# l-tamas/Fiasco

Hardware: AMD Instinct MI355X
Metric: grayscale frames/sec encoded (higher is better)
Workload: dtype f32

## Files before the change

### fiasco_amd/__init__.py

```python
import ctypes
import os
import subprocess

_HERE = os.path.dirname(os.path.abspath(__file__))
LIB_PATH = os.path.join(_HERE, "libfiasco_amd.so")
CSRC = os.path.join(_HERE, "csrc")

FIASCO_NO_VERBOSITY, FIASCO_SOME_VERBOSITY, FIASCO_ULTIMATE_VERBOSITY = 0, 1, 2
FIASCO_TILING_SPIRAL_ASC, FIASCO_TILING_SPIRAL_DSC = 0, 1
FIASCO_TILING_VARIANCE_ASC, FIASCO_TILING_VARIANCE_DSC = 2, 3
FIASCO_RPF_RANGE_0_75, FIASCO_RPF_RANGE_1_00, FIASCO_RPF_RANGE_1_50, FIASCO_RPF_RANGE_2_00 = 0, 1, 2, 3
FIASCO_PROGRESS_NONE, FIASCO_PROGRESS_BAR, FIASCO_PROGRESS_PERCENT = 0, 1, 2

EXPORTED_SYMBOLS = [
    "fiasco_get_error_message", "fiasco_set_verbosity", "fiasco_get_verbosity", "fiasco_coder",
    "fiasco_c_options_new", "fiasco_c_options_delete", "fiasco_c_options_set_smoothing",
    "fiasco_c_options_set_frame_pattern", "fiasco_c_options_set_tiling",
    "fiasco_c_options_set_basisfile", "fiasco_c_options_set_chroma_quality",
    "fiasco_c_options_set_optimizations", "fiasco_c_options_set_prediction",
    "fiasco_c_options_set_video_param", "fiasco_c_options_set_quantization",
    "fiasco_c_options_set_progress_meter", "fiasco_c_options_set_comment",
    "fiasco_c_options_set_title", "fiasco_calloc", "open_file", "fiasco_amd_set_limits",
    "fiasco_amd_get_limits", "fiasco_amd_encode_batch", "fiasco_amd_free",
    "fiasco_amd_get_stats", "fiasco_amd_reset_stats", "fiasco_amd_spec_workgroups", "fiasco_amd_core_name", "fiasco_amd_rccl_gather", "fiasco_amd_set_device",
    "fiasco_amd_batch_stage", "fiasco_amd_batch_encode", "fiasco_amd_batch_free",
    "fiasco_amd_batch_submit", "fiasco_amd_batch_collect", "fiasco_amd_batch_stats", "fiasco_amd_batch_decode_psnr", "fiasco_amd_batch_decode_psnr_all", "fiasco_amd_coop_workgroups", "fiasco_amd_share_of", "fiasco_amd_spec_append_helpers", "fiasco_amd_batch_decode_plane", "fiasco_amd_c_options_set_models",
    "fiasco_amd_release_memory", "fiasco_amd_batch_upload", "fiasco_amd_set_devices", "fiasco_amd_device_count",
    "fiasco_amd_selftest_log2", "fiasco_amd_selftest_log2_patched",
    "fiasco_amd_selftest_log2_max_ulp",
    "fiasco_amd_seq_open", "fiasco_amd_seq_free", "fiasco_amd_seq_gops", "fiasco_amd_seq_frames",
    "fiasco_amd_seq_gop_of", "fiasco_amd_seq_ycol_size", "fiasco_amd_seq_initial_level",
    "fiasco_amd_seq_search", "fiasco_amd_seq_gop_result", "fiasco_amd_seq_ycol", "fiasco_amd_seq_write",
    "fiasco_amd_seq_probe",
    "fiasco_amd_batch_stage_device", "fiasco_amd_batch_upload_device", "fiasco_amd_batch_input_planes",
]

FIASCO_AMD_GRAY8, FIASCO_AMD_RGB8_INTERLEAVED, FIASCO_AMD_RGB8_PLANAR = 0, 1, 2


class DeviceFrame(ctypes.Structure):
    _fields_ = [("data", ctypes.c_void_p), ("pitch", ctypes.c_size_t), ("plane_stride", ctypes.c_size_t),
                ("width", ctypes.c_uint), ("height", ctypes.c_uint), ("layout", ctypes.c_int)]


class Stats(ctypes.Structure):
    _fields_ = [("kernel_ms", ctypes.c_double), ("launches", ctypes.c_ulonglong),
                ("frames", ctypes.c_ulonglong), ("bytes_mp", ctypes.c_ulonglong),
                ("bytes_img", ctypes.c_ulonglong), ("bytes_gram", ctypes.c_ulonglong),
                ("n_mp", ctypes.c_ulonglong), ("n_steps", ctypes.c_ulonglong),
                ("n_blocks", ctypes.c_ulonglong), ("n_appends", ctypes.c_ulonglong),
                ("n_fulleval", ctypes.c_ulonglong), ("t_init", ctypes.c_ulonglong),
                ("t_approx", ctypes.c_ulonglong), ("t_ipis", ctypes.c_ulonglong),
                ("t_append", ctypes.c_ulonglong), ("t_serial", ctypes.c_ulonglong),
                ("t_total", ctypes.c_ulonglong), ("t_mpA", ctypes.c_ulonglong),
                ("t_mpB", ctypes.c_ulonglong), ("n_blockevals", ctypes.c_ulonglong),
                ("dbg", ctypes.c_ulonglong * 8), ("states_sum", ctypes.c_ulonglong),
                ("states_max", ctypes.c_ulonglong), ("reencodes", ctypes.c_ulonglong),
                ("frames_by_build", ctypes.c_ulonglong * 5),
                ("spec_frames", ctypes.c_ulonglong), ("spec_tasks", ctypes.c_ulonglong),
                ("spec_confirmed", ctypes.c_ulonglong), ("spec_wrong", ctypes.c_ulonglong),
                ("spec_timeout", ctypes.c_ulonglong), ("spec_inline", ctypes.c_ulonglong),
                ("spec_wait", ctypes.c_ulonglong), ("spec_tab_used", ctypes.c_ulonglong),
                ("spec_tab_missed", ctypes.c_ulonglong), ("spec_adopted", ctypes.c_ulonglong),
                ("decoder_frames", ctypes.c_ulonglong), ("decoder_bytes", ctypes.c_ulonglong),
                ("decoder_us", ctypes.c_ulonglong), ("coop_frames", ctypes.c_ulonglong),
                ("coop_workgroups", ctypes.c_ulonglong),
                ("spec_app_rows", ctypes.c_ulonglong), ("spec_app_wait", ctypes.c_ulonglong)]


def build(verbose=False):
    out = None if verbose else subprocess.DEVNULL
    subprocess.check_call(["make", "-C", CSRC], stdout=out)
    if not os.path.exists(LIB_PATH):
        raise RuntimeError("build did not produce %s" % LIB_PATH)


class FiascoError(RuntimeError):
    pass


class Library:

    def __init__(self, path=LIB_PATH):
        if not os.path.exists(path):
            raise FiascoError("%s is missing: run fiasco_amd.build() (there is no fallback)" % path)
        self.path = path
        L = self.L = ctypes.CDLL(path)
        c = ctypes
        L.fiasco_get_error_message.restype = c.c_char_p
        L.fiasco_set_verbosity.argtypes = [c.c_int]
        L.fiasco_get_verbosity.restype = c.c_int
        L.fiasco_c_options_new.restype = c.c_void_p
        L.fiasco_c_options_delete.argtypes = [c.c_void_p]
        L.fiasco_coder.argtypes = [c.POINTER(c.c_char_p), c.c_char_p, c.c_float, c.c_void_p]
        L.fiasco_coder.restype = c.c_int
        L.fiasco_amd_c_options_set_models.argtypes = [c.c_void_p, c.c_char_p, c.c_char_p, c.c_char_p, c.c_char_p]
        L.fiasco_amd_c_options_set_models.restype = c.c_int
        for name, args in [
            ("set_smoothing", [c.c_int]), ("set_frame_pattern", [c.c_char_p]),
            ("set_tiling", [c.c_int, c.c_uint]), ("set_basisfile", [c.c_char_p]),
            ("set_chroma_quality", [c.c_float, c.c_uint]),
            ("set_optimizations", [c.c_uint] * 5), ("set_prediction", [c.c_int, c.c_uint, c.c_uint]),
            ("set_video_param", [c.c_uint, c.c_int, c.c_int, c.c_int]),
            ("set_quantization", [c.c_uint, c.c_int, c.c_uint, c.c_int]),
            ("set_progress_meter", [c.c_int]), ("set_comment", [c.c_char_p]),
            ("set_title", [c.c_char_p]),
        ]:
            fn = getattr(L, "fiasco_c_options_" + name)
            fn.argtypes = [c.c_void_p] + args
            fn.restype = c.c_int
        L.fiasco_amd_set_limits.argtypes = [c.c_uint, c.c_uint]
        L.fiasco_amd_set_limits.restype = c.c_int
        L.fiasco_amd_get_limits.argtypes = [c.POINTER(c.c_uint), c.POINTER(c.c_uint)]
        L.fiasco_amd_encode_batch.argtypes = [c.c_uint, c.POINTER(c.c_char_p), c.POINTER(c.c_size_t),
                                              c.c_float, c.c_void_p, c.POINTER(c.c_void_p),
                                              c.POINTER(c.c_size_t)]
        L.fiasco_amd_encode_batch.restype = c.c_int
        L.fiasco_amd_free.argtypes = [c.c_void_p]
        L.fiasco_amd_core_name.restype = c.c_char_p
        if hasattr(L, "fiasco_amd_get_stats"):
            L.fiasco_amd_get_stats.argtypes = [c.POINTER(Stats)]

    def error_message(self):
        return self.L.fiasco_get_error_message().decode("latin-1")

    def core_name(self):
        return self.L.fiasco_amd_core_name().decode()

    def set_verbosity(self, level):
        self.L.fiasco_set_verbosity(level)

    def set_limits(self, max_states, max_level):
        if not self.L.fiasco_amd_set_limits(max_states, max_level):
            raise FiascoError(self.error_message())

    def get_limits(self):
        a, b = ctypes.c_uint(), ctypes.c_uint()
        self.L.fiasco_amd_get_limits(ctypes.byref(a), ctypes.byref(b))
        return a.value, b.value

    def set_devices(self, ids):
        arr = (ctypes.c_int * max(len(ids), 1))(*ids)
        self.L.fiasco_amd_set_devices.argtypes = [ctypes.POINTER(ctypes.c_int), ctypes.c_int]
        if not self.L.fiasco_amd_set_devices(arr, len(ids)):
            raise FiascoError(self.error_message())

    def device_count(self):
        return self.L.fiasco_amd_device_count()

    def set_device(self, device):
# ... 404 lines not shown
```

### fiasco_amd/csrc/hip/core_hip.cpp

```cpp
#include <hip/hip_runtime.h>
#include <stdio.h>
#include <stdlib.h>
#include <string.h>
#include <stddef.h>
#include <pthread.h>
#include <algorithm>
#include <utility>
#include <vector>
#include "fa_host.h"
#include "frame_coder.h"
#include "libfiasco_amd_hip.h"

extern "C" const char *fa_knob(const char *name)
{
    const char *d = getenv("FIASCO_AMD_DEBUG");
    return d && *d && strcmp(d, "0") != 0 ? getenv(name) : nullptr;
}
static long long knob_int(const char *name, long long d)
{
    const char *e = fa_knob(name);
    return e ? atoll(e) : d;
}


// ... 741 lines not shown
    return room > (size_t) G ? room - (size_t) G : 0;
}
static int spec_app_policy(size_t frames, int cus, int G, bool wide_build, int occ)
{
    if (!frames || G < 2 || cus < 1) return 0;
    size_t H = spec_app_room(frames, cus, G, occ);
    if (!wide_build) {
        return H >= 3 && 2 * frames * ((size_t) G + 3) <= 3 * (size_t) cus ? 3 : 0;
    }
    if (H > 3) H = 3;
    return H >= 2 ? (int) H : 0;
}
extern "C" int fiasco_amd_spec_append_helpers(unsigned frames, int cus, int G, int wide_build)
{
    return spec_app_policy(frames, cus, G, wide_build != 0, wide_build ? 1 : 4);
}

static int spec_groups(size_t frames, int cus, bool big_frames, bool narrow_only)
{
    const char *e = fa_knob("FIASCO_AMD_SPEC");
    if (e && atoi(e) <= 1) return 0;
    if (fa_knob("FIASCO_AMD_TRACE") || fa_knob("FIASCO_AMD_NO_WIDE") || fa_knob("FIASCO_AMD_FORCE_TRI")) return 0;
    int occ = fc_occupancy_spec();
    if (occ < 1) occ = 1;
    if (!frames) return 0;
    if (e) {
        size_t G = (size_t) cus * (size_t) occ / frames;
        if ((size_t) atoi(e) < G) G = (size_t) atoi(e);
        if (G > FC_SPEC_MAXG) G = FC_SPEC_MAXG;
        return G >= 2 ? (int) G : 0;
    }
    return spec_policy(frames, cus, big_frames, narrow_only, occ);
}

static int spec_policy(size_t frames, int cus, bool big_frames, bool narrow_only, int occ)
{
    if (!frames || cus < 1) return 0;
    size_t G = (size_t) cus / frames;
    if (G > FC_SPEC_MAXG) G = FC_SPEC_MAXG;
    if (narrow_only && !big_frames && occ >= 2) {
        G = (size_t) cus * (size_t) occ / frames;
        if (G > FC_SPEC_MAXG) G = FC_SPEC_MAXG;
        if (G > 5 && 2 * frames * G > 5 * (size_t) cus) {
            G = 5 * (size_t) cus / (2 * frames);
            if (G < 5) G = 5;
        }
    }
    (void) big_frames;
    return G >= 3 ? (int) G : 0;
}

static void fill_frame(FrameSlot &fs, const fa_job *job)
{
    const fa_cparams *cp = &job->cp;
    const fa_wfa *w = job->wfa;
    DevFrame &F = fs.F;
    const Layout &L = fs.L;
    char *base = fs.base;
    memset(&F, 0, sizeof F);
    F.price = cp->price;
    F.lc_min = (int) cp->lc_min_level; F.lc_max = (int) cp->lc_max_level;
    F.images_level = (int) cp->images_level; F.max_elements = (int) cp->max_elements;
    const bool bxl = long_basis(w);
    {
        unsigned live = cp->max_elements;
        for (unsigned st = 0; st < (bxl ? 0u : w->basis_states); st++)
            for (unsigned l = 0; l < 2; l++) {
                unsigned e = 0;
                while (e < 6 && FA_INTO(w, st, l, e) != FA_NO_EDGE) e++;
                if (e > live) live = e;
            }
        F.maxe_live = (int) live;
    }
    F.level = (int) cp->level; F.width = (int) job->image->width; F.height = (int) job->image->height;
    F.pool_max = (int) cp->pool_max_states; F.limit_states = (int) cp->limit_states;
    F.ML = (int) cp->limit_level;
    F.rpf_mant = (int) cp->rpf.mantissa_bits; F.dc_mant = (int) cp->dc_rpf.mantissa_bits;
    F.rpf_range = cp->rpf.range; F.dc_range = cp->dc_rpf.range;
    F.P = fs.P; F.PA = fs.PA;
    F.gram_ls = fs.tri ? (unsigned) ((size_t) fs.P * (fs.P + 1) / 2 + fs.P) : (unsigned) fs.P * (unsigned) fs.P;
    F.color = job->image->color ? 1 : 0;
    F.chroma_cl_cap = (int) knob_int("FIASCO_AMD_CLMAX", 0);
    F.chroma_sparse = !fa_knob("FIASCO_AMD_CHROMA_FULL") && (cp->pool_kind == FA_POOL_RLE || cp->pool_kind == FA_POOL_ADAPTIVE || cp->pool_kind == FA_POOL_BASIS);
    F.chroma_max = (int) cp->chroma_max_states;
    F.chroma_decrease = cp->chroma_decrease;
    F.plane = (unsigned long long) job->image->width * job->image->height;
    F.gl0 = (int) (cp->lc_min_level < cp->images_level ? cp->lc_min_level : cp->images_level);
    F.NL = (int) cp->lc_max_level - F.gl0 + 1;
    F.second_domain_block = cp->second_domain_block ? 1 : 0;
    F.check_underflow = cp->check_for_underflow ? 1 : 0;
    F.check_overflow = cp->check_for_overflow ? 1 : 0;
    F.full_search = cp->full_search ? 1 : 0;
    F.NS = (int) fa_size_of_tree(cp->products_level);
    F.NA = 1 << (cp->lc_max_level - cp->images_level);
    F.NI = (int) fa_size_of_tree(cp->images_level);
    F.dcs = 1 << (1 + F.dc_mant); F.sy = 1 << (1 + F.rpf_mant);
    F.coeff_size = (F.lc_max - F.lc_min + 1) * F.sy + F.dcs;
    F.coeff_nt = F.lc_max - F.lc_min + 2;
    F.basis_states = (int) w->basis_states;
    F.bx = bxl ? (const int *) (base + L.bx) : nullptr;
    F.gm_pool[0] = (int) cp->pool_kind; F.gm_pool[1] = (int) cp->d_pool_kind;
    F.gm_coeff[0] = (int) cp->coeff_kind; F.gm_coeff[1] = (int) cp->d_coeff_kind;
    F.gq = fs.gm ? (int16_t *) (base + L.gq) : nullptr;
    F.lginv = fs.gm ? (const double *) (base + L.lginv) : nullptr;
    for (unsigned s = 0; s < (bxl ? 0u : w->basis_states); s++) {
        F.b_final[s] = w->final_distribution[s];
        F.b_dtype[s] = w->domain_type[s];
        for (int l = 0; l < 2; l++) {
            F.b_tree[s][l] = FA_TREE(w, s, l);
            for (int e = 0; e < 6; e++) {
                F.b_into[s][l][e] = FA_INTO(w, s, l, e);
                F.b_weight[s][l][e] = FA_WEIGHT(w, s, l, e);
                if (FA_INTO(w, s, l, e) == FA_NO_EDGE) break;
            }
        }
    }
    F.pix16 = (const int16_t *) (base + L.pix16);
    F.gram = (float *) (base + L.gram); F.diag = (float *) (base + L.diag);
    F.ipis = (float *) (base + L.ipis); F.d5 = (float *) (base + L.d5);
    F.gcol = (float *) (base + L.gcol);
    F.d4 = (float *) (base + L.d4); F.imgT4 = (float *) (base + L.imgT4);
    F.img = (float *) (base + L.img); F.imgT = (float *) (base + L.imgT);
    F.norms = (float *) (base + L.norms);
    F.num = (float *) (base + L.num); F.den = (float *) (base + L.den);
    F.est = (float *) (base + L.est); F.ipdo = (float *) (base + L.ipdo);
    F.used = (uint8_t *) (base + L.used);
    F.tree = (int16_t *) (base + L.tree); F.into = (int16_t *) (base + L.into);
    F.weight = (float *) (base + L.weight); F.final_d = (float *) (base + L.final_d);
    F.level_of_state = (uint8_t *) (base + L.level_of_state);
    F.domain_type = (uint8_t *) (base + L.domain_type);
    F.x = (uint16_t *) (base + L.x); F.y = (uint16_t *) (base + L.y);
    F.ycol = (uint8_t *) (base + L.ycol);
    F.ycol0 = job->ycol_carry ? (const uint8_t *) (base + L.ycol0) : nullptr;
    F.pool_states = (int16_t *) (base + L.pool_states);
    F.pos = (int16_t *) (base + L.pos);
    F.hits = (int *) (base + L.hits);
    F.snap_hbm = fs.big ? (void *) (base + L.snap) : nullptr;
    F.l2_keys = g_l2.d_keys; F.l2_vals = g_l2.d_vals; F.l2_mask = g_l2.mask;
    const int inter = job->frame_type != FA_I_FRAME;
    F.pred_on = cp->prediction || inter ? 1 : 0;
    F.pred_root = job->image->color ? inter : (cp->prediction || inter ? 1 : 0);
    F.search_range = (int) cp->search_range;
    F.mv = (int16_t *) (base + L.mv);
    F.past = (const int16_t *) (base + L.past); F.future = (const int16_t *) (base + L.future);
    F.coop = (FcCoop *) (base + L.coop);
    F.mc_fwd = (float *) (base + L.mc_fwd); F.mc_bwd = inter ? (float *) (base + L.mc_bwd) : nullptr;
    F.pix_chroma = (int16_t *) (base + L.pix_chroma);
    F.frame_type = job->frame_type;
    F.p_min = (int) cp->p_min_level; F.p_max = (int) cp->p_max_level;
    F.d_rpf_mant = (int) cp->d_rpf.mantissa_bits; F.d_dc_mant = (int) cp->d_dc_rpf.mantissa_bits;
    F.d_rpf_range = cp->d_rpf.range; F.d_dc_range = cp->d_dc_rpf.range;
    F.d_dcs = 1 << (1 + F.d_dc_mant); F.d_sy = 1 << (1 + F.d_rpf_mant);
    F.d_coeff_size = (F.lc_max - F.lc_min + 1) * F.d_sy + F.d_dcs;
    F.ipis_alt = (float *) (base + L.ipis_alt); F.d5_alt = (float *) (base + L.d5_alt);
    F.d4_alt = (float *) (base + L.d4_alt); F.pix_save = (float *) (base + L.pix_save);
    F.sv_gram = (float *) (base + L.sv_gram); F.sv_img = (float *) (base + L.sv_img);
    F.sv_auto = (FcSavedRow *) (base + L.sv_auto);
    F.max_save = L.max_save;
    F.slab_base = base; F.slab_bytes = L.total;
}

static void slot_layout(Staged *S, FrameSlot &fs)
{
    const fa_job *job = &S->jobs[fs.job];
    const fa_cparams *cp = &job->cp;
    int il = (int) cp->images_level;
// ... 431 lines not shown
    }
    const char *const host = pinned;
    const int16_t *tree = (const int16_t *) host;
    const int16_t *into = (const int16_t *) (host + (L.into - L.tree));
    const float *weight = (const float *) (host + (L.weight - L.tree));
    const float *fin = (const float *) (host + (L.final_d - L.tree));
    const uint8_t *los = (const uint8_t *) (host + (L.level_of_state - L.tree));
    const uint8_t *dt = (const uint8_t *) (host + (L.domain_type - L.tree));
    const uint16_t *xs = (const uint16_t *) (host + (L.x - L.tree));
    const uint16_t *ys = (const uint16_t *) (host + (L.y - L.tree));
    const uint8_t *ycol = (const uint8_t *) (host + (L.ycol - L.tree));
    const int16_t *mv = (const int16_t *) (host + (L.mv - L.tree));
    const bool inter = job->frame_type != FA_I_FRAME;
    for (unsigned s = 0; s < w->basis_states; s++) w->level_of_state[s] = 0xff;
    fa_wfa_remove_states(w, w->basis_states);
    for (unsigned s = w->basis_states; s < ns; s++) {
        w->final_distribution[s] = fin[s];
        w->domain_type[s] = dt[s];
        w->level_of_state[s] = los[s];
        w->delta_state[s] = 0;
        for (int l = 0; l < 2; l++) {
            FA_TREE(w, s, l) = tree[(size_t) l * P + s];
            w->x[s * 2 + l] = xs[(size_t) l * P + s];
            w->y[s * 2 + l] = ys[(size_t) l * P + s];
            w->y_state[s * 2 + l] = FA_RANGE;
            w->y_column[s * 2 + l] = F.color ? ycol[(size_t) l * P + s] : 0;
            w->prediction[s * 2 + l] = 0;
            if (inter) {
                fa_mv *m = &w->mv[s * 2 + l];
                m->type = mv[(size_t) (0 * 2 + l) * P + s]; m->fx = mv[(size_t) (1 * 2 + l) * P + s];
                m->fy = mv[(size_t) (2 * 2 + l) * P + s]; m->bx = mv[(size_t) (3 * 2 + l) * P + s];
                m->by = mv[(size_t) (4 * 2 + l) * P + s];
            }
            for (int e = 0; e < 6; e++) {
                FA_INTO(w, s, l, e) = into[(size_t) (l * 6 + e) * P + s];
                FA_WEIGHT(w, s, l, e) = weight[(size_t) (l * 6 + e) * P + s];
                if (FA_INTO(w, s, l, e) == FA_NO_EDGE) break;
            }
        }
    }
    if (F.color)
        for (unsigned s = 0; s < w->cap && s < (unsigned) P; s++)
            for (int l = 0; l < 2; l++) w->y_column[s * 2 + l] = ycol[(size_t) l * P + s];
    w->states = ns;
    w->root_state = (unsigned) F.root_state;
    job->stats[0].costs = F.costs; job->stats[0].err = F.err;
    job->stats[0].tree_bits = F.tree_bits; job->stats[0].matrix_bits = F.matrix_bits;
    job->stats[0].weights_bits = F.weights_bits;
    if (F.color) {
        for (int b = 0; b < 2; b++) {
            job->stats[b + 1].costs = F.c_costs[b]; job->stats[b + 1].err = F.c_err[b];
            job->stats[b + 1].tree_bits = F.c_tree_bits[b];
            job->stats[b + 1].matrix_bits = F.c_matrix_bits[b];
            job->stats[b + 1].weights_bits = F.c_weights_bits[b];
        }
        int ycb = FA_TREE(w, ns - 1, 0), crs = FA_TREE(w, ns - 1, 1);
        int roots[2] = { FA_TREE(w, ycb, 1), FA_TREE(w, crs, 0) };
        int yroot = FA_TREE(w, ycb, 0);
        std::vector<std::pair<int, int>> stack;
        for (int b = 0; b < 2; b++) {
            stack.push_back(std::make_pair(roots[b], yroot));
            while (!stack.empty()) {
                std::pair<int, int> t = stack.back();
                stack.pop_back();
                int s = t.first, y = t.second;
                if (s == FA_RANGE || (unsigned) s < w->basis_states) continue;
                for (int l = 0; l < 2; l++) {
                    int ny = y != FA_RANGE ? FA_TREE(w, y, l) : FA_RANGE;
                    w->y_state[s * 2 + l] = (int16_t) ny;
                    stack.push_back(std::make_pair((int) FA_TREE(w, s, l), ny));
                }
            }
        }
    }
    job->lc_min_level_out = (unsigned) F.lc_min_out;
    job->status = 1;
    g_stats.frames += 1;
    g_stats.bytes_mp += F.bytes_mp; g_stats.bytes_img += F.bytes_img; g_stats.bytes_gram += F.bytes_gram;
    g_stats.n_mp += F.n_mp; g_stats.n_steps += F.n_steps; g_stats.n_blocks += F.n_blocks;
    g_stats.n_appends += F.n_appends; g_stats.n_fulleval += F.n_fulleval;
    g_stats.t_init += F.t_init; g_stats.t_approx += F.t_approx; g_stats.t_ipis += F.t_ipis;
    g_stats.t_append += F.t_append; g_stats.t_serial += F.t_serial; g_stats.t_total += F.t_total;
    g_stats.t_mpA += F.t_mpA; g_stats.t_mpB += F.t_mpB; g_stats.n_blockevals += F.n_blockevals;
    for (int k = 0; k < 8; k++) g_stats.dbg[k] += F.dbg[k];
    g_stats.states_sum += ns;
    if (ns > g_stats.states_max) g_stats.states_max = ns;
    cap_hint_put(job, F.ystates_out, F.states);
    if (fa_knob("FIASCO_AMD_CAP_TRACE"))
        fprintf(stderr, "capacity: frame type %d used %d table states of %d, %d states of %d; %.3f s on the device\n", job->frame_type,
                F.ystates_out, fs.P, F.states, fs.PA, (double) F.t_total / 1e8);
    return 1;
}

static bool queue_resources(Staged *S, size_t frames)
{
    if (!grow_buffer(S->d_ring, S->ring_n, 5 * frames)) return false;
    if (!S->d_queue && hipMalloc((void **) &S->d_queue, 2 * 5 * sizeof(unsigned)) != hipSuccess) {
        S->d_queue = nullptr; (void) hipGetLastError(); return false;
    }
    if (!S->ptrmask_ready) {
        const size_t words = FC_DESC_WORDS, mwords = (words + 31) / 32;
        std::vector<unsigned> mask(mwords, 0u);
        FrameSlot a = S->slots[S->lender0], b = S->slots[S->lender0];
        const fa_job *job = &S->jobs[a.job];
        b.base = a.base + (1u << 24);
        fill_frame(a, job); fill_frame(b, job);
        const unsigned long long *wa = (const unsigned long long *) &a.F, *wb = (const unsigned long long *) &b.F;
        for (size_t w = 0; w < sizeof(DevFrame) / 8; w++)
            if (wa[w] != wb[w]) mask[w >> 5] |= 1u << (w & 31);
        const size_t wp = offsetof(DevFrame, pack_src) / 8;
        mask[wp >> 5] |= 1u << (wp & 31);
        if (!S->d_ptrmask && hipMalloc((void **) &S->d_ptrmask, mwords * sizeof(unsigned)) != hipSuccess) {
            S->d_ptrmask = nullptr; (void) hipGetLastError(); return false;
        }
        if (hipMemcpy(S->d_ptrmask, mask.data(), mwords * sizeof(unsigned), hipMemcpyHostToDevice) != hipSuccess) return false;
        S->ptrmask_ready = true;
    }
    return true;
}

struct WaveGroups { size_t n[N_BUILDS], lend[N_BUILDS], borrow[N_BUILDS]; };

static bool order_batch(Staged *S, WaveGroups &g)
{
    std::vector<size_t> &batch = S->batch;
    batch.clear();
    for (size_t k = 0; k < S->slots.size(); k++)
        if (S->slots[k].staged && !S->slots[k].done) batch.push_back(k);
    if (batch.empty()) return false;
    memset(&g, 0, sizeof g);
    const bool few = batch.size() <= (size_t) S->ncu && !fa_knob("FIASCO_AMD_NO_WIDE");
    std::vector<int> key(S->slots.size());
    for (size_t k : batch) {
        const FrameSlot &fs = S->slots[k];
        const Build b = build_of(S, fs, few);
        const int part = fs.borrow ? 1 : S->borrowers && queue_eligible(S, fs) && queue_layout(S, fs) ? 0 : 2;
        key[k] = 3 * b + part;
        g.n[b]++;
        if (part == 0) g.lend[b]++; else if (part == 1) g.borrow[b]++;
        if (k_build[b].stats_slot >= 0) g_stats.frames_by_build[k_build[b].stats_slot]++; else g_stats.spec_frames++;
    }
    std::stable_sort(batch.begin(), batch.end(), [&](size_t a, size_t b) { return key[a] < key[b]; });
    return true;
}

static void place_packs(Staged *S)
{
    const std::vector<size_t> &batch = S->batch;
    std::vector<DevFrame> &hf = S->hf;
    hf.resize(batch.size());
    S->pack_off.assign(batch.size(), 0);
    size_t need = 0;
    for (size_t b = 0; b < batch.size(); b++) {
        const FrameSlot &fs = S->slots[batch[b]];
        hf[b] = fs.F;
        hf[b].pack_src = fs.F.slab_base + fs.L.tree;
        hf[b].pack_bytes = (unsigned) (fs.L.pool_states - fs.L.tree);
        S->pack_off[b] = need;
        need += align_up(fs.L.pool_states - fs.L.tree, 256);
    }
    S->pack_need = need;
    S->parity ^= 1;
    char *&pack = S->d_pack[S->parity];
    (void) grow_buffer(pack, S->d_pack_bytes[S->parity], need);
    if (!S->cstream && hipStreamCreateWithFlags(&S->cstream, hipStreamNonBlocking) != hipSuccess) {
        S->cstream = nullptr; (void) hipGetLastError();
// ... 930 lines not shown
```

### fiasco_amd/csrc/hip/fc_lds.inc

```

#define RANGE_E (FC_MAXE + 1)
struct __attribute__((aligned(16))) Range {
    int   x, y, image, address, level, tree;
    float weight[RANGE_E];
    short into[RANGE_E];
    float err, tree_bits, matrix_bits, weights_bits;
#if FC_VARIANT_BIG
    float nd_tree_bits, nd_weights_bits, mv_tree_bits, mv_coord_bits;
    int   prediction;
    short mv[5];
#endif
};

struct Pool {
    short count[MAXED + 1];
    unsigned short total, n, max_domains, y_index;
    short d0_index;
    unsigned short d0_yindex, d0_n;
};

struct __attribute__((aligned(16))) SFrame {
    Range rg, lrange, rrange, child[2];
    Pool  pool0, pool_lc;
    float max_costs, lincomb, subdiv, ret, price;
    int   label, states, phase, leaf, coop;
    int   y_state, ny[2];
#if FC_GM
    int   rn0;
#endif
#if FC_SPEC
    int   ckpt;
#endif
#if FC_VARIANT_BIG
    int   pred, delta, try_pred, pred_done, rec_states;
    int   norm_first, norm_done;
    Pool  dpool0, pool_rec, dpool_rec;
    Range prange;
    float pred_max, pred_costs, nd_w, nd_wbits, nd_tbits;
#endif
};

struct MPState {
    int   n, best_n, index, D, N, level, image, address, row_state;
    short indices[MAXED + 1], into[MAXED + 1];
    float weight[MAXED];
    unsigned symp;
    float matrix_bits, weights_bits, err, costs, min_costs;
    float sel_ipdo[MAXED][MAXED];
    float norm_ov[MAXED + 1], ipio[MAXED + 1];
    short psorted[MAXED + 1];
    int   np;
    float wb_dc, wb_nd, norm, ab, price;
    int   y_state, ypos;
#if FC_VARIANT_BIG
    const float *numrow;
    short excl[MAXED + 1];
#endif
#if FC_GM
    short kq[MAXED + 1];
#endif
    float s1_pre[MAXED], s1_sfx[MAXED], s1_z0, s1_zy;
    int   s1_last[MAXED], s1_k[MAXED], s1_thr[MAXED];
    unsigned s1_cd, s1_has;
};

struct __attribute__((aligned(16))) CoeffBuf {
    short tot[16];
    short cnt[FC_VARIANT_BIG ? FC_MAXCOEFF_BIG : FC_MAXCOEFF];
};
#if FC_VARIANT_BIG
#define SNAP_POOL16 880
#define SNAP_TM_WORDS 2392
#else
#define SNAP_POOL16 (FC_VARIANT_WIDE ? FC_SNAP16_WIDE : FC_SNAP16_NARROW)
#define SNAP_TM_WORDS (FC_VARIANT_WIDE ? FC_SNAPTM_WIDE : FC_SNAPTM_NARROW)
#endif
#if FC_VARIANT_BIG || FC_VARIANT_WIDE
#define NBLOCKMIN   256
#else
#define NBLOCKMIN   64
#endif
#define TM_WORDS    (4 * 26 + 8)

struct RoundBox {
    float m2[2];
    int   state;
    int   idx;
    float cost, mbits, wbits, err, f[MAXED];
    float num, den, ip[MAXED - 1];
    unsigned evals, blockevals;
    unsigned symp;
};
#define SYMP_NONE 0u
#define SYMP_HAS(p, k) ((k) < 3 && (((p) >> (10 * (k))) & 1023u) != 0u)
#define SYMP_GET(p, k) ((int) (((p) >> (10 * (k))) & 1023u) - 2)
#define SYMP_PUT(sym, k) ((unsigned) ((sym) + 2) << (10 * (k)))

struct Sh {
    RoundBox rb;
    SFrame   st[FC_DEPTH];
    int      sp;
    int      op, a0, a1, a2, a3;
#if FC_VARIANT_BIG
    unsigned coopW, coop_seq;
    int      coopD, coop_minsub;
    unsigned long long coop_ticks;
#endif
    Pool     pool;
    CoeffBuf cb;
#if FC_VARIANT_BIG
    Pool     dpool;
    CoeffBuf dcb;
    struct { int rpf_mant, dc_mant, sy, dcs; float rpf_range, dc_range; int half_nd, half_dc; } dq;
    int      nslot;
    uint4   *snap_tm_p;
    int      pred_active, pred_lo, pred_rec;
    struct { int type, fx, fy, bx, by; float bits, tree_bits; } mc;
    unsigned long long mcred[B / 64];
    unsigned pred_saved[FC_MAXSAVE / 32];
#endif
    uint4    snap_pool[SNAP_POOL16];
    uint4   *snap;
    int      n16;
    __attribute__((aligned(16))) unsigned tm[TM_WORDS];
    __attribute__((aligned(16))) unsigned snap_tm[SNAP_TM_WORDS];
    float    m0tab[12];
    double   lgdc[FC_MAXSYM], lglv[FC_MAXSYM], lglv_m1;
    float    Ltab[MAXED + 1];
    float    Q0, Q1;
    float    tb[2];
    MPState  mp;
#if FC_VARIANT_BIG
    MPState  mp_keep;
    int      apx_stage, apx_it, apx_more;
#endif
    float    blockmin[NBLOCKMIN];
    __attribute__((aligned(16))) float pixels[FC_PIXELS];
    float    norms[FC_PIXELS / 32];
    unsigned long long tk[16];
    struct {
        unsigned long long bytes_mp, bytes_img, bytes_gram, n_mp, n_steps, n_blocks, n_appends,
                           n_fulleval, n_blockevals, t_mpA, t_mpB;
    } cnt;
#ifdef FC_SERIAL_PROFILE
    unsigned long long tk_ph[8], ph_t0, tk_init[2], tk_apx[4];
    int      ph_prev;
#endif
    int      band, lc_min, tree_band[3], ystates, after_chroma;
    short    dl[64];
#if !FC_SPEC
    short    cl[FC_CLMAX];
    int      cln;
#endif
    unsigned long long red[B / 64];
    int      gs_idx[2][MAXED + 1], gs_n[2], gs_c[2], gs_raw_idx[2][MAXED + 1];
    float    gs_raw_w[2][MAXED + 1];
    float    gs_w[2][MAXED + 1];
    struct {
        int lc_max, width, height, limit_states, PA, P, ML; float price, chroma_decrease;
        float *gram, *diag, *ipis; int16_t *pos; unsigned gram_ls;
        float *gcol;
        float *d5, *d4;
        const unsigned *l2_keys; const double *l2_vals; unsigned l2_mask;
        int max_elements, rpf_mant, dc_mant, sy, dcs, gl0, images_level, lc_min_opt, trace_on;
        int snap_b1;
        int16_t *at_tree, *at_into, *at_pool; float *at_weight, *at_final; uint8_t *at_los, *at_dtype, *at_ycol;
        uint16_t *at_x, *at_y; int color;
        float rpf_range, dc_range;
        int half_nd, half_dc;
    } par;
#if FC_GM
    struct { int pk[2], ck[2], qa; float base, kept; double lg1; int16_t *gq; int P; } gm;
#endif
    int      states;
    int      flim;
    int      failed;
#if FC_SPEC
    int      gap_lo, gap_hi, gap_shift;
    unsigned deadmask;
    int      cap;
    int      blk;
    int      tab_shared;
    int      tab_from;
    struct SpecLocal {
        FcSpecCtl *ctl;
        char     *slots;
        int       role, on;
        int       mode;
        int       T;
        int       chroma_tabs;
        char     *tabs;
        unsigned  rb_s[32];
        unsigned  blkof[FC_SPEC_W];
        unsigned  sk[FC_SPEC_W];
        unsigned long long n_tab_used, n_tab_missed, n_adopted;
        int       floor;
        unsigned  head, commit;
        unsigned  spec_mask;
        int       nospec;
        unsigned  epoch;
        int       verdict, abort, busy;
        unsigned  ops;
        float     mlc, lin[FC_SPEC_W];
        unsigned  nlc;
        float     learn;
        unsigned long long n_tasks, n_confirmed, n_wrong, n_timeout, n_inline, t_wait;
        unsigned  app_H, app_min, app_seq, app_off;
        unsigned long long n_app_dealt, t_app_wait;
    } sl;
#endif
};
#if FC_GM
#define GM_QAC(k)   ((k) == FC_PK_ADAPTIVE || (k) == FC_PK_BASIS)
#define GM_RLE(k)   ((k) == FC_PK_RLE || (k) == FC_PK_RLE_NO_CHROMA)
#define GQ_CUR(sh, set)          ((sh).gm.gq + (size_t) ((sh).gm.qa ^ (set)) * (sh).gm.P)
#define GQ_SNAP(sh, depth, slot) ((sh).gm.gq + (size_t) (2 + (depth) * 5 + (slot)) * (sh).gm.P)
#endif
#if FC_SPEC
#define DEAD(sh, s) ((unsigned) ((int) (s) - (sh).gap_lo) < (unsigned) ((sh).gap_hi - (sh).gap_lo))
#else
#define DEAD(sh, s) false
#endif
```

### fiasco_amd/csrc/hip/fc_models.inc

```

#if FC_VARIANT_BIG
#define SNAP(sh) ((sh).snap)
#define NSLOT(sh) ((sh).nslot)
#define SNAP_TM(sh) ((sh).snap_tm_p)
#define TM_SLOTS(sh) ((sh).nslot == 5 ? 2 : 1)
#else
#define SNAP(sh) ((sh).snap_pool)
#define NSLOT(sh) 2
#define SNAP_TM(sh) ((uint4 *) (sh).snap_tm)
#define TM_SLOTS(sh) 1
#endif
#if FC_VARIANT_BIG
#define SNAP_AT(sh, depth, which) (SNAP(sh) + ((depth) * NSLOT(sh) + (which)) * (sh).n16)
#else
#define SNAP_AT(sh, depth, which) (SNAP(sh) + ((which) ? (sh).par.snap_b1 + (depth) : (depth)) * (sh).n16)
#endif
#if FC_VARIANT_BIG
#define TM_N16(ML) (ML)
#else
#define TM_N16(ML) ((2 * (ML) + 3) / 4)
#endif
#define TM_AT(sh, depth, which, ML) (SNAP_TM(sh) + ((depth) * TM_SLOTS(sh) + (which)) * TM_N16(ML))

#if FC_GM

__device__ __forceinline__ float gm_m0(const Sh &sh, int idx) { return sh.m0tab[qac_shift(idx)]; }
__device__ __forceinline__ float gm_m1(int idx) { return (float) qac_shift(idx); }

__device__ void gq_copy(int16_t *dst, const int16_t *src, int n)
{
    const int n16 = (n + 7) / 8;
    for (int i = 0; i < n16; i++) ((uint4 *) dst)[i] = ((const uint4 *) src)[i];
}
__device__ void gq_save(Sh &sh, int set, int depth, int slot)
{
    if (GM_QAC(sh.gm.pk[set])) gq_copy(GQ_SNAP(sh, depth, slot), GQ_CUR(sh, set), set ? sh.dpool.n : sh.pool.n);
}
__device__ void gq_load(Sh &sh, int set, int depth, int slot)
{
    if (GM_QAC(sh.gm.pk[set])) gq_copy(GQ_CUR(sh, set), GQ_SNAP(sh, depth, slot), set ? sh.dpool.n : sh.pool.n);
}
__device__ __forceinline__ void gq_save_par(Sh &sh, int set, int depth, int slot)
{
    if (!GM_QAC(sh.gm.pk[set])) return;
    const int n = set ? sh.dpool.n : sh.pool.n;
    int16_t *d = GQ_SNAP(sh, depth, slot);
    const int16_t *c = GQ_CUR(sh, set);
    for (int i = threadIdx.x; i < n; i += B) d[i] = c[i];
}

__device__ __forceinline__ bool gm_accepts(const Pool &m, int kind)
{
    return kind == FC_PK_CONSTANT || kind == FC_PK_UNIFORM || m.n < m.max_domains;
}
__device__ bool gm_take(Sh &sh, Pool &m, int kind, int set, int state)
{
    if (kind == FC_PK_CONSTANT) return false;
    if (kind != FC_PK_UNIFORM && m.n >= m.max_domains) return false;
    if (GM_QAC(kind)) { int16_t *q = GQ_CUR(sh, set); q[m.n] = m.n > 0 ? q[m.n - 1] : (int16_t) 0; }
    if (GM_RLE(kind) && state == 0) { m.d0_index = 0; m.d0_n = 1; }
    m.n++;
    return true;
}
__device__ void gm_offer(DevFrame &F, Sh &sh, int s)
{
    const int L = sh.pool.n > sh.dpool.n ? sh.pool.n : sh.dpool.n;
    bool grow = gm_take(sh, sh.pool, sh.gm.pk[0], 0, s);
    if (F.pred_on) grow = gm_take(sh, sh.dpool, sh.gm.pk[1], 1, s) || grow;
    F.pos[s] = -1;
    if (grow) { F.pos[s] = (short) L; F.pool_states[L] = (short) s; }
}
#endif

__device__ __forceinline__ void snap_coop_before(Sh &sh, SFrame &fr, int depth, int ML)
{
    const int tid = threadIdx.x;
#if FC_HM
    for (int i = tid; i < sh.n16; i += B) SNAP_AT(sh, depth, 0)[i] = ((const uint4 *) &sh.cb)[i];
    if (tid >= 96 && tid < 96 + TM_N16(ML)) TM_AT(sh, depth, 0, ML)[tid - 96] = ((const uint4 *) sh.tm)[tid - 96];
    if (tid == 128) fr.pool0 = sh.pool;
#if FC_GM
    if (tid == 130) fr.rn0 = sh.dpool.n;
    gq_save_par(sh, 0, depth, 0);
#endif
    if (sh.nslot == 5 && !fr.delta) {
        if (tid == 129) fr.dpool0 = sh.dpool;
        for (int i = tid; i < sh.n16; i += B) SNAP_AT(sh, depth, 2)[i] = ((const uint4 *) &sh.dcb)[i];
#if FC_GM
        gq_save_par(sh, 1, depth, 2);
#endif
    }
    return;
#endif
    if (tid < sh.n16) SNAP_AT(sh, depth, 0)[tid] = ((const uint4 *) &sh.cb)[tid];
    else if (tid >= 96 && tid < 96 + TM_N16(ML))
        TM_AT(sh, depth, 0, ML)[tid - 96] = ((const uint4 *) sh.tm)[tid - 96];
    else if (tid == 128) fr.pool0 = sh.pool;
#if FC_VARIANT_BIG
    else if (sh.nslot == 5 && !fr.delta) {
        if (tid == 129) fr.dpool0 = sh.dpool;
        else if (tid >= 160 && tid < 160 + sh.n16) SNAP_AT(sh, depth, 2)[tid - 160] = ((const uint4 *) &sh.dcb)[tid - 160];
    }
#endif
}

__device__ __forceinline__ void snap_coop_after(Sh &sh, SFrame &fr, int depth)
{
    const int tid = threadIdx.x;
#if FC_HM
    for (int i = tid; i < sh.n16; i += B) {
        SNAP_AT(sh, depth, 1)[i] = ((const uint4 *) &sh.cb)[i];
        ((uint4 *) &sh.cb)[i] = SNAP_AT(sh, depth, 0)[i];
    }
#if FC_GM
    if (GM_QAC(sh.gm.pk[0])) {
        const int n1 = sh.pool.n, n0 = fr.pool0.n;
        int16_t *cur = GQ_CUR(sh, 0), *s1 = GQ_SNAP(sh, depth, 1);
        const int16_t *s0 = GQ_SNAP(sh, depth, 0);
        for (int i = tid; i < (n1 > n0 ? n1 : n0); i += B) {
            if (i < n1) s1[i] = cur[i];
            if (i < n0) cur[i] = s0[i];
        }
    }
    __syncthreads();
#endif
    if (tid == 128) {
#else
    if (tid < sh.n16) {
        SNAP_AT(sh, depth, 1)[tid] = ((const uint4 *) &sh.cb)[tid];
        ((uint4 *) &sh.cb)[tid] = SNAP_AT(sh, depth, 0)[tid];
    } else if (tid == 128) {
#endif
        fr.pool_lc = sh.pool;
        sh.pool = fr.pool0;
#if FC_GM
        if (fr.delta) sh.dpool.n = (unsigned short) fr.rn0;
#endif
    }
}

__device__ float tree_bits_dev(const Sh &sh, int ML, int child, int level, int which);
```

### fiasco_amd/csrc/hip/fc_serial.inc

```


__device__ float tree_bits_dev(const Sh &sh, int ML, int child, int level, int which)
{
    const unsigned *counts = sh.tm + which * 2 * ML;
    float prob = counts[level] / (float) counts[ML + level];
    return child ? (float) -log2((double) prob) : (float) -log2((double) (1 - prob));
}

__device__ void tree_update_dev(Sh &sh, int ML, int child, int level, int which)
{
    unsigned *counts = sh.tm + which * 2 * ML;
    if (child) counts[level]++;
    counts[ML + level]++;
}

__device__ __forceinline__ void copy16(uint4 *dst, const uint4 *src, int n)
{
    int i = 0;
    for (; i + 8 <= n; i += 8) {
        uint4 t0 = src[i], t1 = src[i + 1], t2 = src[i + 2], t3 = src[i + 3];
        uint4 t4 = src[i + 4], t5 = src[i + 5], t6 = src[i + 6], t7 = src[i + 7];
        dst[i] = t0; dst[i + 1] = t1; dst[i + 2] = t2; dst[i + 3] = t3;
        dst[i + 4] = t4; dst[i + 5] = t5; dst[i + 6] = t6; dst[i + 7] = t7;
    }
    for (; i < n; i++) dst[i] = src[i];
}

__device__ void snap_save(const DevFrame &F, Sh &sh, int depth, int which)
{
    copy16(SNAP_AT(sh, depth, which), (const uint4 *) &sh.cb, sh.n16);
}

__device__ void snap_load(const DevFrame &F, Sh &sh, int depth, int which)
{
    copy16((uint4 *) &sh.cb, SNAP_AT(sh, depth, which), sh.n16);
}

#if FC_VARIANT_BIG
__device__ void snap_save_d(Sh &sh, int depth, int which)
{
    copy16(SNAP_AT(sh, depth, which), (const uint4 *) &sh.dcb, sh.n16);
}

__device__ void snap_load_d(Sh &sh, int depth, int which)
{
    copy16((uint4 *) &sh.dcb, SNAP_AT(sh, depth, which), sh.n16);
}
#endif

__device__ __forceinline__ void tm_save(Sh &sh, int depth, int ML, int which = 0)
{
    copy16(TM_AT(sh, depth, which, ML), (const uint4 *) sh.tm, TM_N16(ML));
}

__device__ __forceinline__ void tm_load(Sh &sh, int depth, int ML, int which = 0)
{
    copy16((uint4 *) sh.tm, TM_AT(sh, depth, which, ML), TM_N16(ML));
}

__device__ float final_distribution_dev(const DevFrame &F, int s)
{
    float f = 0;
    int dom;
    for (int l = 0; l < 2; l++) {
        if ((dom = TREE(F, s, l)) != RANGE_) f += F.final_d[dom];
        for (int e = 0; (dom = INTO(F, s, l, e)) != NOEDGE; e++)
            f += WEIGHT(F, s, l, e) * F.final_d[dom];
    }
    return f / 2;
}

#if !FC_VARIANT_BIG
__device__ void store_new_state(DevFrame &__restrict__ F, Sh &sh, SFrame &fr, int aux)
{
    const int s = sh.states, PA = sh.par.PA;
    GLOBAL_AS int16_t *const tree = (GLOBAL_AS int16_t *) sh.par.at_tree, *const into = (GLOBAL_AS int16_t *) sh.par.at_into;
    GLOBAL_AS int16_t *const posv = (GLOBAL_AS int16_t *) sh.par.pos, *const pool = (GLOBAL_AS int16_t *) sh.par.at_pool;
    GLOBAL_AS float *const weight = (GLOBAL_AS float *) sh.par.at_weight, *const fin = (GLOBAL_AS float *) sh.par.at_final;
    GLOBAL_AS uint16_t *const xs = (GLOBAL_AS uint16_t *) sh.par.at_x, *const ys = (GLOBAL_AS uint16_t *) sh.par.at_y;
    short p = -1;
    if (!aux && sh.pool.n < sh.pool.max_domains) {
        p = (short) sh.pool.n;
        pool[sh.pool.n++] = (short) s;
    }
    posv[s] = p;
    fr.rrange.into[0] = NOEDGE;
    fr.rrange.tree = s;
    int   tr[2], i[2][3];
    float w[2][3], fd_t[2], fd_e[2][3];
#pragma unroll
    for (int l = 0; l < 2; l++) {
        const Range &ch = fr.child[l];
        tr[l] = ch.tree;
        bool live = true;
#pragma unroll
        for (int e = 0; e < 3; e++) {
// ... 103 lines not shown
    F.final_d[s] = final_distribution_dev(F, s);
    F.level_of_state[s] = (uint8_t) fr.rrange.level;
    F.domain_type[s] = aux ? 0 : 2;
}
#endif

__device__ int append_join_state(DevFrame &__restrict__ F, Sh &__restrict__ sh, int t0, int t1, int level)
{
    const int s = sh.states;
    if (s >= F.PA) { sh.failed = FC_ERR_CAPACITY; return 0; }
    TREE(F, s, 0) = (short) t0; TREE(F, s, 1) = (short) t1;
    for (int l = 0; l < 2; l++) {
        INTO(F, s, l, 0) = NOEDGE;
        F.x[l * F.PA + s] = 0; F.y[l * F.PA + s] = 0;
    }
    F.final_d[s] = final_distribution_dev(F, s);
    F.level_of_state[s] = (uint8_t) level;
    F.domain_type[s] = 0;
    F.pos[s] = -1;
#if FC_VARIANT_BIG
    if (F.frame_type) for (int k = 0; k < 10; k++) F.mv[k * F.PA + s] = 0;
#endif
    sh.states++;
    if (sh.states >= F.limit_states) { sh.failed = FC_ERR_STATES; return 0; }
    return 1;
}

__device__ void push_root(DevFrame &__restrict__ F, Sh &__restrict__ sh, int y_state)
{
    SFrame &r = sh.st[0];
    r.rg.x = r.rg.y = r.rg.image = r.rg.address = 0;
    r.rg.level = F.level; r.rg.tree = RANGE_;
    for (int i = 0; i < RANGE_E; i++) { r.rg.weight[i] = 0; r.rg.into[i] = 0; }
    r.rg.err = r.rg.tree_bits = r.rg.matrix_bits = r.rg.weights_bits = 0;
    r.max_costs = MAXCOSTS;
    r.y_state = y_state;
    r.phase = PH_ENTER;
#if FC_SPEC
    r.ckpt = 0;
#endif
#if FC_VARIANT_BIG
    r.rg.nd_tree_bits = r.rg.nd_weights_bits = r.rg.mv_tree_bits = r.rg.mv_coord_bits = 0; r.rg.prediction = 0;
    for (int i = 0; i < 5; i++) r.rg.mv[i] = 0;
    r.pred = sh.band == 0 ? F.pred_root : 0;
    r.delta = 0;
#endif
    sh.sp = 0;
}

__device__ int band_advance(DevFrame &__restrict__ F, Sh &__restrict__ sh)
{
    if (!sh.after_chroma) {
        const SFrame &r = sh.st[0];
        const Range &rg = r.rg;
        const int band = sh.band;
        if (band == 0) {
            F.costs = r.ret; F.err = rg.err; F.tree_bits = rg.tree_bits;
            F.matrix_bits = rg.matrix_bits; F.weights_bits = rg.weights_bits;
            F.root_state = rg.tree;
        } else {
            F.c_costs[band - 1] = r.ret; F.c_err[band - 1] = rg.err;
            F.c_tree_bits[band - 1] = rg.tree_bits; F.c_matrix_bits[band - 1] = rg.matrix_bits;
            F.c_weights_bits[band - 1] = rg.weights_bits;
        }
        if (sh.failed) return 0;
        if (rg.tree == RANGE_) { sh.failed = FC_ERR_NOROOT; return 0; }
        if (!F.color) return 0;
        sh.tree_band[band] = rg.tree;
        if (band == 1) {
            if (!append_join_state(F, sh, sh.tree_band[0], sh.tree_band[1], F.level + 1)) return 0;
            sh.tree_band[1] = sh.states - 1;
        }
        if (band == 2) {
            if (!append_join_state(F, sh, sh.tree_band[2], RANGE_, F.level + 1)) return 0;
            if (!append_join_state(F, sh, sh.tree_band[1], sh.states - 1, F.level + 2)) return 0;
            F.root_state = sh.states - 1;
            return 0;
        }
        sh.band = band + 1;
        if (band == 0) { sh.op = OP_CHROMA; sh.after_chroma = 1; return 1; }
    }
    sh.after_chroma = 0;
    sh.op = OP_NOP;
    push_root(F, sh, sh.tree_band[0]);
    return 1;
}

#if FC_SPEC
#define SPEC_DEKKER_FENCE() __builtin_amdgcn_fence(__ATOMIC_SEQ_CST, "agent")
#define SPEC_TIMEOUT_TICKS 20000000ull
__device__ __noinline__ int spec_poll(Sh &sh, bool drain)
{
    Sh::SpecLocal &sl = sh.sl;
    FcSpecCtl *c = sl.ctl;
    unsigned long long t0 = 0;
    if (sl.learn != 0.0f) { sl.mlc = sl.nlc ? 0.9f * sl.mlc + 0.1f * sl.learn : sl.learn; sl.nlc++; sl.learn = 0.0f; }
    while (sl.commit != sl.head) {
        const unsigned slot = sl.commit % FC_SPEC_W;
        const bool mine = (sl.spec_mask >> slot) & 1u;
        if (!mine) { sl.commit++; t0 = 0; continue; }
        const unsigned v = __hip_atomic_load(&c->verdict[slot], __ATOMIC_RELAXED, __HIP_MEMORY_SCOPE_AGENT);
        if ((v >> 11) != sl.commit + 1) {
            if (!drain && sl.head - sl.commit < FC_SPEC_W) {
                __hip_atomic_store(&c->committed, sl.commit, __ATOMIC_RELAXED, __HIP_MEMORY_SCOPE_AGENT);
                return 0;
            }
            const unsigned long long now = wall_clock64();
            if (!t0) t0 = now;
            if (now - t0 < SPEC_TIMEOUT_TICKS) { __builtin_amdgcn_s_sleep(16); continue; }
            sl.t_wait += now - t0;
            sl.n_timeout++;
        } else {
            if (t0) { sl.t_wait += wall_clock64() - t0; t0 = 0; }
            if ((v & 3u) == 1u) {
                if (sh.par.color) {
                    GLOBAL_AS uint8_t *yc = (GLOBAL_AS uint8_t *) sh.par.at_ycol;
                    const unsigned used = (v >> 2) & 63u, s0 = sl.sk[slot];
                    for (unsigned j = 0; j < used; j++) { yc[s0 + j] = 0; yc[(unsigned) sh.par.PA + s0 + j] = 0; }
                }
                sl.mlc = sl.nlc ? 0.9f * sl.mlc + 0.1f * sl.lin[slot] : sl.lin[slot]; sl.nlc++;
                sl.commit++; sl.n_confirmed++;
                continue;
            }
            sl.n_wrong++;
            if ((v & 3u) == 3u && sl.sk[slot] + ((v >> 2) & 63u) <= (unsigned) sh.cap)
                return (1 + (int) slot) | 0x100 | (int) (((v >> 2) & 63u) << 16) | (int) (((v >> 8) & 7u) << 24);
        }
        return 1 + (int) slot;
    }
    __hip_atomic_store(&c->committed, sl.commit, __ATOMIC_RELAXED, __HIP_MEMORY_SCOPE_AGENT);
    return 0;
}
#endif

#if FC_SPEC
__device__ __noinline__ void spec_luminance_done(Sh &sh)
{
    FcSpecCtl *c = sh.sl.ctl;
    sh.sl.epoch++;
    __hip_atomic_store(&c->epoch, sh.sl.epoch, __ATOMIC_RELEASE, __HIP_MEMORY_SCOPE_AGENT);
    SPEC_DEKKER_FENCE();
    const unsigned long long t0 = wall_clock64();
    while (__hip_atomic_load(&c->busy, __ATOMIC_ACQUIRE, __HIP_MEMORY_SCOPE_AGENT) != 0) {
        if (wall_clock64() - t0 > 100000000ull) { sh.failed = FC_ERR_INTERNAL; break; }
        __builtin_amdgcn_s_sleep(32);
    }
    sh.sl.on = 0; sh.sl.mode = 0;
    sh.sl.chroma_tabs = c->n_tabs > c->n_blocks;
}
#endif

#ifndef FC_SERIAL_LOOP
#define FC_SERIAL_LOOP 0
#endif
__device__ __forceinline__ int serial_step(DevFrame &__restrict__ F, Sh &__restrict__ sh, int &sp, int &phase)
{
    const int ML = sh.par.ML;
    {
#if FC_SPEC
        const int spec_mode = *(volatile int *) &sh.sl.mode;
#endif
        if (sp < 0) {
            sh.sp = sp;
#if FC_SPEC
            if (spec_mode == 1) {
                sh.op = OP_SPEC_CKPT; sh.a0 = 2;
                return 0;
            }
#endif
            const int more = band_advance(F, sh);
            sp = sh.sp; phase = sp >= 0 ? sh.st[sp].phase : 0;
            if (!more) { sh.op = OP_DONE; return 0; }
            if (sh.op == OP_CHROMA) return 0;
            return 1;
        }
        SFrame &fr = sh.st[sp];
#ifdef FC_SERIAL_PROFILE
        {
            unsigned long long t = wall_clock64();
            sh.tk_ph[sh.ph_prev] += t - sh.ph_t0; sh.ph_t0 = t; sh.ph_prev = phase;
        }
#endif
        switch (phase) {
        case PH_ENTER: {
            Range &rg = fr.rg;
            rg.into[0] = NOEDGE;
            rg.tree = RANGE_;
            fr.ret = MAXCOSTS;
            if (sh.failed || rg.level < 3) { fr.ret = MAXCOSTS; goto pop; }
            if (rg.x >= sh.par.width || rg.y >= sh.par.height) { fr.ret = 0; goto pop; }
#if FC_SPEC
#endif
            fr.price = sh.par.price;
            if (sh.band) fr.price *= sh.par.chroma_decrease;
#if FC_VARIANT_BIG
            fr.try_pred = 0;
            if (fr.pred && rg.level >= F.p_min && rg.level <= F.p_max) {
                if (F.frame_type == 0) fr.try_pred = 1;
                else if (rg.x + (int) width_of_level(rg.level) <= sh.par.width
                         && rg.y + (int) height_of_level(rg.level) <= sh.par.height) fr.try_pred = 2;
            }
            fr.pred_done = 0;
            fr.norm_first = 1; fr.norm_done = 0;
#endif
            phase = PH_AFTER_INIT;
            if (rg.level == sh.par.lc_max) {
                rg.address = rg.image = 0;
                sh.op = OP_INIT_RANGE; sh.a0 = rg.x; sh.a1 = rg.y;
#if FC_SPEC
                sh.a2 = (!sh.band || sh.sl.chroma_tabs) ? sh.blk++ : -1;
#endif
                return 0;
            }
            break;
        }
        case PH_AFTER_INIT: {
            Range &rg = fr.rg;
#if FC_SPEC
            if (spec_mode == 1 && rg.level == sh.par.lc_max && !sh.band && !fr.ckpt && sp > 0) {
                fr.ckpt = 1; sh.op = OP_SPEC_CKPT; sh.a0 = 1;
                return 0;
            }
#endif
            fr.leaf = rg.level <= sh.lc_min && rg.level <= sh.par.lc_max;
#if FC_VARIANT_BIG
            if (fr.try_pred) fr.leaf = 0;
#endif
            fr.coop = !fr.leaf && rg.level <= sh.par.lc_max;
            if (!fr.leaf && !fr.coop) {
                fr.pool0 = sh.pool;
                snap_save(F, sh, sp, 0);
                tm_save(sh, sp, ML);
#if FC_GM
                fr.rn0 = sh.dpool.n;
                gq_save(sh, 0, sp, 0);
#endif
#if FC_VARIANT_BIG
                if (sh.nslot == 5 && !fr.delta) {
                    fr.dpool0 = sh.dpool; snap_save_d(sh, sp, 2);
#if FC_GM
                    gq_save(sh, 1, sp, 2);
#endif
                }
#endif
            }
            fr.states = sh.states;
            for (int l = 0; l < 2; l++)
                fr.ny[l] = (sh.band && fr.y_state != RANGE_) ? (int) TREE(F, fr.y_state, l) : RANGE_;
            phase = PH_AFTER_LC;
            if (rg.level <= sh.par.lc_max) {
                fr.lrange = rg;
                fr.lrange.tree = RANGE_;
#if FC_VARIANT_BIG
                fr.lrange.tree_bits = tree_bits_dev(sh, ML, 0, rg.level, 0);
#endif
                fr.lrange.matrix_bits = 0;
                fr.lrange.weights_bits = 0;
#if FC_VARIANT_BIG
                fr.lrange.nd_tree_bits = 0; fr.lrange.nd_weights_bits = 0; fr.lrange.prediction = 0;
                fr.lrange.mv_tree_bits = fr.try_pred == 2 ? 1.0f : 0.0f;
                fr.lrange.mv_coord_bits = 0;
#endif
                sh.op = OP_APPROX;
                return 0;
            }
            fr.lincomb = MAXCOSTS;
            break;
        }
        case PH_AFTER_LC: {
            Range &rg = fr.rg;
            if (fr.leaf) {
                fr.subdiv = MAXCOSTS;
                phase = PH_DECIDE;
                break;
            }
            if (!fr.coop) {
#if FC_VARIANT_BIG
                fr.pool_lc = sh.pool;
                snap_save(F, sh, sp, 1);
#if FC_GM
                gq_save(sh, 0, sp, 1);
#endif
                sh.pool = fr.pool0;
                snap_load(F, sh, sp, 0);
#if FC_GM
                gq_load(sh, 0, sp, 0);
                if (fr.delta) sh.dpool.n = (unsigned short) fr.rn0;
#endif
#else
                fr.pool_lc = sh.pool;
#endif
            }
#if FC_SPEC
            if (fr.ckpt == 3) {
                fr.subdiv = MAXCOSTS;
                phase = PH_DECIDE;
                break;
            }
#endif
            if (rg.level > sh.lc_min) {
                Range z;
                z.x = z.y = z.image = z.address = z.level = 0; z.tree = 0;
                for (int i = 0; i < RANGE_E; i++) { z.weight[i] = 0; z.into[i] = 0; }
                z.err = z.tree_bits = z.matrix_bits = z.weights_bits = 0;
#if FC_VARIANT_BIG
                z.nd_tree_bits = z.nd_weights_bits = z.mv_tree_bits = z.mv_coord_bits = 0; z.prediction = 0;
                for (int i = 0; i < 5; i++) z.mv[i] = 0;
#endif
                fr.child[0] = z; fr.child[1] = z;
                fr.rrange = rg;
#if FC_VARIANT_BIG
                fr.rrange.tree_bits = tree_bits_dev(sh, ML, 1, rg.level, 0);
#else
                fr.rrange.tree_bits = rg.level <= sh.par.lc_max ? sh.tb[1] : tree_bits_dev(sh, ML, 1, rg.level, 0);
#endif
                fr.rrange.matrix_bits = 0;
                fr.rrange.weights_bits = 0;
                fr.rrange.err = 0;
#if FC_VARIANT_BIG
                fr.rrange.mv_tree_bits = fr.try_pred == 2 ? 1.0f : 0.0f;
                fr.rrange.mv_coord_bits = 0;
                fr.rrange.nd_tree_bits = fr.try_pred == 1 ? tree_bits_dev(sh, ML, 1, rg.level, 1) : 0.0f;
                fr.rrange.nd_weights_bits = 0;
                fr.rrange.prediction = 0;
                fr.subdiv = (fr.rrange.tree_bits + fr.rrange.weights_bits + fr.rrange.matrix_bits
                             + fr.rrange.mv_tree_bits + fr.rrange.mv_coord_bits + fr.rrange.nd_tree_bits
                             + fr.rrange.nd_weights_bits) * fr.price;
#else
                fr.subdiv = (fr.rrange.tree_bits + fr.rrange.weights_bits + fr.rrange.matrix_bits) * fr.price;
#endif
                fr.label = 0;
                phase = PH_CHILD;
            } else {
                fr.subdiv = MAXCOSTS;
                phase = PH_DECIDE;
            }
            break;
        }
        case PH_CHILD: {
            const Range &rr = fr.rrange;
            const int label = fr.label;
            Range &ch = fr.child[label];
            ch.image = rr.image * 2 + label + 1;
            ch.address = rr.address * 2 + label;
            ch.level = rr.level - 1;
            ch.x = (rr.level & 1) ? rr.x : rr.x + label * (int) width_of_level(rr.level - 1);
            ch.y = (rr.level & 1) ? rr.y + label * (int) height_of_level(rr.level - 1) : rr.y;
            phase = PH_CHILD2;
            if (label && rr.level <= sh.par.lc_max && sh.states > fr.states && !sh.band) {
                sh.op = OP_IPIS_INCR; sh.a0 = ch.image; sh.a1 = ch.address; sh.a2 = ch.level;
                sh.a3 = fr.states;
                return 0;
            }
            break;
        }
        case PH_CHILD2: {
            float lim = fr.lincomb > fr.max_costs ? fr.max_costs : fr.lincomb;
            float remaining = lim - fr.subdiv;
            phase = PH_CHILD_RET;
            fr.ret = 0;
            if (remaining > 0) {
                if (sp + 1 >= FC_DEPTH) { sh.failed = FC_ERR_INTERNAL; break; }
                SFrame &cf = sh.st[sp + 1];
                cf.rg = fr.child[fr.label];
                cf.y_state = fr.ny[fr.label];
                cf.max_costs = remaining;
                cf.phase = PH_ENTER;
#if FC_SPEC
                cf.ckpt = 0;
#endif
#if FC_VARIANT_BIG
                cf.pred = fr.pred; cf.delta = fr.delta;
#endif
                fr.phase = phase; sp++; phase = PH_ENTER;
                break;
            }
            fr.ret = -1;
            break;
        }
        case PH_CHILD_RET: {
            const int label = fr.label;
            float lim = fr.lincomb > fr.max_costs ? fr.max_costs : fr.lincomb;
#if FC_VARIANT_BIG
            if (fr.try_pred == 2 && !fr.norm_done) {
                const Range &c0 = fr.child[label];
                sh.op = OP_NORMS; sh.a0 = fr.rg.level; sh.a1 = fr.norm_first;
                sh.a2 = (fr.ret < 0 && c0.level >= F.p_min) ? c0.level : -1;
                sh.a3 = c0.x | (c0.y << 16);
                fr.norm_first = 0; fr.norm_done = 1;
                return 0;
            }
            fr.norm_done = 0;
#endif
            if (fr.ret >= 0) fr.subdiv += fr.ret;
            if (fr.subdiv >= lim) {
                fr.subdiv = MAXCOSTS;
                phase = PH_DECIDE;
                break;
            }
            const Range &ch = fr.child[label];
            fr.rrange.err          += ch.err;
            fr.rrange.tree_bits    += ch.tree_bits;
            fr.rrange.matrix_bits  += ch.matrix_bits;
            fr.rrange.weights_bits += ch.weights_bits;
#if FC_VARIANT_BIG
            fr.rrange.mv_tree_bits    += ch.mv_tree_bits;
            fr.rrange.mv_coord_bits   += ch.mv_coord_bits;
            fr.rrange.nd_weights_bits += ch.nd_weights_bits;
            fr.rrange.nd_tree_bits    += ch.nd_tree_bits;
            tree_update_dev(sh, ML, ch.tree != RANGE_, ch.level, 0);
            tree_update_dev(sh, ML, !ch.prediction, ch.level, 1);
#else
            tree_update_dev(sh, ML, ch.tree != RANGE_, ch.level, 0);
#endif
            fr.label = label + 1;
            phase = fr.label < 2 ? PH_CHILD : PH_DECIDE;
            break;
        }
        case PH_DECIDE: {
            Range &rg = fr.rg;
#if FC_SPEC
            if (spec_mode >= 2 && sp == spec_mode - 2) {
                sh.sl.verdict = (!sh.failed && !fr.leaf && fr.lincomb < MAXCOSTS && fr.lincomb < fr.subdiv) ? 1 : 2;
                if (!sh.failed && !fr.leaf && fr.subdiv < MAXCOSTS && !(fr.lincomb < fr.subdiv)) sh.sl.verdict = 3;
                sh.op = OP_DONE;
                return 0;
            }
#endif
#if FC_VARIANT_BIG
            if (fr.try_pred && !fr.pred_done && !sh.failed) { phase = PH_PRED_BEGIN; break; }
#endif
            if (fr.leaf) {
                if (fr.lincomb < MAXCOSTS) { rg = fr.lrange; fr.ret = fr.lincomb; }
                else fr.ret = MAXCOSTS;
                goto pop;
            } else if (fr.lincomb >= MAXCOSTS && fr.subdiv >= MAXCOSTS) {
                sh.pool = fr.pool0;
                snap_load(F, sh, sp, 0);
                tm_load(sh, sp, ML);
#if FC_GM
                gq_load(sh, 0, sp, 0);
                if (fr.delta) sh.dpool.n = (unsigned short) fr.rn0;
#endif
#if FC_VARIANT_BIG
                if (sh.nslot == 5 && !fr.delta) {
                    sh.dpool = fr.dpool0; snap_load_d(sh, sp, 2);
#if FC_GM
                    gq_load(sh, 1, sp, 2);
#endif
                }
#endif
                sh.states = fr.states;
                if (sh.flim > sh.states) sh.flim = sh.states & ~(GRAM_FB - 1);
                fr.ret = MAXCOSTS;
                goto pop;
            } else if (fr.lincomb < fr.subdiv) {
#if FC_SPEC
                if (fr.ckpt == 2 && spec_mode == 1) sh.sl.learn = fr.lincomb;
#endif
                sh.pool = fr.pool_lc;
                snap_load(F, sh, sp, 1);
                tm_load(sh, sp, ML);
#if FC_GM
                gq_load(sh, 0, sp, 1);
                if (fr.delta) sh.dpool.n = (unsigned short) fr.rn0;
#endif
#if FC_VARIANT_BIG
                if (sh.nslot == 5 && !fr.delta) {
                    sh.dpool = fr.dpool0; snap_load_d(sh, sp, 2);
#if FC_GM
                    gq_load(sh, 1, sp, 2);
#endif
                }
#endif
                rg = fr.lrange;
                sh.states = fr.states;
                if (sh.flim > sh.states) sh.flim = sh.states & ~(GRAM_FB - 1);
                fr.ret = fr.lincomb;
                goto pop;
            } else {
                int aux = sh.band > 0 || rg.x + (int) width_of_level(rg.level) > sh.par.width
                          || rg.y + (int) height_of_level(rg.level) > sh.par.height;
#if FC_VARIANT_BIG
#if FC_GM
                if (!(gm_accepts(sh.pool, sh.gm.pk[0]) || !F.pred_on || gm_accepts(sh.dpool, sh.gm.pk[1]))) aux = 1;
#else
                if (F.pred_on && sh.pool.n >= sh.pool.max_domains) aux = 1;
#endif
#endif
#if FC_SPEC
                if (sh.states >= (sh.band ? sh.par.PA : *(volatile int *) &sh.cap)) { sh.failed = FC_ERR_CAPACITY; fr.ret = MAXCOSTS; goto pop; }
#else
                if (sh.states >= (sh.band ? sh.par.PA : sh.par.P)) { sh.failed = FC_ERR_CAPACITY; fr.ret = MAXCOSTS; goto pop; }
#endif
                store_new_state(F, sh, fr, aux);
                phase = PH_AFTER_APPEND;
                if (!aux) { sh.op = OP_APPEND; sh.a0 = sh.states; return 0; }
                break;
            }
        }
#if FC_SPEC
        case PH_SPEC_END: {
            sh.sl.verdict = 2; sh.op = OP_DONE;
            return 0;
        }
#endif
        case PH_AFTER_APPEND: {
            sh.states++;
#if FC_SPEC
            if (sh.states - *(volatile int *) &sh.gap_shift >= sh.par.limit_states) sh.failed = FC_ERR_STATES;
#else
            if (sh.states >= sh.par.limit_states) sh.failed = FC_ERR_STATES;
#endif
            fr.rg = fr.rrange;
            fr.ret = fr.subdiv;
            goto pop;
        }
#if FC_VARIANT_BIG
        case PH_PRED_BEGIN: {
            Range &rg = fr.rg;
            const int il = sh.par.images_level, P = sh.par.P;
            float maxc = fr.lincomb > fr.subdiv ? fr.subdiv : fr.lincomb;
            if (maxc > fr.max_costs) maxc = fr.max_costs;
            fr.pred_done = 1;
            fr.pred_max = maxc;
            fr.rec_states = sh.states;
            fr.pool_rec = sh.pool; fr.dpool_rec = sh.dpool;
            snap_save(F, sh, sp, 3); snap_save_d(sh, sp, 4); tm_save(sh, sp, ML, 1);
#if FC_GM
            gq_save(sh, 0, sp, 3); gq_save(sh, 1, sp, 4);
#endif
            sh.pool = fr.pool0; sh.dpool = fr.dpool0;
            snap_load(F, sh, sp, 0); snap_load_d(sh, sp, 2); tm_load(sh, sp, ML, 0);
#if FC_GM
            gq_load(sh, 0, sp, 0); gq_load(sh, 1, sp, 2);
#endif
            sh.states = fr.states;
            if (sh.flim > sh.states) sh.flim = sh.states & ~(GRAM_FB - 1);
            if (fr.try_pred == 2) {
                sh.op = OP_MC_SEARCH; sh.a0 = rg.level; sh.a1 = rg.x | (rg.y << 16);
                sh.a2 = (rg.level == F.p_min ? 1 : 0) | (rg.level > F.p_min && fr.norm_first ? 2 : 0);
                phase = PH_PRED_MC2;
                return 0;
            }
            {
// ... 147 lines not shown
```

### fiasco_amd/csrc/hip/frame_coder.h

```cpp
#ifndef FRAME_CODER_H
#define FRAME_CODER_H
#include <stdint.h>

#define FC_MAXED    5
#define FC_BLOCK    256
#define FC_MAXDEPTH 22
#define FC_MAXDEPTH_BIG 32
#define FC_MAXDEPTH_NARROW 18
#define FC_SNAP16_NARROW 480
#define FC_SNAP16_WIDE   840
#define FC_SNAPTM_NARROW 988
#define FC_SNAPTM_WIDE   1092
#define FC_MAXSAVE  512
#define FC_MAXCOEFF 224
#ifndef FC_HM
#define FC_HM 0
#endif
#ifndef FC_GM
#define FC_GM 0
#endif
enum { FC_PK_ADAPTIVE = 0, FC_PK_CONSTANT = 1, FC_PK_BASIS = 2, FC_PK_UNIFORM = 3, FC_PK_RLE = 4, FC_PK_RLE_NO_CHROMA = 5 };
enum { FC_CK_ADAPTIVE = 0, FC_CK_UNIFORM = 1 };
#define FC_GQ_SLOTS (2 + FC_MAXDEPTH_BIG * 5)
#define FC_MAXCOEFF_BIG_STD 640
#define FC_MAXSYM_STD   64
#define FC_MAXCOEFF_HM  5120
#define FC_MAXSYM_HM    512
#define FC_MAXCOEFF_BIG (FC_HM ? FC_MAXCOEFF_HM : FC_MAXCOEFF_BIG_STD)
#define FC_MAXSYM       (FC_HM ? FC_MAXSYM_HM : FC_MAXSYM_STD)
#define FC_N16(coeffs)  ((32 + 2 * (coeffs) + 15) / 16)
#define FC_N16MAX       FC_N16(FC_MAXCOEFF_BIG)
#define FC_MAXBASIS 16
#define FC_BX_BYTES (64 * 1024)
#ifndef FC_TRI_HOT
#define FC_TRI_HOT  8
#endif

enum { FC_OK = 1, FC_ERR_STATES = 2, FC_ERR_CAPACITY = 3, FC_ERR_NOROOT = 4, FC_ERR_INTERNAL = 5,
       FC_ERR_QUEUE = 6,
       FC_ERR_COOP = 7 };
struct FcCoop {
    unsigned seq;
    unsigned done;
    unsigned quit;
    unsigned depth;
    int      level, from, to;
    int      minsub;
    float   *ipis, *d5, *d4;
    unsigned long long done_ticks;
};
#define FC_COOP_HDR 128
#define FC_COOP_WAIT_TICKS 3000000000ull
#define FC_COOP_DONE_TICKS 500000000ull
#define FC_QUEUE_WAIT_TICKS 60000000000ull

struct FcTrace;
typedef struct DevFrame {
    float    price;
    int      lc_min, lc_max, images_level, max_elements;
    int      maxe_live;
    int      gl0;
    int      second_domain_block;
    int      check_underflow, check_overflow, full_search;
    int      level, width, height;
    int      pool_max, limit_states, ML;
    int      rpf_mant, dc_mant;
    float    rpf_range, dc_range;
    int      P;
    unsigned gram_ls;
    int      PA;
    int      color;
    int      chroma_sparse;
    int      chroma_cl_cap;
    int      chroma_max;
    float    chroma_decrease;
    unsigned long long plane;
    int      NL, NS, NA, NI;
    int      coeff_size, coeff_nt, dcs, sy;
    int      basis_states;
    int16_t  b_tree[FC_MAXBASIS][2];
    int16_t  b_into[FC_MAXBASIS][2][6];
    float    b_weight[FC_MAXBASIS][2][6];
    float    b_final[FC_MAXBASIS];
    uint8_t  b_dtype[FC_MAXBASIS];
    const int *bx;
    int      gm_pool[2], gm_coeff[2];
    int16_t *gq;
    const double *lginv;
    const int16_t *pix16;
    float   *gram, *diag, *ipis, *d5, *img, *imgT, *norms;
    float   *gcol;
    float   *d4, *imgT4;
    float   *num, *den, *est, *ipdo;
    uint8_t *used;
    int16_t *tree, *into;
    float   *weight, *final_d;
    uint8_t *level_of_state, *domain_type;
    uint16_t *x, *y;
    uint8_t *ycol;
    const uint8_t *ycol0;
    void    *snap_hbm;
    int      pred_root;
    int      pred_on;
    int      frame_type;
    int      p_min, p_max;
    int      d_rpf_mant, d_dc_mant;
    float    d_rpf_range, d_dc_range;
    int      d_coeff_size, d_dcs, d_sy;
    float   *ipis_alt, *d5_alt, *d4_alt;
    float   *pix_save;
    float   *sv_gram;
    float   *sv_img;
    struct FcSavedRow *sv_auto;
    int      max_save;
    const int16_t *past, *future;
    float   *mc_fwd, *mc_bwd;
    int16_t *mv;
    int16_t *pix_chroma;
    int      search_range;
    int16_t *pool_states;
    int16_t *pos;
    int     *hits;
    const void *pack_src;
    void    *pack_dst;
    unsigned pack_bytes;
    const unsigned *l2_keys;
    const double   *l2_vals;
    unsigned        l2_mask;
    int      status;
    int      states, root_state;
    FcCoop  *coop;
    int      ystates_out;
    float    costs, err, tree_bits, matrix_bits, weights_bits;
    float    c_costs[2], c_err[2], c_tree_bits[2], c_matrix_bits[2], c_weights_bits[2];
    int      lc_min_out;
    unsigned long long bytes_mp, bytes_img, bytes_gram;
    unsigned long long n_mp, n_steps, n_blocks, n_appends, n_fulleval;
    unsigned long long t_init, t_approx, t_ipis, t_append, t_serial, t_total;
    unsigned long long t_mpA, t_mpB, n_blockevals;
    unsigned long long dbg[8];
    struct FcTrace *trace;
    int      trace_cap, trace_n;
    char    *slab_base;
    unsigned long long slab_bytes;
    struct FcSpecCtl *spec;
    int      spec_role, spec_G;
    int      spec_tb;
    int      spec_cap;
    int      spec_T;
} DevFrame;

#define FC_DESC_WORDS ((sizeof(DevFrame) + 7) / 8)

#define FC_SPEC_W      16
#define FC_SPEC_TEMPS  16
#define FC_SPEC_MAXG   8
#define FC_SPEC_R      24
typedef struct FcSpecCtl {
    unsigned next;
    unsigned epoch;
    unsigned done;
    unsigned committed;
    unsigned adopting;
    unsigned busy;
    unsigned slot_bytes;
    unsigned slot_seq[FC_SPEC_W];
    unsigned verdict[FC_SPEC_W];
    unsigned long long n_tasks, n_confirmed, n_wrong, n_timeout, n_inline, t_wait;
    unsigned long long n_tab_used, n_tab_missed;
    unsigned long long n_adopted;
    unsigned s_pub;
    unsigned tab_free;
    unsigned blk_cur;
    unsigned chroma_ready, tab_next, ystates;
    unsigned n_tabs;
    unsigned n_blocks;
    unsigned tab_stride;
    unsigned tab_wait;
    unsigned long long off_blocks, off_tabs;
    unsigned tab_seq[FC_SPEC_R];
    unsigned tab_s[FC_SPEC_R];
    unsigned tab_epoch[FC_SPEC_R];
    unsigned app_H;
    unsigned app_min;
    unsigned app_wait;
    unsigned app_seq;
    unsigned app_done;
    unsigned app_off;
    unsigned app_dbg;
    int      app_s, app_flim;
    int      app_n[2], app_c[2], app_idx[2][FC_MAXED + 1];
    float    app_w[2][FC_MAXED + 1];
    unsigned long long n_app_dealt, t_app_wait;
} FcSpecCtl;

typedef struct FcSavedRow {
    int16_t  tree[2], into[2][6];
    float    weight[2][6];
    float    final_d;
    uint16_t x[2], y[2];
    int16_t  pos;
    int16_t  mv[2][5];
    uint8_t  level, dtype, ycol[2], tables;
} FcSavedRow;

typedef struct FcTrace {
    int   seq, level, image, D, states, nedges;
    float cost, err, mbits, wbits;
    short into[6];
    float w[5];
} FcTrace;

#endif
```

### fiasco_amd/csrc/hip/frame_coder.hip

```cpp
#include <hip/hip_runtime.h>
#include <stdint.h>
#include <math.h>
#include "frame_coder.h"

#include "fc_config.inc"
#include "fc_lds.inc"
#include "fc_access.inc"
#include "fc_tables.inc"
#include "fc_append.inc"
#include "fc_predict.inc"
#include "fc_models.inc"
#include "mp_device.inc"
#include "fc_serial.inc"
#include "fc_spec.inc"

__device__ void basis_init(DevFrame &F, Sh &sh)
{
    const int nb = F.basis_states, il = F.images_level;
    for (int s = 0; s < nb; s++) {
        F.img[(size_t) s * F.NI] = F.final_d[s];
        if (il == 0) F.imgT[s] = F.final_d[s];
    }
    for (int l = 1; l <= il; l++)
        for (int s = 0; s < nb; s++)
// ... 102 lines not shown
    if (threadIdx.x == 0) {
        sh.coopW = F.coop ? cW : 1; sh.coop_seq = 0;
        sh.coopD = cW > 1 && F.coop ? (int) F.coop->depth : 0; sh.coop_minsub = cW > 1 && F.coop ? F.coop->minsub : 0;
        sh.coop_ticks = cW > 1 && F.coop ? F.coop->done_ticks : 0;
    }
#else
    DevFrame &F = frames[blockIdx.x];
#endif
    const int tid = threadIdx.x;

#if !FC_SPEC
    if (ring && blockIdx.x >= nlend) {
        __shared__ unsigned long long got;
        if (tid == 0) {
            const unsigned t = atomicAdd(&ctr[0], 1u);
            unsigned long long b;
            const unsigned long long t_give_up = wall_clock64() + queue_wait_ticks;
            while ((b = __hip_atomic_load(&ring[t], __ATOMIC_ACQUIRE, __HIP_MEMORY_SCOPE_AGENT)) == 0) {
                if (wall_clock64() > t_give_up) break;
                __builtin_amdgcn_s_sleep(32);
            }
            got = b;
        }
        __syncthreads();
        if (got == 0) {
            if (tid == 0) { F.status = FC_ERR_QUEUE; F.states = 0; }
            return;
        }
        {
            unsigned long long *d = (unsigned long long *) &F;
            const unsigned long long lo = (unsigned long long) F.slab_base, span = F.slab_bytes;
            const unsigned long long delta = got - lo;
            unsigned long long v[(FC_DESC_WORDS + B - 1) / B];
#pragma unroll
            for (unsigned k = 0; k < (FC_DESC_WORDS + B - 1) / B; k++) {
                const unsigned w = k * B + tid;
                v[k] = w < FC_DESC_WORDS ? d[w] : 0;
            }
            __syncthreads();
#pragma unroll
            for (unsigned k = 0; k < (FC_DESC_WORDS + B - 1) / B; k++) {
                const unsigned w = k * B + tid;
                if (w < FC_DESC_WORDS && ((ptrmask[w >> 5] >> (w & 31)) & 1u) && v[k] - lo < span) d[w] = v[k] + delta;
            }
        }
        __threadfence();
        __syncthreads();
        __builtin_amdgcn_s_dcache_inv();
    }
#endif

#if FC_SPEC
    if (tid == 0) {
        Sh::SpecLocal &sl = sh.sl;
        sh.gap_lo = sh.gap_hi = 0; sh.gap_shift = 0; sh.deadmask = 0;
        sh.cap = F.spec ? F.spec_cap : F.P;
        sl.ctl = F.spec; sl.slots = F.spec ? SPEC_SLOTS(F.spec) : nullptr;
        sl.role = (int) role; sl.on = F.spec != nullptr && G > 1;
        sl.mode = role == 0 && sl.on ? 1 : 0;
        sl.T = F.spec_T; sl.tabs = F.spec ? (char *) F.spec + F.spec->off_tabs : nullptr;
        sl.chroma_tabs = 0;
        sl.n_tab_used = sl.n_tab_missed = sl.n_adopted = 0;
        sl.app_H = role == 0 && F.spec && G > 1 ? F.spec->app_H : 0u; sl.app_min = F.spec ? F.spec->app_min : 0u;
        sl.app_seq = 0; sl.app_off = 0; sl.n_app_dealt = sl.t_app_wait = 0;
        for (int k = 0; k < 32; k++) sl.rb_s[k] = 0;
        sh.blk = 0; sh.tab_shared = 0; sh.tab_from = 0;
        sl.floor = 0; sl.head = sl.commit = 0; sl.spec_mask = 0; sl.nospec = 0; sl.epoch = 0;
        sl.verdict = 0; sl.abort = 0; sl.ops = 0; sl.mlc = 0.0f; sl.nlc = 0; sl.learn = 0.0f;
        sl.n_tasks = sl.n_confirmed = sl.n_wrong = sl.n_timeout = sl.n_inline = sl.t_wait = 0;
        sl_keep = sl;
    }
    if (role == 0) {
#endif
    if (tid < 10 && tid >= 1)
        sh.m0tab[tid] = (float) -log2((double) (1 - 1 / (float) (1 << tid)));
    if (tid == 0) {
        const int ML = F.ML;
        static const unsigned c0[22] = {20,17,15,10,5,4,3,2,1,1,1,1,1,1,1,1,1,1,1,1,1,1};
        static const unsigned c1[22] = {1,1,1,1,1,1,1,1,1,2,3,5,10,15,20,25,30,35,60,60,60,60};
        sh.failed = 0;
        sh.cnt.bytes_mp = sh.cnt.bytes_img = sh.cnt.bytes_gram = 0;
        sh.cnt.n_mp = sh.cnt.n_steps = sh.cnt.n_blocks = sh.cnt.n_appends = sh.cnt.n_fulleval = 0;
        sh.cnt.t_mpA = sh.cnt.t_mpB = sh.cnt.n_blockevals = 0;
        F.trace_n = 0;
        for (int k = 0; k < 8; k++) F.dbg[k] = 0;
#ifdef FC_LATENCY_PROBE
        {
            volatile float *a = F.est;
            for (int k = 0; k < 64; k++) a[k] = (float) ((k * 7 + 3) & 63);
            __builtin_amdgcn_s_waitcnt(0);
            unsigned long long c0 = __builtin_readcyclecounter();
            int idx = 0;
            for (int k = 0; k < 64; k++) idx = (int) a[idx];
            unsigned long long c1 = __builtin_readcyclecounter();
            F.dbg[5] = (c1 - c0) / 64 + (idx & 0);
            c0 = __builtin_readcyclecounter();
            for (int k = 0; k < 64; k++) { a[64] = (float) k; idx += (int) a[64]; }
            c1 = __builtin_readcyclecounter();
            F.dbg[6] = (c1 - c0) / 64 + (idx & 0);
        }
#endif
#if FC_VARIANT_BIG
        if (F.bx) {
            const BxView V = bx_view(F);
            for (int s = 0; s < V.nb; s++) {
                F.final_d[s] = V.final_d[s];
                F.domain_type[s] = (uint8_t) V.dtype[s];
                F.level_of_state[s] = 0xff;
                for (int l = 0; l < 2; l++) { TREE(F, s, l) = RANGE_; INTO(F, s, l, 0) = NOEDGE; }
            }
        } else
#endif
        for (int s = 0; s < F.basis_states; s++) {
            F.final_d[s] = F.b_final[s];
            F.domain_type[s] = F.b_dtype[s];
            F.level_of_state[s] = 0xff;
            for (int l = 0; l < 2; l++) {
                TREE(F, s, l) = F.b_tree[s][l];
                for (int e = 0; e < 6; e++) {
                    INTO(F, s, l, e) = F.b_into[s][l][e];
                    WEIGHT(F, s, l, e) = F.b_weight[s][l][e];
                    if (F.b_into[s][l][e] == NOEDGE) break;
                }
            }
        }
        for (int w = 0; w < 2; w++)
            for (int l = 0; l < ML; l++) {
                int k = l < 22 ? l : 21;
                sh.tm[w * 2 * ML + l] = c1[k];
                sh.tm[w * 2 * ML + ML + l] = c0[k] + c1[k];
            }
        for (int i = 4 * ML; i < TM_WORDS; i++) sh.tm[i] = 0;
        Pool &m = sh.pool;
        m.total = 0;
        for (int i = 0; i <= MAXED; i++) { m.count[i] = 1; m.total++; }
        m.n = 0; m.max_domains = (unsigned short) F.pool_max; m.y_index = 0;
        m.d0_index = 0; m.d0_yindex = 0; m.d0_n = 0;
#if FC_GM
        sh.gm.pk[0] = F.gm_pool[0]; sh.gm.pk[1] = F.pred_on ? F.gm_pool[1] : FC_PK_CONSTANT;
        sh.gm.ck[0] = F.gm_coeff[0]; sh.gm.ck[1] = F.gm_coeff[1];
        sh.gm.qa = 0; sh.gm.gq = F.gq; sh.gm.P = F.P;
        sh.gm.base = sh.gm.kept = 0.0f; sh.gm.lg1 = 0.0;
        sh.dpool = m;
        for (int set = 0; set < 2; set++) {
            Pool &pm = set ? sh.dpool : sh.pool;
            const int k = sh.gm.pk[set];
            int maxd = F.pool_max ? F.pool_max : 1;
            if (k == FC_PK_BASIS) maxd = F.basis_states;
            if (k == FC_PK_UNIFORM || k == FC_PK_CONSTANT) maxd = 0xffff;
            pm.max_domains = (unsigned short) maxd;
            if (!GM_RLE(k)) { pm.total = 0; for (int i = 0; i <= MAXED; i++) pm.count[i] = 0; }
        }
        for (int s = 0; s < F.basis_states; s++) {
            F.pos[s] = -1;
            if (F.domain_type[s] & 2) gm_offer(F, sh, s);
        }
        if ((F.domain_type[0] & 2) && F.pos[0] < 0) { F.pos[0] = 0; F.pool_states[0] = 0; }
        if (sh.gm.pk[0] == FC_PK_CONSTANT) sh.pool.n = 1;
        if (sh.gm.pk[1] == FC_PK_CONSTANT) sh.dpool.n = 0;
#else
        for (int s = 0; s < F.basis_states; s++) {
            F.pos[s] = -1;
            if ((F.domain_type[s] & 2) && m.n < m.max_domains) {
                F.pos[s] = (short) m.n;
                F.pool_states[m.n++] = (short) s;
                if (s == 0) m.d0_n = 1;
            }
        }
#endif
        sh.n16 = (32 + 2 * F.coeff_size + 15) / 16;
#if FC_VARIANT_BIG
        if (F.pred_on && (32 + 2 * F.d_coeff_size + 15) / 16 > sh.n16) sh.n16 = (32 + 2 * F.d_coeff_size + 15) / 16;
        sh.nslot = F.pred_on ? 5 : 2;
        sh.snap = (F.pred_on || (F.level - F.lc_min + 3) * 2 * sh.n16 > SNAP_POOL16) && F.snap_hbm
                  ? (uint4 *) F.snap_hbm : sh.snap_pool;
        sh.snap_tm_p = F.pred_on && F.snap_hbm ? (uint4 *) F.snap_hbm + FC_DEPTH * 5 * FC_N16MAX : (uint4 *) sh.snap_tm;
        sh.pred_active = 0; sh.pred_lo = sh.pred_rec = 0;
#endif
        {
            const int depth_need = F.level - F.lc_min + 2
#if FC_VARIANT_BIG
                                   + (F.pred_on ? F.p_max - F.lc_min + 2 : 0)
#endif
                                   ;
#if FC_VARIANT_BIG
            const bool snap_lds = sh.snap == &sh.snap_pool[0];
            const bool tm_lds = (const void *) sh.snap_tm_p == (const void *) &sh.snap_tm[0];
#else
            const bool snap_lds = true, tm_lds = true;
#endif
#if FC_VARIANT_BIG
            const int snap_need = (F.level - F.lc_min + 3) * 2 * sh.n16;
#else
            const int snap_need = (F.level - F.lc_min + 3 + F.lc_max - F.lc_min) * sh.n16;
            sh.par.snap_b1 = (F.level - F.lc_min + 3) - (F.level - F.lc_max);
#endif
            if ((snap_lds && snap_need > SNAP_POOL16)
                || (tm_lds && (F.level - F.lc_min + 3) * 4 * TM_N16(ML) > SNAP_TM_WORDS) || F.coeff_nt > 16
                || (F.P + 63) / 64 > NBLOCKMIN
                || depth_need > FC_DEPTH
                || F.max_elements > FC_MAXE
                || (!FC_VARIANT_BIG && F.pred_on))
                sh.failed = FC_ERR_INTERNAL;
        }
        for (int i = 0; i < (FC_VARIANT_BIG ? FC_MAXCOEFF_BIG : FC_MAXCOEFF); i++) sh.cb.cnt[i] = 0;
        for (int i = 0; i < 16; i++) sh.cb.tot[i] = 0;
        for (int i = 0; i < F.coeff_size; i++) sh.cb.cnt[i] = 1;
        sh.cb.tot[0] = (short) F.dcs;
        for (int i = 1; i < F.coeff_nt; i++) sh.cb.tot[i] = (short) F.sy;
#if FC_VARIANT_BIG
        for (int i = 0; i < FC_MAXCOEFF_BIG; i++) sh.dcb.cnt[i] = 0;
        for (int i = 0; i < 16; i++) sh.dcb.tot[i] = 0;
        for (int i = 0; i < F.d_coeff_size; i++) sh.dcb.cnt[i] = 1;
        sh.dcb.tot[0] = (short) F.d_dcs;
        for (int i = 1; i < F.coeff_nt; i++) sh.dcb.tot[i] = (short) F.d_sy;
#if !FC_GM
        sh.dpool = sh.pool;
#endif
        sh.dq.rpf_mant = F.d_rpf_mant; sh.dq.dc_mant = F.d_dc_mant; sh.dq.sy = F.d_sy; sh.dq.dcs = F.d_dcs;
        sh.dq.rpf_range = F.d_rpf_range; sh.dq.dc_range = F.d_dc_range;
        sh.dq.half_nd = rtob_dev(0.5f, F.d_rpf_mant, F.d_rpf_range); sh.dq.half_dc = rtob_dev(0.5f, F.d_dc_mant, F.d_dc_range);
        if (F.pred_on && F.d_coeff_size > FC_MAXCOEFF_BIG) sh.failed = FC_ERR_INTERNAL;
#endif
#if FC_VARIANT_BIG
        if (F.bx) sh.states = F.basis_states;
        else
#else
        if (F.bx) sh.failed = FC_ERR_INTERNAL;
#endif
        basis_init(F, sh);
        sh.flim = 0;
        sh.par.lc_max = F.lc_max; sh.par.width = F.width; sh.par.height = F.height;
        sh.par.limit_states = F.limit_states; sh.par.PA = F.PA; sh.par.P = F.P; sh.par.ML = F.ML;
        sh.par.price = F.price; sh.par.chroma_decrease = F.chroma_decrease;
        sh.par.gram = F.gram; sh.par.gram_ls = F.gram_ls; sh.par.diag = F.diag; sh.par.ipis = F.ipis; sh.par.pos = F.pos;
        sh.par.gcol = F.gcol;
        sh.par.d5 = F.d5; sh.par.d4 = F.d4;
        sh.par.at_tree = F.tree; sh.par.at_into = F.into; sh.par.at_pool = F.pool_states; sh.par.at_weight = F.weight;
        sh.par.at_final = F.final_d; sh.par.at_los = F.level_of_state; sh.par.at_dtype = F.domain_type;
        sh.par.at_ycol = F.ycol; sh.par.at_x = F.x; sh.par.at_y = F.y; sh.par.color = F.color;
        sh.par.l2_keys = F.l2_keys; sh.par.l2_vals = F.l2_vals; sh.par.l2_mask = F.l2_mask;
        sh.par.max_elements = F.max_elements; sh.par.rpf_mant = F.rpf_mant; sh.par.dc_mant = F.dc_mant;
        sh.par.sy = F.sy; sh.par.dcs = F.dcs; sh.par.gl0 = F.gl0; sh.par.images_level = F.images_level;
        sh.par.lc_min_opt = F.lc_min; sh.par.trace_on = F.trace != nullptr;
        sh.par.rpf_range = F.rpf_range; sh.par.dc_range = F.dc_range;
        sh.par.half_nd = rtob_dev(0.5f, F.rpf_mant, F.rpf_range); sh.par.half_dc = rtob_dev(0.5f, F.dc_mant, F.dc_range);
        sh.band = 0; sh.lc_min = F.lc_min; sh.after_chroma = 0; sh.ystates = 0;
        push_root(F, sh, RANGE_);
        sh.op = OP_NOP;
    }
    if (F.color)
        for (int i = tid; i < 2 * F.PA; i += B) F.ycol[i] = F.ycol0 ? F.ycol0[i] : (uint8_t) 0;
#if FC_VARIANT_BIG
    if (F.bx) { __syncthreads(); basis_init_bx(F, sh); }
#endif
#if FC_SPEC
    }
#endif
    unsigned long long *tk = sh.tk;
    if (tid == 0) for (int k = 0; k < 16; k++) tk[k] = 0;
#ifdef FC_SERIAL_PROFILE
    if (tid == 0) { for (int k = 0; k < 8; k++) sh.tk_ph[k] = 0; sh.ph_prev = 0; sh.ph_t0 = 0; sh.tk_init[0] = sh.tk_init[1] = 0; for (int k = 0; k < 4; k++) sh.tk_apx[k] = 0; }
#endif
    unsigned long long t_begin = wall_clock64();
#if FC_SPEC
    const unsigned T = F.spec ? (unsigned) F.spec_T : 0u;
    if (role == 0 && F.spec && G > 1) {
        __threadfence();
        __syncthreads();
        if (tid == 0) __hip_atomic_store(&F.spec->s_pub, (unsigned) sh.states, __ATOMIC_RELEASE, __HIP_MEMORY_SCOPE_AGENT);
    }
    if (role >= 1 && role <= T) { spec_worker(F, sh, role, T, false); return; }
    for (;;) {
    if (role) {
        FcSpecCtl *const c = F.spec;
        __syncthreads();
        if (tid == 0) {
            unsigned t = atomicAdd(&c->next, 1u);
            int go = 1;
            for (;;) {
                const unsigned q = __hip_atomic_load(&c->slot_seq[t % FC_SPEC_W], __ATOMIC_RELAXED, __HIP_MEMORY_SCOPE_AGENT);
                if (q == t + 1) { take_acquire(); break; }
                if (q > t + 1) { t = atomicAdd(&c->next, 1u); continue; }
                if (__hip_atomic_load(&c->done, __ATOMIC_RELAXED, __HIP_MEMORY_SCOPE_AGENT)) { go = 0; break; }
                if (__hip_atomic_load(&c->chroma_ready, __ATOMIC_RELAXED, __HIP_MEMORY_SCOPE_AGENT)) { take_acquire(); go = 2; break; }
                __builtin_amdgcn_s_sleep(32);
            }
            task_seq = t; task_go = go;
        }
        __syncthreads();
        if (task_go != 1) break;
        {
            const uint4 *src = (const uint4 *) (SPEC_SLOTS(c) + (size_t) (task_seq % FC_SPEC_W) * SPEC_STRIDE);
            for (unsigned i = tid; i < sizeof(Sh) / 16; i += B) ((uint4 *) &sh)[i] = src[i];
        }
        __syncthreads();
        if (tid == 0) {
            const unsigned task_epoch = sh.sl.epoch;
            bool valid = __hip_atomic_load(&c->slot_seq[task_seq % FC_SPEC_W], __ATOMIC_ACQUIRE, __HIP_MEMORY_SCOPE_AGENT) == task_seq + 1
                         && __hip_atomic_load(&c->epoch, __ATOMIC_ACQUIRE, __HIP_MEMORY_SCOPE_AGENT) == task_epoch;
            sh.sl = sl_keep;
            sh.sl.epoch = task_epoch;
            const int S0 = sh.states, TB = F.spec_tb;
            if (valid && (S0 > TB || sh.sp < 0 || sh.sp >= FC_DEPTH)) valid = false;
            sh.sl.floor = sh.sp; sh.sl.verdict = 2; sh.sl.abort = valid ? 0 : 1; sh.sl.ops = 0; sh.sl.busy = 0;
            sh.sl.mode = 2 + sh.sp;
            if (sh.sp > 0) sh.st[sh.sp - 1].phase = PH_SPEC_END;
            sh.gap_lo = S0; sh.gap_hi = TB; sh.gap_shift = TB - S0; sh.states = TB; sh.cap = TB + FC_SPEC_TEMPS;
            unsigned dm = 0;
            for (int k = 0; k < 32; k++) if (k * B >= S0 && (k + 1) * B <= TB) dm |= 1u << k;
            sh.deadmask = dm;
            sh.par.at_pool = F.pool_states;
            sh.par.trace_on = 0;
            sh.par.color = 0;
            for (int k = 0; k < FC_SPEC_TEMPS; k++) F.level_of_state[TB + k] = 0;
            sh.op = valid ? OP_NOP : OP_DONE;
            if (valid) {
                atomicAdd(&c->busy, 1u);
                SPEC_DEKKER_FENCE();
                if (__hip_atomic_load(&c->epoch, __ATOMIC_ACQUIRE, __HIP_MEMORY_SCOPE_AGENT) != task_epoch) {
                    atomicSub(&c->busy, 1u); valid = false; sh.sl.abort = 1; sh.op = OP_DONE;
                } else sh.sl.busy = 1;
            }
            if (valid && !sh.tab_shared) {
                const Range &rg = sh.st[sh.sp].rg;
                sh.par.ipis = F.ipis; sh.par.d5 = F.d5;
                sh.op = OP_INIT_RANGE; sh.a0 = rg.x; sh.a1 = rg.y; sh.a2 = -1;
            }
        }
    }
#endif
    for (;;) {
        __syncthreads();
        const int op = sh.op;
        if (op == OP_DONE) break;
        unsigned long long t0 = wall_clock64();
#if FC_PRIO_ROTATE
        {
            const unsigned pr = ((unsigned) (t0 >> FC_PRIO_SHIFT) + (blockIdx.x >> 8)) & 3u;
            if (pr == 0) __builtin_amdgcn_s_setprio(0);
            else if (pr == 1) __builtin_amdgcn_s_setprio(1);
            else if (pr == 2) __builtin_amdgcn_s_setprio(2);
            else __builtin_amdgcn_s_setprio(3);
        }
#endif
        switch (op) {
#if FC_SPEC
        case OP_SPEC_CKPT: {
            FcSpecCtl *const c = sh.sl.ctl;
            if (tid == 0) {
                int act = 0;
                const int back = spec_poll(sh, sh.a0 == 2);
                if (back) {
                    act = (back & 0x100) ? 3 : 2; spec_slot = (unsigned) ((back & 0xff) - 1);
                    spec_used = (unsigned) (back >> 16) & 63u; spec_vid = (unsigned) (back >> 24) & 7u;
                    if (act == 3) {
                        __builtin_amdgcn_fence(__ATOMIC_ACQUIRE, "agent");
                        const Sh *im = (const Sh *) (sh.sl.slots + (size_t) (FC_SPEC_W + spec_vid) * SPEC_STRIDE);
                        const int TB = im->gap_hi, S0 = im->gap_lo, m = im->states - TB;
                        int bad = 0;
                        if (S0 != (int) sh.sl.sk[spec_slot]) bad |= 1;
                        if (TB < F.spec_cap || TB + FC_SPEC_TEMPS > F.P || ((TB - F.spec_cap) % FC_SPEC_TEMPS)) bad |= 2;
                        if (m < 0 || m > FC_SPEC_TEMPS || m > (int) spec_used) bad |= 4;
                        if (im->sp < 1 || im->sp >= FC_DEPTH) bad |= 8;
                        if (im->sl.epoch != sh.sl.epoch) bad |= 16;
                        if (S0 + m > F.spec_cap) bad |= 32;
                        if (im->sl.verdict != 3 || im->failed) bad |= 64;
                        if (bad) { spec_bad |= bad; act = 2; }
                    }
                }
                else if (sh.a0 == 1) {
                    SFrame &fr = sh.st[sh.sp];
                    if (!sh.sl.nospec && fr.rg.level > sh.lc_min) { fr.ckpt = 2; act = 1; }
                } else if (sh.par.color && !sh.band && !sh.after_chroma) spec_luminance_done(sh);
                else { sh.sl.on = 0; sh.sl.mode = 0; }
                spec_act = act;
            }
            __syncthreads();
            if (spec_act == 1) {
                const unsigned seq = sh.sl.head, slot = seq % FC_SPEC_W;
                if (tid == 0) __hip_atomic_store(&c->slot_seq[slot], 0u, __ATOMIC_RELAXED, __HIP_MEMORY_SCOPE_AGENT);
                WAVE_DRAIN();
                __syncthreads();
                uint4 *dst = (uint4 *) (sh.sl.slots + (size_t) slot * SPEC_STRIDE);
                for (unsigned i = tid; i < sizeof(Sh) / 16; i += B) dst[i] = ((const uint4 *) &sh)[i];
                WAVE_DRAIN();
                __syncthreads();
                if (tid == 0) {
                    publish_release();
                    __hip_atomic_store(&c->s_pub, (unsigned) sh.states, __ATOMIC_RELAXED, __HIP_MEMORY_SCOPE_AGENT);
                    __hip_atomic_store(&c->slot_seq[slot], seq + 1, __ATOMIC_RELAXED, __HIP_MEMORY_SCOPE_AGENT);
                    sh.sl.head = seq + 1; sh.sl.spec_mask &= ~(1u << slot); sh.sl.n_tasks++;
                    sh.sl.blkof[slot] = (unsigned) (sh.blk - 1);
                    sh.sl.sk[slot] = (unsigned) sh.states;
                }
            } else if (spec_act == 3) {
                if (tid == 0) sl_keep = sh.sl;
                __builtin_amdgcn_fence(__ATOMIC_ACQUIRE, "agent");
                __syncthreads();
                const uint4 *src = (const uint4 *) (sl_keep.slots + (size_t) (FC_SPEC_W + spec_vid) * SPEC_STRIDE);
                for (unsigned i = tid; i < sizeof(Sh) / 16; i += B) ((uint4 *) &sh)[i] = src[i];
                __syncthreads();
                const int TB = sh.gap_hi, S0 = sh.gap_lo, m = sh.states - TB, shift = TB - S0;
                __syncthreads();
                if (tid == 0) {
                    sh.sl = sl_keep;
                    sh.sl.nospec = 0;
                    sh.sl.commit = sh.sl.head;
                    sh.sl.rb_s[sh.sl.epoch % 32u] = (unsigned) S0;
                    __hip_atomic_store(&c->s_pub, (unsigned) S0, __ATOMIC_RELEASE, __HIP_MEMORY_SCOPE_AGENT);
                    __hip_atomic_store(&c->adopting, 1u, __ATOMIC_RELEASE, __HIP_MEMORY_SCOPE_AGENT);
                    sh.sl.epoch++;
                    __hip_atomic_store(&c->epoch, sh.sl.epoch, __ATOMIC_RELEASE, __HIP_MEMORY_SCOPE_AGENT);
                    SPEC_DEKKER_FENCE();
                    while (__hip_atomic_load(&c->busy, __ATOMIC_ACQUIRE, __HIP_MEMORY_SCOPE_AGENT)) __builtin_amdgcn_s_sleep(8);
                    sh.sl.n_adopted++;
                    sh.gap_lo = sh.gap_hi = sh.gap_shift = 0; sh.deadmask = 0;
                    sh.cap = F.spec_cap;
                    sh.states = S0 + m;
                    sh.par.at_pool = F.pool_states; sh.par.color = F.color; sh.par.trace_on = 0;
                    if (!sh.tab_shared) { sh.par.ipis = F.ipis; sh.par.d5 = F.d5; }
                    sh.st[sh.sp - 1].phase = PH_CHILD_RET;
                    SFrame &fr = sh.st[sh.sp];
                    fr.states = S0;
                    for (int l = 0; l < 2; l++) {
                        Range &ch = fr.child[l];
                        if (ch.tree >= TB) ch.tree -= shift;
                        for (int e = 0; e < RANGE_E; e++) if (ch.into[e] >= TB) ch.into[e] = (short) (ch.into[e] - shift);
                    }
                    if (F.color) {
                        GLOBAL_AS uint8_t *yc = (GLOBAL_AS uint8_t *) F.ycol;
                        for (unsigned j = 0; j < spec_used; j++) { yc[S0 + j] = 0; yc[(unsigned) F.PA + S0 + j] = 0; }
                    }
                }
                __syncthreads();
                __builtin_amdgcn_fence(__ATOMIC_ACQUIRE, "agent");
                for (int j = 0; j < m; j++) {
                    const int sid = TB + j, did = S0 + j;
                    if (tid < 2) {
                        const int l = tid;
                        const int t = TREE(F, sid, l);
                        TREE(F, did, l) = (short) (t >= TB ? t - shift : t);
                        for (int e = 0; e < 6; e++) {
                            const int d = INTO(F, sid, l, e);
                            INTO(F, did, l, e) = (short) (d >= TB ? d - shift : d);
                            WEIGHT(F, did, l, e) = WEIGHT(F, sid, l, e);
                        }
                        F.x[l * F.PA + did] = F.x[l * F.PA + sid]; F.y[l * F.PA + did] = F.y[l * F.PA + sid];
                    } else if (tid == 2) {
                        F.final_d[did] = F.final_d[sid]; F.level_of_state[did] = F.level_of_state[sid];
                        F.domain_type[did] = F.domain_type[sid];
                        const short p = F.pos[sid];
                        F.pos[did] = p;
                        if (p >= 0) F.pool_states[p] = (short) did;
                    }
                    if (!F.domain_type[sid]) continue;
                    for (int i = tid; i < F.NI; i += B) F.img[(size_t) did * F.NI + i] = F.img[(size_t) sid * F.NI + i];
                    if (tid < 32) F.imgT[(size_t) tid * F.P + did] = F.imgT[(size_t) tid * F.P + sid];
                    for (int q = 0; q < F.NL; q++) {
                        const float *Gs = GRAM(F, q) + GROW(sid, F.P);
                        float *Gd = GRAM(F, q) + GROW(did, F.P);
                        for (int t = tid; t < S0; t += B) Gd[t] = Gs[t];
                        if (tid <= j) Gd[S0 + tid] = Gs[TB + tid];
                        if (tid == 0) F.diag[(size_t) q * F.P + did] = F.diag[(size_t) q * F.P + sid];
                    }
                }
                __threadfence();
                __syncthreads();
                if (tid == 0)
                    __hip_atomic_store(&c->adopting, 0u, __ATOMIC_RELEASE, __HIP_MEMORY_SCOPE_AGENT);
            } else if (spec_act == 2) {
                const unsigned slot = spec_slot;
                if (tid == 0) sl_keep = sh.sl;
                __builtin_amdgcn_fence(__ATOMIC_ACQUIRE, "agent");
                __syncthreads();
                const uint4 *src = (const uint4 *) (sl_keep.slots + (size_t) slot * SPEC_STRIDE);
                for (unsigned i = tid; i < sizeof(Sh) / 16; i += B) ((uint4 *) &sh)[i] = src[i];
                __syncthreads();
                if (tid == 0) {
                    sh.sl = sl_keep;
                    sh.sl.nospec = 1;
                    sh.sl.commit = sh.sl.head;
                    sh.sl.rb_s[sh.sl.epoch % 32u] = (unsigned) sh.states;
                    __hip_atomic_store(&c->s_pub, (unsigned) sh.states, __ATOMIC_RELEASE, __HIP_MEMORY_SCOPE_AGENT);
                    sh.sl.epoch++;
                    __hip_atomic_store(&c->epoch, sh.sl.epoch, __ATOMIC_RELEASE, __HIP_MEMORY_SCOPE_AGENT);
                    SPEC_DEKKER_FENCE();
                    while (__hip_atomic_load(&c->busy, __ATOMIC_ACQUIRE, __HIP_MEMORY_SCOPE_AGENT)) __builtin_amdgcn_s_sleep(8);
                }
                __syncthreads();
                if (!sh.tab_shared) op_init_range(F, sh, sh.st[sh.sp].rg.x, sh.st[sh.sp].rg.y, 0);
                if (tid == 0 && sh.sl.n_timeout >= 3) { sh.sl.on = 0; sh.sl.mode = 0; }
            }
            break;
        }
#endif
#if FC_SPEC
        case OP_INIT_RANGE:
            if (((sh.sl.on && sh.sl.T > 0) || sh.sl.chroma_tabs) && sh.sl.role == 0 && sh.a2 >= 0) spec_tables(F, sh, sh.a2);
            else if (tid == 0) { sh.tab_from = 0; if (sh.sl.role == 0) { sh.par.ipis = F.ipis; sh.par.d5 = F.d5; sh.tab_shared = 0; } }
            __syncthreads();
            op_init_range(F, sh, sh.a0, sh.a1, sh.tab_from);
            break;
#else
        case OP_INIT_RANGE: op_init_range(F, sh, sh.a0, sh.a1, 0); FC_DUP(OP_INIT_RANGE, op_init_range(F, sh, sh.a0, sh.a1, 0)); break;
#endif
        case OP_APPROX:     op_approx(F, sh); break;
        case OP_IPIS_INCR:  op_ipis(F, sh, sh.a0, sh.a1, sh.a2, sh.a3); FC_DUP(OP_IPIS_INCR, op_ipis(F, sh, sh.a0, sh.a1, sh.a2, sh.a3)); break;
        case OP_APPEND:     op_append(F, sh, sh.a0); FC_DUP(OP_APPEND, op_append(F, sh, sh.a0)); break;
        case OP_CHROMA:
            op_chroma_pool(F, sh);
#if FC_SPEC
            if (sh.sl.chroma_tabs) {
                __threadfence();
                __syncthreads();
                if (tid == 0) {
                    FcSpecCtl *c = sh.sl.ctl;
                    c->ystates = (unsigned) sh.ystates;
                    __hip_atomic_store(&c->chroma_ready, 1u, __ATOMIC_RELEASE, __HIP_MEMORY_SCOPE_AGENT);
                }
            }
#endif
            break;
#if FC_VARIANT_BIG
        case OP_PRED_SETUP:  op_pred_setup(F, sh, sh.a0, sh.a1); break;
        case OP_PRED_FINISH: op_pred_finish(F, sh, sh.a0); break;
        case OP_NORMS:       op_norms(F, sh, sh.a0, sh.a1, sh.a2, sh.a3); break;
        case OP_MC_SEARCH:   op_mc_search(F, sh, sh.a0, sh.a1, sh.a2); break;
#endif
        default: break;
        }
        __syncthreads();
#if FC_SPEC
        if (tid == 0 && role && (++sh.sl.ops & 1u) == 0
            && __hip_atomic_load(&F.spec->epoch, __ATOMIC_RELAXED, __HIP_MEMORY_SCOPE_AGENT) != sh.sl.epoch) {
            sh.sl.abort = 1; sh.op = OP_DONE;
        } else
#endif
        if (tid == 0) {
            unsigned long long t1 = wall_clock64();
            tk[op] += t1 - t0;
#ifdef FC_SERIAL_PROFILE
            sh.ph_t0 = t1;
#endif
            serial_advance(F, sh);
#ifdef FC_SERIAL_PROFILE
            { unsigned long long t = wall_clock64(); sh.tk_ph[sh.ph_prev] += t - sh.ph_t0; }
#endif
            tk[0] += wall_clock64() - t1;
        }
    }
#if FC_SPEC
    if (!role) break;
    __syncthreads();
    if (tid == 0 && !sh.sl.abort
        && __hip_atomic_load(&F.spec->epoch, __ATOMIC_ACQUIRE, __HIP_MEMORY_SCOPE_AGENT) != sh.sl.epoch) sh.sl.abort = 1;
    __syncthreads();
    if (!sh.sl.abort && sh.sl.verdict == 3) {
        uint4 *dst = (uint4 *) (SPEC_SLOTS(F.spec) + (size_t) (FC_SPEC_W + (role - T - 1)) * SPEC_STRIDE);
        for (unsigned i = tid; i < sizeof(Sh) / 16; i += B) dst[i] = ((const uint4 *) &sh)[i];
        __threadfence();
        __syncthreads();
    }
    if (tid == 0) {
        if (!sh.sl.abort) {
            unsigned used = 0;
            while (used < FC_SPEC_TEMPS && F.level_of_state[sh.gap_hi + (int) used] != 0) used++;
            __hip_atomic_store(&F.spec->verdict[task_seq % FC_SPEC_W],
                               ((task_seq + 1) << 11) | ((role - T - 1) << 8) | (used << 2) | (unsigned) sh.sl.verdict,
                               __ATOMIC_RELEASE, __HIP_MEMORY_SCOPE_AGENT);
        }
        if (sh.sl.busy) { __threadfence(); atomicSub(&F.spec->busy, 1u); }
        if (!sh.sl.abort && sh.sl.verdict == 3) {
            while (__hip_atomic_load(&F.spec->epoch, __ATOMIC_ACQUIRE, __HIP_MEMORY_SCOPE_AGENT) == sh.sl.epoch
                   && __hip_atomic_load(&F.spec->committed, __ATOMIC_ACQUIRE, __HIP_MEMORY_SCOPE_AGENT) <= task_seq
                   && !__hip_atomic_load(&F.spec->done, __ATOMIC_ACQUIRE, __HIP_MEMORY_SCOPE_AGENT))
                __builtin_amdgcn_s_sleep(16);
            while (__hip_atomic_load(&F.spec->adopting, __ATOMIC_ACQUIRE, __HIP_MEMORY_SCOPE_AGENT)) __builtin_amdgcn_s_sleep(16);
        }
    }
    }
    if (role) {
        if (task_go == 2) spec_worker(F, sh, role, T, true);
        return;
    }
    if (tid == 0 && sh.sl.ctl && G > 1) {
        FcSpecCtl *const c = sh.sl.ctl;
        __hip_atomic_store(&c->epoch, sh.sl.epoch + 1, __ATOMIC_RELEASE, __HIP_MEMORY_SCOPE_AGENT);
        __hip_atomic_store(&c->done, 1u, __ATOMIC_RELEASE, __HIP_MEMORY_SCOPE_AGENT);
        c->n_tasks = sh.sl.n_tasks; c->n_confirmed = sh.sl.n_confirmed; c->n_wrong = sh.sl.n_wrong;
        c->n_timeout = sh.sl.n_timeout; c->n_inline = sh.sl.n_inline; c->t_wait = sh.sl.t_wait;
        c->n_tab_used = sh.sl.n_tab_used; c->n_tab_missed = sh.sl.n_tab_missed; c->n_adopted = sh.sl.n_adopted;
        c->n_app_dealt = sh.sl.n_app_dealt; c->t_app_wait = sh.sl.t_app_wait;
    }
#endif
    if (tid == 0) {
        F.t_serial = tk[0]; F.t_init = tk[OP_INIT_RANGE]; F.t_approx = tk[OP_APPROX];
        F.t_ipis = tk[OP_IPIS_INCR]; F.t_append = tk[OP_APPEND];
        F.t_total = wall_clock64() - t_begin;
        F.bytes_mp = sh.cnt.bytes_mp; F.bytes_img = sh.cnt.bytes_img; F.bytes_gram = sh.cnt.bytes_gram;
        F.n_mp = sh.cnt.n_mp; F.n_steps = sh.cnt.n_steps; F.n_blocks = sh.cnt.n_blocks;
        F.n_appends = sh.cnt.n_appends; F.n_fulleval = sh.cnt.n_fulleval;
        F.n_blockevals = sh.cnt.n_blockevals; F.t_mpA = sh.cnt.t_mpA; F.t_mpB = sh.cnt.t_mpB;
#if FC_VARIANT_BIG && !defined(FC_SERIAL_PROFILE)
        F.dbg[2] = tk[OP_CHROMA]; F.dbg[3] = tk[OP_PRED_SETUP]; F.dbg[4] = tk[OP_PRED_FINISH];
        F.dbg[5] = tk[OP_NORMS]; F.dbg[6] = tk[OP_MC_SEARCH];
#endif
#ifdef FC_SERIAL_PROFILE
        for (int k = 0; k < 8; k++) F.dbg[k] = sh.tk_ph[k];
        F.dbg[0] = sh.tk_init[0]; F.dbg[7] = sh.tk_init[1];
        F.dbg[3] = sh.tk_apx[0]; F.dbg[4] = sh.tk_apx[1]; F.dbg[5] = sh.tk_apx[2]; F.dbg[2] = sh.tk_apx[3];
#endif
    }
#if FC_SPEC && !defined(FC_SERIAL_PROFILE)
    if (tid == 0) { F.dbg[0] = tk[OP_SPEC_CKPT]; F.dbg[1] = 0; }
#endif
    if (tid == 0) {
#if FC_VARIANT_BIG && !FC_SPEC
        if (sh.coopW > 1 && F.coop) __hip_atomic_store(&F.coop->quit, 1u, __ATOMIC_RELAXED, __HIP_MEMORY_SCOPE_AGENT);
#endif
        F.states = sh.states;
        F.ystates_out = sh.band ? sh.ystates : sh.states;
        F.lc_min_out = sh.lc_min;
        F.status = sh.failed ? sh.failed : FC_OK;
#if FC_SPEC
        if (spec_bad) F.status = 128 + spec_bad;
#endif
    }
    if (F.pack_dst) {
        const uint4 *src = (const uint4 *) F.pack_src;
        uint4 *dst = (uint4 *) F.pack_dst;
        const unsigned n16 = F.pack_bytes / 16;
        for (unsigned i = tid; i < n16; i += B) dst[i] = src[i];
    }
#if !FC_SPEC
    if (ring) {
        __threadfence();
        __syncthreads();
        if (tid == 0) {
            const unsigned i = atomicAdd(&ctr[1], 1u);
            __hip_atomic_store(&ring[i], (unsigned long long) F.slab_base, __ATOMIC_RELEASE, __HIP_MEMORY_SCOPE_AGENT);
        }
    }
#endif
}

extern "C" int FC_OCCUPANCY(void)
{
    const int by_lds = (int) (163840 / sizeof(Sh));
    return by_lds < FC_WG_PER_CU ? (by_lds < 1 ? 1 : by_lds) : FC_WG_PER_CU;
}

#if FC_SPEC
extern "C" void FC_LAUNCH(DevFrame *d_frames, DevFrame *d_vframes, unsigned n, unsigned G, unsigned H, hipStream_t stream)
{
    hipLaunchKernelGGL(FC_KERNEL, dim3(n * (G + H)), dim3(B), 0, stream, d_frames, d_vframes, G, n, H);
}
extern "C" unsigned FC_SPEC_SLOT_BYTES(void) { return SPEC_STRIDE; }
#if !FC_VARIANT_WIDE
extern "C" unsigned fc_spec_ctl_bytes(void) { return (unsigned) ((sizeof(FcSpecCtl) + 255) / 256 * 256); }
#endif
#else
extern "C" void FC_LAUNCH(DevFrame *d_frames, unsigned n, unsigned nlend, unsigned long long *ring, unsigned *ctr,
                          const unsigned *ptrmask, unsigned long long queue_wait_ticks, unsigned coopW, hipStream_t stream)
{
    const unsigned grid = coopW > 1 ? (n + 7) / 8 * 8 * coopW : n;
    hipLaunchKernelGGL(FC_KERNEL, dim3(grid), dim3(B), 0, stream, d_frames, nlend, ring, ctr, ptrmask, queue_wait_ticks, coopW);
}
#endif
```

### fiasco_amd/csrc/hip/mp_device.inc

```

struct StepCtx {
    int      np;
    int      p[MAXED - 1];
    float    pre[MAXED];
    int      last[MAXED], k[MAXED], thr[MAXED];
    unsigned cd, has;
    float    sfx[MAXED - 1];
    float    z0, zy;
    int      ypos;
    float    wb_dc, wb_nd;
    float    ab, price, err;
    unsigned N;
};

__device__ __forceinline__ int   uni(int v)      { return __builtin_amdgcn_readfirstlane(v); }
__device__ __forceinline__ float unif(float v)   { return __int_as_float(__builtin_amdgcn_readfirstlane(__float_as_int(v))); }

__device__ __forceinline__ void load_step_ctx(const MPState &mp, StepCtx &c)
{
    c.np = uni(mp.np);
#pragma unroll
    for (int i = 0; i < MAXED - 1; i++) { c.p[i] = uni(mp.psorted[i]); c.sfx[i] = unif(mp.s1_sfx[i]); }
#pragma unroll
    for (int i = 0; i < MAXED; i++) {
// ... 194 lines not shown
#endif
        ev.m_bits = bits;
    }
    nov[NN] = den; ipio[NN] = num;
#pragma unroll
    for (int k = 0; k <= NN; k++)
#pragma unroll
        for (int l = 0; l <= NN; l++)
            if (l > k) r[k] += ipd[l][k] * r[l] / nov[k];
    float m_err = mp.norm;
#pragma unroll
    for (int k = 0; k <= NN; k++) m_err += r[k] * r[k] * nov[k] - 2 * r[k] * ipio[k];
    ev.m_err = m_err;
    ev.costs = (ev.m_bits + ev.w_bits + mp.ab) * mp.price + m_err;
#pragma unroll
    for (int k = 0; k < MAXED; k++) ev.f[k] = k <= NN ? f[k] : 0.0f;
}

template <int MAXN>
__device__ __forceinline__ void full_eval(const DevFrame &F, const Sh &sh, const MPState &mp, const double *lglv,
                                          int n, int d, int state,
                                          float num, float den, float ip0, float ip1, float ip2,
                                          float ip3, Eval &ev)
{
    if (n == 0) full_eval_n<0>(F, sh, mp, lglv, d, state, num, den, ip0, ip1, ip2, ip3, ev);
    else if (n == 1 && MAXN >= 1) full_eval_n<(MAXN >= 1 ? 1 : 0)>(F, sh, mp, lglv, d, state, num, den, ip0, ip1, ip2, ip3, ev);
    else if (n == 2 && MAXN >= 2) full_eval_n<(MAXN >= 2 ? 2 : 0)>(F, sh, mp, lglv, d, state, num, den, ip0, ip1, ip2, ip3, ev);
    else if (n == 3 && MAXN >= 3) full_eval_n<(MAXN >= 3 ? 3 : 0)>(F, sh, mp, lglv, d, state, num, den, ip0, ip1, ip2, ip3, ev);
    else if (MAXN >= 4) full_eval_n<(MAXN >= 4 ? 4 : 0)>(F, sh, mp, lglv, d, state, num, den, ip0, ip1, ip2, ip3, ev);
}

#if FC_HM
__device__ __noinline__ void mp_tables(const DevFrame &F, Sh &sh, int level, int y)
{
    const int tid = threadIdx.x;
    const int ctx = level - sh.par.lc_min_opt, dcs = sh.par.dcs, sy = sh.par.sy;
    const int nrole = dcs + sy + MAXED + 2;
    for (int t = tid; t < nrole; t += B) {
        const int r = t - dcs - sy;
        int ci, ti = 0;
        const bool coeff = r <= 0;
        if (t < dcs) ci = t;
        else if (r < 0) { ci = dcs + ctx * sy + t - dcs; ti = ctx + 1; }
        else if (r == 0) { ci = dcs + ctx * sy - 1; ti = ctx + 1; }
        else ci = r - 1;
        const float num = coeff ? (float) sh.cb.cnt[ci] : (float) sh.pool.count[ci];
        const float den = coeff ? (float) sh.cb.tot[ti] : (float) sh.pool.total;
        const double lg = log2((double) (num / den));
        if (t < dcs) sh.lgdc[t] = lg;
        else if (r < 0) sh.lglv[t - dcs] = lg;
        else if (r == 0) sh.lglv_m1 = lg;
        else sh.Ltab[ci] = (float) -lg;
    }
    __syncthreads();
    if (tid == 0) {
        const Pool &m = sh.pool;
        float q0 = 0, q1;
        if (m.d0_n && y != 0) q0 += sh.m0tab[qac_shift(m.d0_index)];
        if (y >= 0) q0 += sh.m0tab[qac_shift(m.d0_yindex)];
        q1 = q0;
        if (y == 0) { q1 -= sh.m0tab[qac_shift(m.d0_yindex)]; q1 += (float) qac_shift(m.d0_yindex); }
        else        { q1 -= sh.m0tab[qac_shift(m.d0_index)];  q1 += (float) qac_shift(m.d0_index); }
        sh.Q0 = q0; sh.Q1 = q1;
#if FC_GM
        {
            const int k = sh.gm.pk[0];
            sh.gm.base = 0.0f;
            if (GM_QAC(k)) {
                const int16_t *q = GQ_CUR(sh, 0), *list = F.pool_states;
                float bits = 0;
                for (int e = 0; e < (int) m.n; e++)
                    if (list[e] != y) bits += gm_m0(sh, q[e]);
                if (y >= 0) bits += gm_m0(sh, m.y_index);
                sh.gm.base = bits;
            } else if (k == FC_PK_UNIFORM) {
                const unsigned nn = m.n;
                sh.gm.base = (float) ((double) (0u - nn) * log2_host(sh, (float) (nn - 1) / (float) nn));
                sh.gm.lg1 = F.lginv[nn];
            }
        }
#endif
    }
}
#else
__device__ __noinline__ void mp_tables(const DevFrame &F, Sh &sh, int level, int y)
{
    const int tid = threadIdx.x;
    const int ctx = level - sh.par.lc_min_opt, dcs = sh.par.dcs, sy = sh.par.sy;
    const int om = 64 + sy + 12 <= 128 ? 64 + sy : 128;
    const int sl = (om + 12 <= 128 && B > 128) ? 128 : om + 11;
    if (tid == sl) {
        const Pool &m = sh.pool;
        float q0 = 0, q1;
        if (m.d0_n && y != 0) q0 += sh.m0tab[qac_shift(m.d0_index)];
        if (y >= 0) q0 += sh.m0tab[qac_shift(m.d0_yindex)];
        q1 = q0;
        if (y == 0) { q1 -= sh.m0tab[qac_shift(m.d0_yindex)]; q1 += (float) qac_shift(m.d0_yindex); }
        else        { q1 -= sh.m0tab[qac_shift(m.d0_index)];  q1 += (float) qac_shift(m.d0_index); }
        sh.Q0 = q0; sh.Q1 = q1;
#if !FC_VARIANT_BIG
        if (!sh.band) {
            MPState &mp = sh.mp;
            const unsigned N = (unsigned) sh.pool.n;
            mp.s1_last[0] = 1;
            const unsigned mv = N - 2u;
            if (mv != 0) {
                const unsigned kk = 31u - (unsigned) __clz((int) (mv + 1));
                const unsigned r = (mv + 1) - (1u << kk);
                mp.s1_cd = 1u; mp.s1_k[0] = (int) kk; mp.s1_thr[0] = (int) (mv + 1 - 2 * r);
            } else {
                mp.s1_cd = 0u; mp.s1_k[0] = 0; mp.s1_thr[0] = 0;
            }
            mp.s1_has = 0u;
            mp.np = 0;
        }
#endif
    }
    if (tid < om + 12) {
        int ci = 0, ti = 0, role = 0;
        const int r = tid - om;
        if (tid < dcs) { role = 1; ci = tid; ti = 0; }
        else if (tid >= 64 && tid < 64 + sy) { role = 1; ci = dcs + ctx * sy + tid - 64; ti = ctx + 1; }
        else if (r == 6) {
            role = 1; ci = dcs + ctx * sy - 1; ti = ctx + 1;
        }
        else if (r >= 0 && r < MAXED + 1) { role = 2; ci = r; }
#if !FC_VARIANT_BIG
        else if (r == 7 || r == 8) role = 3;
        else if (r == 9 && !sh.band) {
            role = 1; ci = dcs + ctx * sy + sh.par.half_nd; ti = ctx + 1;
        } else if (r == 10 && !sh.band) {
            role = 1; ci = sh.par.half_dc; ti = 0;
        }
#endif
        float num = 1.0f, den = 1.0f;
        if (role == 1)      { num = (float) sh.cb.cnt[ci]; den = (float) sh.cb.tot[ti]; }
        else if (role == 2) { num = (float) sh.pool.count[ci]; den = (float) sh.pool.total; }
#if !FC_VARIANT_BIG
        else if (role == 3) {
            const unsigned *counts = sh.tm;
            num = (float) counts[level]; den = (float) counts[sh.par.ML + level];
        }
#endif
        float p = num / den;
#if !FC_VARIANT_BIG
        if (r == 7) p = 1 - p;
#endif
        const double lg = log2((double) p);
        if (role == 1) {
            if (tid < dcs) sh.lgdc[tid] = lg;
            else if (r == 6) sh.lglv_m1 = lg;
#if !FC_VARIANT_BIG
            else if (r == 9) sh.mp.wb_nd = sub_log2(sh, 0.0f, lg, ci, ti);
            else if (r == 10) sh.mp.wb_dc = sub_log2(sh, 0.0f, lg, ci, ti);
#endif
            else sh.lglv[tid - 64] = lg;
        } else if (role == 2) sh.Ltab[ci] = (float) -lg;
#if !FC_VARIANT_BIG
        else if (role == 3) sh.tb[r - 7] = (float) -lg;
#endif
    }
}

#endif

__device__ void mp_step_prepare(const DevFrame &F, Sh &sh, MPState &mp, const double *lglv, double lglv_m1)
{
    float wb = 0;
    int np = 0;
    for (int k = 0; k < mp.n; k++)
        if (mp.weight[k] != 0) {
            const bool have = SYMP_HAS(mp.symp, k);
            if (mp.into[k]) {
                const int sym = have ? SYMP_GET(mp.symp, k) : rtob_dev(mp.weight[k], sh.par.rpf_mant, sh.par.rpf_range);
                {
                    const int ctx = mp.level - sh.par.lc_min_opt;
                    wb = sub_log2(sh, wb, sym >= 0 ? lglv[sym] : lglv_m1, sh.par.dcs + ctx * sh.par.sy + sym, ctx + 1);
                }
            }
            else {
                const int sym = have ? SYMP_GET(mp.symp, k) : rtob_dev(mp.weight[k], sh.par.dc_mant, sh.par.dc_range);
                wb = sym >= 0 ? sub_log2(sh, wb, sh.lgdc[sym], sym, 0)
                              : (float) ((double) wb + (double) INFINITY);
            }
            if (mp.indices[k] == mp.ypos) continue;
            int j = np++;
            while (j > 0 && mp.psorted[j - 1] > mp.indices[k]) { mp.psorted[j] = mp.psorted[j - 1]; j--; }
            mp.psorted[j] = mp.indices[k];
        }
    mp.np = np;
    {
        const unsigned N = (unsigned) mp.N;
        const short *p = mp.psorted;
        const bool p0zero = np > 0 && p[0] == 0;
        float e[MAXED];
        bool  ev[MAXED];
        for (int j = 0; j < np; j++) {
            if (j == 0) {
                ev[0] = p[0] != 0 && (N - 2) != 0;
                e[0] = ev[0] ? (float) bits_bin_code((unsigned) p[0] - 1, N - 2) : 0.0f;
            } else {
                ev[j] = (unsigned) p[j - 1] != N - 2;
                e[j] = ev[j] ? (float) bits_bin_code((unsigned) (p[j] - p[j - 1] - 1), N - 2 - (unsigned) p[j - 1]) : 0.0f;
            }
        }
        float b = sh.Ltab[np + 1];
        b += p0zero ? sh.Q1 : sh.Q0;
        unsigned cd = 0, has = 0;
        for (int i = 0; i <= np; i++) {
            mp.s1_pre[i] = b;
            unsigned last = i == 0 ? 1u : (unsigned) p[i - 1] + 1;
            unsigned mv = N - 1 - last;
            mp.s1_last[i] = (int) last;
            if (mv != 0) {
                unsigned kk = 31u - (unsigned) __clz((int) (mv + 1));
                unsigned r = (mv + 1) - (1u << kk);
                cd |= 1u << i;
                mp.s1_k[i] = (int) kk; mp.s1_thr[i] = (int) (mv + 1 - 2 * r);
            } else {
                mp.s1_k[i] = 0; mp.s1_thr[i] = 0;
            }
            if (i < np && ev[i]) b += e[i];
        }
        for (int j = 1; j < np; j++) { mp.s1_sfx[j] = e[j]; if (ev[j]) has |= 1u << j; }
        mp.s1_cd = cd; mp.s1_has = has;
        b = sh.Ltab[np + 1]; b += sh.Q1;
        for (int j = 0; j < np; j++) if (ev[j]) b += e[j];
        mp.s1_z0 = b;
        b = sh.Ltab[np]; b += p0zero ? sh.Q1 : sh.Q0;
        for (int j = 0; j < np; j++) if (ev[j]) b += e[j];
        mp.s1_zy = b;
    }
    {
        const int ctx = mp.level - sh.par.lc_min_opt;
        const int s_nd = sh.par.half_nd, s_dc = sh.par.half_dc;
        mp.wb_nd = sub_log2(sh, wb, lglv[s_nd], sh.par.dcs + ctx * sh.par.sy + s_nd, ctx + 1);
        mp.wb_dc = sub_log2(sh, wb, sh.lgdc[s_dc], s_dc, 0);
    }
#if FC_GM
    {
        const int k = sh.gm.pk[0];
        float b = sh.gm.base;
        if (GM_QAC(k)) {
            for (int i = 0; i < mp.n; i++)
                if (mp.weight[i] != 0) {
                    if (mp.indices[i] == mp.ypos) { b -= gm_m0(sh, sh.pool.y_index); b += gm_m1(sh.pool.y_index); }
// ... 12 lines not shown
            mp.wb_dc = w; mp.wb_dc += (float) (sh.par.dc_mant + 1);
        }
    }
#endif
#if FC_VARIANT_BIG
    mp.min_costs = F.full_search ? MAXCOSTS : mp.costs;
#else
    mp.min_costs = mp.costs;
#endif
}

__device__ void models_update(const DevFrame &F, Sh &sh, const short *indices, const short *into,
                              const float *weight, int level, int y, unsigned symp = SYMP_NONE)
{
    Pool &m = sh.pool;
    int state_0 = 0, state_y = 0, edge = 0;
#if FC_GM
    if (GM_QAC(sh.gm.pk[0])) {
        int16_t *q = GQ_CUR(sh, 0);
        const int16_t *list = F.pool_states;
        int used_y = 0, y_is_domain = y >= 0 && F.pos[y] >= 0 && F.pos[y] < (int) m.n;
        short nv[MAXED + 1], np_[MAXED + 1];
        int nu = 0;
        for (int e = 0; indices[e] != NOEDGE; e++) {
            const int p = indices[e];
            if (into[e] == y && y >= 0) {
                if (y_is_domain) { np_[nu] = (short) p; nv[nu] = q[p]; nu++; }
                m.y_index >>= 1;
                used_y = 1;
            } else { np_[nu] = (short) p; nv[nu] = (short) (q[p] >> 1); nu++; }
        }
        (void) list;
        for (int i = 0; i < ((int) m.n + 7) / 8; i++) {
            uint4 v = ((uint4 *) q)[i];
            unsigned *w = (unsigned *) &v;
            for (int j = 0; j < 4; j++) {
                unsigned lo = (w[j] & 0xffffu) + 1, hi = (w[j] >> 16) + 1;
                if (lo > 1020) lo = 1020;
                if (hi > 1020) hi = 1020;
                w[j] = lo | (hi << 16);
            }
            ((uint4 *) q)[i] = v;
        }
        for (int i = 0; i < nu; i++) q[np_[i]] = nv[i] > 1020 ? (short) 1020 : nv[i];
        if (y >= 0 && !used_y) m.y_index++;
        if (m.y_index > 1020) m.y_index = 1020;
    } else if (!GM_RLE(sh.gm.pk[0])) {
    } else {
#endif
    for (; indices[edge] != NOEDGE; edge++) {
        if (into[edge] == 0) state_0 = 1;
        else if (into[edge] == y) state_y = 1;
    }
    m.count[edge]++;
    m.total++;
    {
        int used_y = 0, y_is_domain = 0;
        if (m.d0_n) { m.d0_index++; if (y == 0) y_is_domain = 1; }
        if (state_0) {
            if (y == 0) { if (y_is_domain) m.d0_index--; m.d0_yindex >>= 1; used_y = 1; }
            else { m.d0_index--; m.d0_index >>= 1; }
        }
        if (y >= 0 && !used_y) m.d0_yindex++;
        if (m.d0_n && m.d0_index > 1020) m.d0_index = 1020;
        if (m.d0_yindex > 1020) m.d0_yindex = 1020;
    }
    if (state_y) m.y_index >>= 1; else m.y_index++;
    if (m.y_index > 1020) m.y_index = 1020;
#if FC_GM
    }
    if (sh.gm.ck[0] == FC_CK_UNIFORM) return;
#endif
    int ctx = level - sh.par.lc_min_opt;
    for (int e = 0; into[e] != NOEDGE; e++) {
        const bool have = SYMP_HAS(symp, e);
        if (into[e]) {
            sh.cb.cnt[sh.par.dcs + ctx * sh.par.sy + (have ? SYMP_GET(symp, e) : rtob_dev(weight[e], sh.par.rpf_mant, sh.par.rpf_range))]++;
            sh.cb.tot[ctx + 1]++;
        } else {
            sh.cb.cnt[have ? SYMP_GET(symp, e) : rtob_dev(weight[e], sh.par.dc_mant, sh.par.dc_range)]++;
            sh.cb.tot[0]++;
        }
    }
}

__device__ __forceinline__ float wave_min_l63(float v)
{
    asm volatile(
        "s_nop 1\n\t"
        "v_min_f32_dpp %0, %0, %0 row_shr:1 row_mask:0xf bank_mask:0xf\n\t"
        "s_nop 1\n\t"
        "v_min_f32_dpp %0, %0, %0 row_shr:2 row_mask:0xf bank_mask:0xf\n\t"
        "s_nop 1\n\t"
        "v_min_f32_dpp %0, %0, %0 row_shr:4 row_mask:0xf bank_mask:0xf\n\t"
        "s_nop 1\n\t"
        "v_min_f32_dpp %0, %0, %0 row_shr:8 row_mask:0xf bank_mask:0xf\n\t"
        "s_nop 1\n\t"
        "v_min_f32_dpp %0, %0, %0 row_bcast:15 row_mask:0xa bank_mask:0xf\n\t"
        "s_nop 1\n\t"
        "v_min_f32_dpp %0, %0, %0 row_bcast:31 row_mask:0xc bank_mask:0xf\n\t"
        "s_nop 1"
        : "+v"(v));
    return v;
}

__device__ __forceinline__ void wave_min4_l63(float &a, float &b, float &c, float &d)
{
#define MIN4_STEP(ctl)                                                     \
        "v_min_f32_dpp %0, %0, %0 " ctl "\n\t"                             \
        "v_min_f32_dpp %1, %1, %1 " ctl "\n\t"                             \
        "v_min_f32_dpp %2, %2, %2 " ctl "\n\t"                             \
        "v_min_f32_dpp %3, %3, %3 " ctl "\n\t"
    asm volatile(
        "s_nop 1\n\t"
        MIN4_STEP("row_shr:1 row_mask:0xf bank_mask:0xf")
        MIN4_STEP("row_shr:2 row_mask:0xf bank_mask:0xf")
        MIN4_STEP("row_shr:4 row_mask:0xf bank_mask:0xf")
        MIN4_STEP("row_shr:8 row_mask:0xf bank_mask:0xf")
        MIN4_STEP("row_bcast:15 row_mask:0xa bank_mask:0xf")
        MIN4_STEP("row_bcast:31 row_mask:0xc bank_mask:0xf")
        "s_nop 1"
        : "+v"(a), "+v"(b), "+v"(c), "+v"(d));
#undef MIN4_STEP
}

__device__ __forceinline__ float wave_min(float v)
{
    return __int_as_float(__builtin_amdgcn_readlane(__float_as_int(wave_min_l63(v)), 63));
}

#if FC_VARIANT_BIG
#define MP_NUMROW(F, mp)    ((mp).numrow)
__device__ __forceinline__ bool mp_excluded(const MPState &mp, int pos)
{
    bool x = false;
    bool live = true;
#pragma unroll
    for (int i = 0; i < MAXED; i++) {
        live = live && mp.excl[i] != NOEDGE;
        x = x || (live && mp.excl[i] == pos);
    }
    return x;
}
#define MP_EXCLUDED(mp, pos) mp_excluded(mp, pos)
#else
#define MP_NUMROW(F, mp)    (sh.par.ipis + (size_t) (mp).image * sh.par.P)
#define MP_EXCLUDED(mp, pos) false
#endif

__device__ __forceinline__ void lds_barrier()
{
    asm volatile("s_waitcnt lgkmcnt(0)\n\ts_barrier" ::: "memory");
}

#include "mp_reg.inc"

__device__ __noinline__ void mp_steps_global(DevFrame &F, Sh &sh, int q, float size)
{
    const int tid = threadIdx.x, lane = tid & 63, wave = tid >> 6, P = F.P;
    MPState &mp = sh.mp;
    const int S = sh.states;
    const int nblk = (S + 63) >> 6;
    constexpr int U = 4;
    unsigned long long tA = 0, tB = 0, tmark = wall_clock64();
    unsigned blockevals = 0;
    for (;;) {
        const int n = mp.n;
        {
            const float *Gq = GRAM(F, q);
            const int flim = sh.flim;
            const float *diag = F.diag + (size_t) q * P;
            const float *numrow = MP_NUMROW(F, mp);
            const int nv = n - 1;
            StepCtx ctx;
            load_step_ctx(mp, ctx);
            float novk[MAXED - 1], selk[MAXED - 1], nov_nv = 1, ipio_nv = 0;
#pragma unroll
            for (int k = 0; k < MAXED - 1; k++) {
                novk[k] = k < nv ? mp.norm_ov[k] : 1.0f;
                selk[k] = k < nv ? mp.sel_ipdo[nv < 0 ? 0 : nv][k] : 0.0f;
            }
            if (n) { nov_nv = mp.norm_ov[nv]; ipio_nv = mp.ipio[nv]; }
            for (int base = 0; base < nblk * 64; base += B * U) {
                int dd[U], ps[U];
                bool in[U], us[U];
                float num[U], den[U], g[U], ip[U][MAXED - 1], e[U];
#pragma unroll
                for (int u = 0; u < U; u++) {
                    dd[u] = base + u * B + tid;
                    ps[u] = dd[u] < S && !DEAD(sh, dd[u]) ? (int) F.pos[dd[u]] : -1;
                    in[u] = ps[u] >= 0;
                    us[u] = (in[u] && n) ? F.used[dd[u]] != 0 : !in[u];
                }
                if (n == 0) {
#pragma unroll
                    for (int u = 0; u < U; u++) {
                        den[u] = in[u] ? diag[dd[u]] : 1.0f;
                        num[u] = in[u] ? numrow[dd[u]] : 0.0f;
                    }
#pragma unroll
                    for (int u = 0; u < U; u++) {
                        if (!in[u]) continue;
                        bool uu = den[u] / size < MIN_NORM;
                        if (!uu) uu = fabsf(num[u]) < MIN_NORM;
                        if (MP_EXCLUDED(mp, ps[u])) uu = true;
                        us[u] = uu;
                        F.num[dd[u]] = num[u]; F.den[dd[u]] = den[u]; F.used[dd[u]] = uu;
                    }
                } else {
#pragma unroll
                    for (int u = 0; u < U; u++) {
                        bool on = !us[u];
                        num[u] = on ? F.num[dd[u]] : 0.0f;
                        den[u] = on ? F.den[dd[u]] : 1.0f;
                        g[u] = on ? gram_load(Gq, P, mp.row_state, dd[u], flim) : 0.0f;
#pragma unroll
                        for (int k = 0; k < MAXED - 1; k++)
                            ip[u][k] = (on && k < nv) ? F.ipdo[(size_t) k * P + dd[u]] : 0.0f;
                    }
#pragma unroll
                    for (int u = 0; u < U; u++) {
                        if (us[u]) continue;
                        float t = g[u];
#pragma unroll
                        for (int k = 0; k < MAXED - 1; k++)
                            if (k < nv) t -= ip[u][k] / novk[k] * selk[k];
                        F.ipdo[(size_t) nv * P + dd[u]] = t;
                        den[u] -= t * t / nov_nv;
                        num[u] -= ipio_nv / nov_nv * t;
                        if (den[u] / size < MIN_NORM) { us[u] = true; F.used[dd[u]] = 1; }
                        F.num[dd[u]] = num[u]; F.den[dd[u]] = den[u];
                    }
                }
#pragma unroll
                for (int u = 0; u < U; u++) {
                    e[u] = BIGF;
                    if (in[u] && !us[u]) e[u] = stage1<MAXED - 1>(ctx, ps[u], dd[u], num[u], den[u]);
                    if (dd[u] < S) F.est[dd[u]] = e[u];
                    float bm = wave_min(e[u]);
                    int blk = ((base + u * B) >> 6) + wave;
                    if (lane == 0 && blk < NBLOCKMIN) sh.blockmin[blk] = bm;
                }
            }
        }
        __syncthreads();
        if (tid == 0) { unsigned long long t = wall_clock64(); tA += t - tmark; tmark = t; }
        if (wave == 0) {
            float m = mp.min_costs;
            unsigned evals = 0;
            int b_state = -1;
            float b_cost = 0, b_mbits = 0, b_wbits = 0, b_err = 0, b_f[MAXED];
#pragma unroll
            for (int k = 0; k < MAXED; k++) b_f[k] = 0;
            for (int bb = 0; bb < nblk; bb += 64) {
                float bm = (bb + lane < nblk) ? sh.blockmin[bb + lane] : BIGF;
                int lastb = -1;
                for (;;) {
                    unsigned long long mask = __ballot(bm < m && lane > lastb);
                    if (!mask) break;
                    int jb = __ffsll((long long) mask) - 1;
                    lastb = jb;
                    int d = ((bb + jb) << 6) + lane;
                    float e = (d < S) ? F.est[d] : BIGF;
                    bool pass = e < m;
                    Eval ev;
                    ev.costs = BIGF; ev.m_bits = ev.w_bits = ev.m_err = 0;
#pragma unroll
                    for (int k = 0; k < MAXED; k++) ev.f[k] = 0;
                    if (pass) {
                        float i0 = n > 0 ? F.ipdo[d] : 0.0f, i1 = n > 1 ? F.ipdo[(size_t) P + d] : 0.0f;
                        float i2 = n > 2 ? F.ipdo[(size_t) 2 * P + d] : 0.0f, i3 = n > 3 ? F.ipdo[(size_t) 3 * P + d] : 0.0f;
                        full_eval<MAXED - 1>(F, sh, mp, sh.lglv, n, F.pos[d], d, F.num[d], F.den[d], i0, i1, i2, i3, ev);
                    }
                    evals += (unsigned) __popcll(__ballot(pass));
                    blockevals++;
                    int last = -1, win = -1;
                    for (;;) {
                        unsigned long long ok = __ballot(pass && lane > last && e < m && ev.costs < m);
                        if (!ok) break;
                        int j = __ffsll((long long) ok) - 1;
                        last = j; win = j;
                        m = __shfl(ev.costs, j);
                    }
                    if (win >= 0) {
                        b_state = ((bb + jb) << 6) + win;
                        b_cost = __shfl(ev.costs, win); b_mbits = __shfl(ev.m_bits, win);
                        b_wbits = __shfl(ev.w_bits, win); b_err = __shfl(ev.m_err, win);
#pragma unroll
                        for (int k = 0; k < MAXED; k++) b_f[k] = __shfl(ev.f[k], win);
                    }
                }
            }
            if (lane == 0) {
                sh.cnt.n_fulleval += evals;
                int index = b_state >= 0 ? (int) F.pos[b_state] : -1;
                if (index >= 0) {
                    if (b_cost < mp.costs) {
                        mp.costs = b_cost; mp.err = b_err;
                        mp.matrix_bits = b_mbits; mp.weights_bits = b_wbits;
#pragma unroll
                        for (int k = 0; k < MAXED; k++) if (k <= n) mp.weight[k] = b_f[k];
                        mp.symp = SYMP_NONE;
                        mp.best_n = n + 1;
                    }
                    mp.indices[n] = (short) index;
                    mp.into[n] = (short) b_state;
                    F.used[b_state] = 1;
                    mp.norm_ov[n] = F.den[b_state];
                    mp.ipio[n] = F.num[b_state];
#pragma unroll
                    for (int k = 0; k < MAXED - 1; k++)
                        if (k < n) mp.sel_ipdo[n][k] = F.ipdo[(size_t) k * P + b_state];
                    mp.row_state = b_state;
                    mp.n = n + 1;
                    if (mp.n < F.max_elements) mp_step_prepare(F, sh, mp, sh.lglv, sh.lglv_m1);
                }
                mp.index = index;
            }
        }
        __syncthreads();
        if (tid == 0) { unsigned long long t = wall_clock64(); tB += t - tmark; tmark = t; }
        if (!(mp.n < F.max_elements && mp.index >= 0)) break;
    }
    if (tid == 0) { sh.cnt.t_mpA += tA; sh.cnt.t_mpB += tB; sh.cnt.n_blockevals += blockevals; }
}

#if FC_VARIANT_BIG
__device__ __noinline__ void mp_steps_list_global(DevFrame &F, Sh &sh, int q, float size, int D)
{
    const int tid = threadIdx.x, lane = tid & 63, wave = tid >> 6, P = F.P;
    MPState &mp = sh.mp;
    const int16_t *const list = F.pool_states;
    const int nblk = (D + 63) >> 6;
    unsigned blockevals = 0;
    for (;;) {
        const int n = mp.n;
        {
            const float *Gq = GRAM(F, q);
            const int flim = sh.flim;
            const float *diag = F.diag + (size_t) q * P;
            const float *numrow = MP_NUMROW(F, mp);
            const int nv = n - 1;
            StepCtx ctx;
            load_step_ctx(mp, ctx);
            for (int base = 0; base < nblk * 64; base += B) {
                const int c = base + tid;
                const bool in = c < D;
                const int st = in ? (int) list[c] : 0;
                bool us = in ? (n ? F.used[c] != 0 : false) : true;
                float num = 0.0f, den = 1.0f;
                if (in && n == 0) {
                    den = diag[st]; num = numrow[st];
                    bool uu = den / size < MIN_NORM;
                    if (!uu) uu = fabsf(num) < MIN_NORM;
                    if (MP_EXCLUDED(mp, c)) uu = true;
                    us = uu;
                    F.num[c] = num; F.den[c] = den; F.used[c] = uu;
                } else if (!us) {
                    num = F.num[c]; den = F.den[c];
                    float t = gram_load(Gq, P, mp.row_state, st, flim);
                    for (int k = 0; k < MAXED - 1; k++)
                        if (k < nv) t -= F.ipdo[(size_t) k * P + c] / mp.norm_ov[k] * mp.sel_ipdo[nv][k];
                    F.ipdo[(size_t) nv * P + c] = t;
                    den -= t * t / mp.norm_ov[nv];
                    num -= mp.ipio[nv] / mp.norm_ov[nv] * t;
                    if (den / size < MIN_NORM) { us = true; F.used[c] = 1; }
                    F.num[c] = num; F.den[c] = den;
                }
                float e = BIGF;
#if FC_GM
                if (in && !us && !GM_RLE(sh.gm.pk[0])) {
                    const int pk = sh.gm.pk[0];
                    float bits = sh.gm.kept;
                    if (GM_QAC(pk)) {
                        const int qi = c == mp.ypos ? (int) sh.pool.y_index : (int) GQ_CUR(sh, 0)[c < (int) sh.pool.n ? c : 0];
                        bits -= gm_m0(sh, qi); bits += gm_m1(qi);
                    } else if (pk == FC_PK_UNIFORM) bits = (float) ((double) bits - sh.gm.lg1);
                    else bits = 0;
                    const float wbits = st ? ctx.wb_nd : ctx.wb_dc;
                    e = (bits + wbits + ctx.ab) * ctx.price + ctx.err - num * num / den;
                } else
#endif
                if (in && !us) e = stage1<MAXED - 1>(ctx, c, st, num, den);
                if (in) F.est[c] = e;
                const float bm = wave_min(e);
                const int blk = (base >> 6) + wave;
                if (lane == 0 && blk < NBLOCKMIN) sh.blockmin[blk] = bm;
            }
        }
        __syncthreads();
        if (wave == 0) {
            float m = mp.min_costs;
            unsigned evals = 0;
            int b_idx = -1;
            float b_cost = 0, b_mbits = 0, b_wbits = 0, b_err = 0, b_f[MAXED];
#pragma unroll
            for (int k = 0; k < MAXED; k++) b_f[k] = 0;
            for (int bb = 0; bb < nblk; bb += 64) {
                float bm = (bb + lane < nblk) ? sh.blockmin[bb + lane] : BIGF;
                int lastb = -1;
                for (;;) {
                    unsigned long long mask = __ballot(bm < m && lane > lastb);
                    if (!mask) break;
                    int jb = __ffsll((long long) mask) - 1;
                    lastb = jb;
                    const int c = ((bb + jb) << 6) + lane;
                    float e = (c < D) ? F.est[c] : BIGF;
                    bool pass = e < m;
                    Eval ev;
                    ev.costs = BIGF; ev.m_bits = ev.w_bits = ev.m_err = 0;
#pragma unroll
                    for (int k = 0; k < MAXED; k++) ev.f[k] = 0;
                    if (pass) {
                        float i0 = n > 0 ? F.ipdo[c] : 0.0f, i1 = n > 1 ? F.ipdo[(size_t) P + c] : 0.0f;
                        float i2 = n > 2 ? F.ipdo[(size_t) 2 * P + c] : 0.0f, i3 = n > 3 ? F.ipdo[(size_t) 3 * P + c] : 0.0f;
#if FC_GM
                        ev.qc = GM_QAC(sh.gm.pk[0]) && c < (int) sh.pool.n ? (int) GQ_CUR(sh, 0)[c] : 0;
#endif
                        full_eval<MAXED - 1>(F, sh, mp, sh.lglv, n, c, list[c], F.num[c], F.den[c], i0, i1, i2, i3, ev);
                    }
                    evals += (unsigned) __popcll(__ballot(pass));
                    blockevals++;
                    int last = -1, win = -1;
                    for (;;) {
                        unsigned long long ok = __ballot(pass && lane > last && e < m && ev.costs < m);
                        if (!ok) break;
                        int j = __ffsll((long long) ok) - 1;
                        last = j; win = j;
                        m = __shfl(ev.costs, j);
                    }
                    if (win >= 0) {
                        b_idx = ((bb + jb) << 6) + win;
                        b_cost = __shfl(ev.costs, win); b_mbits = __shfl(ev.m_bits, win);
                        b_wbits = __shfl(ev.w_bits, win); b_err = __shfl(ev.m_err, win);
#pragma unroll
                        for (int k = 0; k < MAXED; k++) b_f[k] = __shfl(ev.f[k], win);
                    }
                }
            }
            if (lane == 0) {
                sh.cnt.n_fulleval += evals;
                const int index = b_idx;
                if (index >= 0) {
                    const int b_state = list[index];
                    if (b_cost < mp.costs) {
                        mp.costs = b_cost; mp.err = b_err;
                        mp.matrix_bits = b_mbits; mp.weights_bits = b_wbits;
#pragma unroll
                        for (int k = 0; k < MAXED; k++) if (k <= n) mp.weight[k] = b_f[k];
                        mp.symp = SYMP_NONE;
                        mp.best_n = n + 1;
                    }
                    mp.indices[n] = (short) index;
                    mp.into[n] = (short) b_state;
#if FC_GM
                    mp.kq[n] = GM_QAC(sh.gm.pk[0]) && index < (int) sh.pool.n ? GQ_CUR(sh, 0)[index] : (short) 0;
#endif
                    F.used[index] = 1;
                    mp.norm_ov[n] = F.den[index];
                    mp.ipio[n] = F.num[index];
#pragma unroll
                    for (int k = 0; k < MAXED - 1; k++)
                        if (k < n) mp.sel_ipdo[n][k] = F.ipdo[(size_t) k * P + index];
                    mp.row_state = b_state;
                    mp.n = n + 1;
                    if (mp.n < F.max_elements) mp_step_prepare(F, sh, mp, sh.lglv, sh.lglv_m1);
                }
                mp.index = index;
            }
        }
        __syncthreads();
        if (!(mp.n < F.max_elements && mp.index >= 0)) break;
    }
    if (tid == 0) sh.cnt.n_blockevals += blockevals;
}
#endif

__device__ __noinline__ void mp_steps_chroma(DevFrame &F, Sh &sh, int q, float size, int D)
{
#if FC_VARIANT_BIG
    if (F.chroma_max > 63) { mp_steps_list_global(F, sh, q, size, D); return; }
#endif
    mp_steps_list<MAXED - 1>(F, sh, q, size, D);
}

__device__ __forceinline__ void op_approx(DevFrame &F, Sh &sh)
{
    const int tid = threadIdx.x, lane = tid & 63, wave = tid >> 6, P = sh.par.P;
    SFrame &fr = sh.st[sh.sp];
    MPState &mp = sh.mp;
    const int level = fr.lrange.level;
    const float size = (float) (1u << level);
    const int q = level - sh.par.gl0;
    const int D = sh.pool.n;
    int y = fr.y_state;
    if (y >= 0 && !(F.domain_type[y] & 2)) y = -1;

#ifdef FC_SERIAL_PROFILE
    unsigned long long tp = wall_clock64();
#define APX_MARK(i) do { if (tid == 0) { unsigned long long t_ = wall_clock64(); sh.tk_apx[i] += t_ - tp; tp = t_; } } while (0)
#else
#define APX_MARK(i) do { } while (0)
#endif
    if (fr.coop) snap_coop_before(sh, fr, sh.sp, sh.par.ML);
    mp_tables(F, sh, level, y);
    __syncthreads();
    APX_MARK(0);
    const int S = sh.states;
    const bool regscan = !sh.band && S <= KREG * B && sh.par.max_elements <= FC_NIP + 1;
    Step0 pre;
#if !FC_VARIANT_BIG
    if (regscan) mp_step0_issue(sh, q, sh.par.ipis + (size_t) fr.lrange.image * P, pre);
#endif
#if FC_VARIANT_BIG
    const bool retries = F.second_domain_block || F.check_underflow || F.check_overflow;
    if (tid == 0) {
        sh.apx_stage = 0; sh.apx_it = -1;
        mp.excl[0] = NOEDGE;
        for (int k = 0; k < MAXED; k++) mp.weight[k] = 0;
    }
#else
    const bool retries = false;
#endif
    for (;;) {
    if (tid == 0) {
        mp.n = 0; mp.best_n = 0; mp.symp = SYMP_NONE;
        mp.D = D; mp.N = D;
        mp.y_state = y; mp.ypos = -1;
        if (sh.band) {
            int ypos = -1;
#if FC_VARIANT_BIG
#if FC_GM
            if (sh.gm.pk[0] == FC_PK_UNIFORM || sh.gm.pk[0] == FC_PK_CONSTANT) {
            } else
#endif
            if (FC_GM || F.chroma_max > 63) {
                if (y >= 0) {
                    ypos = F.pos[y];
                    if (ypos < 0 || ypos >= D) { F.pool_states[D] = (short) y; ypos = D; mp.D = D + 1; }
                }
            } else
#endif
            if (y >= 0) {
                for (int i = 0; i < D; i++) if (sh.dl[i] == y) ypos = i;
                if (ypos < 0) { sh.dl[D] = (short) y; ypos = D; mp.D = D + 1; }
            }
            mp.ypos = ypos;
        }
        mp.level = level; mp.image = fr.lrange.image; mp.address = fr.lrange.address;
#if FC_VARIANT_BIG
        if (level > sh.par.images_level) {
            mp.norm = sh.norms[mp.image];
            mp.numrow = sh.par.ipis + (size_t) mp.image * P;
        } else {
            const int npx = 1 << level;
            const float *px = sh.pixels + mp.address * npx;
            float nrm = 0;
            for (int k = 0; k < npx; k++) nrm += px[k] * px[k];
            mp.norm = nrm;
            mp.numrow = (level == sh.par.images_level ? ACT_D5(F, sh) : ACT_D4(F, sh)) + (size_t) mp.address * P;
        }
#else
        mp.norm = sh.norms[mp.image];
#endif
#if FC_VARIANT_BIG
        mp.ab = fr.lrange.tree_bits + fr.lrange.mv_tree_bits + fr.lrange.mv_coord_bits + fr.lrange.nd_tree_bits
                + fr.lrange.nd_weights_bits;
#else
        fr.lrange.tree_bits = sh.tb[0];
        mp.ab = sh.tb[0];
#endif
        mp.price = fr.price;
        mp.err = mp.norm;
        mp.weights_bits = 0;
        mp.matrix_bits = sh.Ltab[0] + sh.Q0;
#if FC_GM
        if (!GM_RLE(sh.gm.pk[0])) mp.matrix_bits = sh.gm.pk[0] == FC_PK_CONSTANT ? 0.0f : sh.gm.base;
#endif
        mp.costs = (mp.matrix_bits + mp.weights_bits + mp.ab) * mp.price + mp.err;
        mp.index = -1;
#if FC_VARIANT_BIG
        mp_step_prepare(F, sh, mp, sh.lglv, sh.lglv_m1);
#else
        if (sh.band) mp_step_prepare(F, sh, mp, sh.lglv, sh.lglv_m1);
        else {
            const float L0 = sh.Ltab[0], L1 = sh.Ltab[1], q0 = sh.Q0, q1 = sh.Q1;
            float b = L1; b += q0; mp.s1_pre[0] = b;
            b = L1; b += q1; mp.s1_z0 = b;
            b = L0; b += q0; mp.s1_zy = b;
            mp.min_costs = mp.costs;
        }
#endif
    }
    lds_barrier();

    APX_MARK(1);
#if FC_GM
    if (true) {
        mp_steps_list_global(F, sh, q, size, mp.D);
    } else
#endif
    if (sh.band) {
        mp_steps_chroma(F, sh, q, size, mp.D);
    } else if (regscan) {
#if FC_VARIANT_BIG
        mp_step0_issue(sh, q, MP_NUMROW(F, mp), pre);
#endif
#if FC_VARIANT_BIG
        const int kslots = (sh.states + B - 1) / B;
        if (sh.par.max_elements <= 3) {
            if (kslots <= KREG / 4) mp_steps_reg<2, KREG / 4>(F, sh, q, size, pre);
            else if (kslots <= KREG / 2) mp_steps_reg<2, KREG / 2>(F, sh, q, size, pre);
            else mp_steps_reg<2>(F, sh, q, size, pre);
        } else if (kslots <= KREG / 4) mp_steps_reg<FC_NIP, KREG / 4>(F, sh, q, size, pre);
        else if (kslots <= KREG / 2) mp_steps_reg<FC_NIP, KREG / 2>(F, sh, q, size, pre);
        else
#endif
        mp_steps_reg<FC_NIP>(F, sh, q, size, pre);
    } else {
        mp_steps_global(F, sh, q, size);
    }
    APX_MARK(2);
    if (!retries) break;
#if FC_VARIANT_BIG
    __syncthreads();
    if (tid == 0) {
        MPState &best = sh.mp_keep;
        mp.indices[mp.best_n] = NOEDGE;
        mp.costs = (mp.matrix_bits + mp.weights_bits + mp.ab) * mp.price + mp.err;
        if (sh.apx_stage == 0) best = mp;
        else if (mp.costs < best.costs) best = mp;
        int more = 0;
        while (!more && sh.apx_stage < 4) {
            if (sh.apx_stage == 0) {
                sh.apx_stage = 1;
                if (F.second_domain_block && (best.indices[0] != NOEDGE || F.full_search)) {
                    mp.excl[0] = best.indices[0]; mp.excl[1] = NOEDGE;
                    more = 1;
                }
            } else if (sh.apx_stage == 1 || sh.apx_stage == 2) {
                const bool on = sh.apx_stage == 1 ? F.check_underflow != 0 : F.check_overflow != 0;
                if (!on) { sh.apx_stage++; sh.apx_it = -1; continue; }
                if (sh.apx_it < 0) mp = best;
                else if (!(sh.apx_it < MAXED - 1)) { sh.apx_stage++; sh.apx_it = -1; continue; }
                const int it = ++sh.apx_it;
                mp.excl[it] = NOEDGE;
                for (int i = 0; mp.indices[i] != NOEDGE; i++) {
                    bool hit;
                    if (sh.apx_stage == 1) hit = mp.weight[i] == 0;
                    else {
                        const int mant = mp.indices[i] ? sh.par.rpf_mant : sh.par.dc_mant;
                        const float range = mp.indices[i] ? sh.par.rpf_range : sh.par.dc_range;
                        hit = mp.weight[i] == btor_fast(rtob_dev(200.0f, mant, range), mant, range)
                              || mp.weight[i] == btor_fast(rtob_dev(-200.0f, mant, range), mant, range);
                    }
                    if (hit) { mp.excl[it] = mp.indices[i]; break; }
                }
                if (mp.excl[it] != NOEDGE) { mp.excl[it + 1] = NOEDGE; more = 1; }
                else { sh.apx_stage++; sh.apx_it = -1; }
            } else sh.apx_stage = 4;
        }
        if (!more) mp = best;
        sh.apx_more = more;
    }
    __syncthreads();
    if (!sh.apx_more) break;
#endif
    }

    if (tid == 0) {
        Range &lr = fr.lrange;
        mp.indices[mp.best_n] = NOEDGE;
        float costs = (mp.matrix_bits + mp.weights_bits + mp.ab) * mp.price + mp.err;
        if (costs < fr.max_costs) {
            int ni = 0;
            unsigned sp = 0;
            for (int oi = 0; mp.indices[oi] != NOEDGE; oi++)
                if (mp.weight[oi] != 0) {
                    mp.indices[ni] = mp.indices[oi]; mp.into[ni] = mp.into[oi];
                    mp.weight[ni] = mp.weight[oi];
                    if (oi < 3) sp |= ((mp.symp >> (10 * oi)) & 1023u) << (10 * ni);
                    ni++;
                }
            mp.indices[ni] = NOEDGE; mp.into[ni] = NOEDGE;
            models_update(F, sh, mp.indices, mp.into, mp.weight, level, mp.y_state, sp);
            int e = 0;
            for (; mp.indices[e] != NOEDGE; e++) { lr.into[e] = mp.into[e]; lr.weight[e] = mp.weight[e]; }
            lr.into[e] = NOEDGE;
            lr.matrix_bits = mp.matrix_bits; lr.weights_bits = mp.weights_bits; lr.err = mp.err;
        } else {
            lr.into[0] = NOEDGE;
            costs = MAXCOSTS;
        }
        fr.lincomb = costs;
#if FC_SPEC
        if (fr.ckpt == 2 && sh.sl.role == 0) {
            Sh::SpecLocal &sl = sh.sl;
            const unsigned slot = (sl.head - 1) % FC_SPEC_W;
            if (sl.nospec) { sl.nospec = 0; sl.n_inline++; }
            else if (costs < (sl.nlc >= 8 ? SPEC_THR * sl.mlc : MAXCOSTS) && !sh.failed) {
                sl.spec_mask |= 1u << slot;
                sl.lin[slot] = costs;
                fr.ckpt = 3;
            } else sl.n_inline++;
        }
#endif
        if (sh.par.trace_on && F.trace_n < F.trace_cap) {
            FcTrace &t = F.trace[F.trace_n];
            t.seq = F.trace_n; t.level = level; t.image = mp.image; t.D = D; t.states = sh.states;
            t.cost = costs; t.err = mp.err; t.mbits = mp.matrix_bits; t.wbits = mp.weights_bits;
            int e = 0;
            for (; e < 6; e++) { t.into[e] = -1; if (e < 5) t.w[e] = 0; }
            for (e = 0; costs < MAXCOSTS && lr.into[e] != NOEDGE; e++) { t.into[e] = lr.into[e]; t.w[e] = lr.weight[e]; }
            t.nedges = e;
            F.trace_n++;
        }
#if FC_VARIANT_BIG
        sh.cnt.bytes_mp += 4ull * D * (2 + mp.n) + 4ull * (1u << level);
        sh.cnt.n_mp++; sh.cnt.n_steps += mp.n;
#endif
    }
#if !FC_VARIANT_BIG
    else if (tid == 64) {
        sh.cnt.bytes_mp += 4ull * D * (2 + mp.n) + 4ull * (1u << level);
        sh.cnt.n_mp++; sh.cnt.n_steps += mp.n;
    }
#endif
    if (fr.coop) {
        __syncthreads();
        snap_coop_after(sh, fr, sh.sp);
    }
    APX_MARK(3);
#undef APX_MARK
}
```

### fiasco_amd/csrc/hip/mp_reg.inc

```

#define KREG FC_KREG
#define NWAVES (B / 64)

struct Step0 { unsigned praw[KREG]; float draw[KREG], nraw[KREG]; };

#if FC_SPEC
#define SPEC_DEADMASK(sh) const unsigned deadmask_ = (unsigned) __builtin_amdgcn_readfirstlane((int) (sh).deadmask);
#define SLOT_LIVE(k)      (!((deadmask_ >> (k)) & 1u))
#else
#define SPEC_DEADMASK(sh)
#define SLOT_LIVE(k)      true
#endif

__device__ __forceinline__ void mp_step0_issue(const Sh &sh, int q, const float *numrow, Step0 &o)
{
    unsigned utid = threadIdx.x;
    asm volatile("" : "+v"(utid));
    const int P = sh.par.P, S = sh.states, K = (S + B - 1) / B;
    const float *diag = sh.par.diag + (size_t) q * P;
    const unsigned short *pos = (const unsigned short *) sh.par.pos;
    SPEC_DEADMASK(sh)
#pragma unroll
    for (int k = 0; k < KREG; k++) {
        o.praw[k] = 0xffffu; o.draw[k] = 1.0f; o.nraw[k] = 0.0f;
        if (k < K && SLOT_LIVE(k)) {
            o.praw[k] = (pos + k * B)[utid];
            o.draw[k] = (diag + k * B)[utid];
            o.nraw[k] = (numrow + k * B)[utid];
        }
    }
}

template <int NIP, int KR = KREG>
__device__ __forceinline__ void mp_steps_reg(DevFrame &F, Sh &sh, int q, float size, const Step0 &pre)
{
    unsigned utid = threadIdx.x;
    asm volatile("" : "+v"(utid));
    const int tid = (int) utid, lane = tid & 63, wave = tid >> 6, P = sh.par.P;
    MPState &mp = sh.mp;
    RoundBox &rb = sh.rb;
    const int S = sh.states, K = (S + B - 1) / B, nblk = (S + 63) >> 6;
    const float rsize = 1.0f / size;
    SPEC_DEADMASK(sh)

    unsigned ps2[(KR + 1) / 2];
#define PS(k) ((int) (short) (ps2[(k) >> 1] >> (((k) & 1) * 16)))
    constexpr int NKEEP = NIP > 1 ? NIP - 1 : 1;
    float    num[KR], den[KR], ip[KR][NKEEP];
    unsigned usmask = 0;

#pragma unroll
    for (int k = 0; k < KR; k++) {
        const bool ok = k < K && k * B + tid < S && !DEAD(sh, k * B + tid);
        const unsigned pk = ok ? pre.praw[k] : 0xffffu;
        den[k] = ok ? pre.draw[k] : 1.0f;
        num[k] = ok ? pre.nraw[k] : 0.0f;
        if (k & 1) ps2[k >> 1] |= pk << 16; else ps2[k >> 1] = pk;
#pragma unroll
        for (int j = 0; j < NKEEP; j++) ip[k][j] = 0.0f;
    }
    if (tid == 0) { rb.evals = 0; rb.blockevals = 0; }
    unsigned long long tA = 0, tB = 0, tmark = wall_clock64();

    for (;;) {
        const int n = mp.n;
        StepCtx ctx;
        load_step_ctx(mp, ctx);
#pragma unroll
        for (int i = 0; i < (KR + 1) / 2; i++) asm volatile("" : "+v"(ps2[i]));
        if (n == 0) {
#pragma unroll
            for (int k = 0; k < KR; k++) {
                bool uu = PS(k) < 0 || MP_EXCLUDED(mp, PS(k));
                if (!uu) {
                    uu = den[k] * rsize < MIN_NORM;
                    if (!uu) uu = fabsf(num[k]) < MIN_NORM;
                }
                usmask |= uu ? (1u << k) : 0u;
            }
        } else {
            const int nv = n - 1, row = mp.row_state;
#if FC_GRAM_TRI
            const float *Gq = PGRAM(sh, q);
            float g[KR];
            if (tid == (row & (B - 1))) usmask |= 1u << (row / B);
            {
                const unsigned urow = (unsigned) row, rowoff = TRI(row), last = (unsigned) (S - 1);
                if (row < FC_TRI_HOT) {
                    const float *Cq = sh.par.gcol + ((size_t) q * FC_TRI_HOT + urow) * P;
#pragma unroll
                    for (int k = 0; k < KR; k++) {
                        g[k] = 0.0f;
                        if (k < K) {
                            unsigned d = (unsigned) (k * B) + utid;
                            d = d < last ? d : last;
                            g[k] = d <= urow ? Gq[rowoff + d] : Cq[d];
                        }
                    }
                } else {
#pragma unroll
                for (int k = 0; k < KR; k++) {
                    g[k] = 0.0f;
                    if (k < K) {
                        unsigned d = (unsigned) (k * B) + utid;
                        d = d < last ? d : last;
                        g[k] = Gq[d <= urow ? rowoff + d : TRI(d) + urow];
                    }
                }
                }
            }
#else
            const float *Grow = PGRAM(sh, q) + (size_t) row * P;
            float g[KR];
            if (tid == (row & (B - 1))) usmask |= 1u << (row / B);
#pragma unroll
            for (int k = 0; k < KR; k++) {
                g[k] = 0.0f;
                if (k < K && SLOT_LIVE(k)) g[k] = (Grow + k * B)[utid];
            }
            {
                const int flim = sh.flim;
                if (S > flim && S - 1 > row) {
                    const float *Gcol = PGRAM(sh, q) + row;
// ... 30 lines not shown
                if (den[k] * rsize < MIN_NORM) usmask |= 1u << k;
            }
        }
#define EST_ONE(NPV, k, ek)                                                                      \
        float ek = BIGF;                                                                         \
        if ((k) < K && !((usmask >> (k)) & 1u))                                                  \
            ek = stage1<NIP, NPV, true>(ctx, PS(k), (k) * B + tid, num[k], den[k]);
#define EST_PASS(NPV)                                                                            \
        _Pragma("unroll")                                                                        \
        for (int k4 = 0; k4 + 4 <= KR; k4 += 4) {                                              \
            if (k4 < K) {                                       \
                EST_ONE(NPV, k4, e0) EST_ONE(NPV, k4 + 1, e1) EST_ONE(NPV, k4 + 2, e2) EST_ONE(NPV, k4 + 3, e3) \
                wave_min4_l63(e0, e1, e2, e3);                                                   \
                if (lane == 63) {                                                                \
                    sh.blockmin[NWAVES * k4 + wave] = e0;                                        \
                    if (k4 + 1 < K) sh.blockmin[NWAVES * (k4 + 1) + wave] = e1;                  \
                    if (k4 + 2 < K) sh.blockmin[NWAVES * (k4 + 2) + wave] = e2;                  \
                    if (k4 + 3 < K) sh.blockmin[NWAVES * (k4 + 3) + wave] = e3;                  \
                }                                                                                \
            }                                                                                    \
        }                                                                                        \
        _Pragma("unroll")                                                                        \
        for (int k = KR / 4 * 4; k < KR; k++) {                                              \
            if (k < K) {                                                                         \
                EST_ONE(NPV, k, ek)                                                              \
                ek = wave_min_l63(ek);                                                           \
                if (lane == 63) sh.blockmin[NWAVES * k + wave] = ek;                             \
            }                                                                                    \
        }
        if (ctx.np == 0)      { EST_PASS(0) }
        else if (ctx.np == 1) { EST_PASS(1) }
        else                  { EST_PASS(-1) }
#undef EST_PASS
#undef EST_ONE
        if (tid == 0) { rb.m2[1] = mp.min_costs; rb.state = -1; }
        __syncthreads();
        if (tid == 0) { unsigned long long t = wall_clock64(); tA += t - tmark; tmark = t; }

        float m = rb.m2[1];
        int round = 0;
        int cursor = -1;
        for (;;) {
            int jb = -1;
            for (int bb = 0; bb < nblk && jb < 0; bb += 64) {
                float bmv = (bb + lane < nblk) ? sh.blockmin[bb + lane] : BIGF;
                unsigned long long mask = __ballot(bmv < m && bb + lane > cursor);
                if (mask) jb = bb + __ffsll((long long) mask) - 1;
            }
            if (jb < 0) break;
            cursor = jb;
            if (jb % NWAVES == wave) {
                const int kk = jb / NWAVES;
                float numk = 0, denk = 1, ipk[NIP];
                int psk = -1;
#pragma unroll
                for (int j = 0; j < NIP; j++) ipk[j] = 0;
#pragma unroll
                for (int k = 0; k < KR; k++)
                    if (k == kk) {
                        numk = num[k]; denk = den[k]; psk = PS(k);
#pragma unroll
                        for (int j = 0; j < NIP - 1; j++) ipk[j] = ip[k][j];
                    }
                const int state = kk * B + tid;
                if (n == NIP) {
                    const int nv = NIP - 1;
                    float t = 0.0f;
                    if (!((usmask >> kk) & 1u)) {
                        t = gram_load(PGRAM(sh, q), P, mp.row_state, state, sh.flim);
#pragma unroll
                        for (int j = 0; j < NIP - 1; j++)
                            if (j < nv) t -= ipk[j] / mp.norm_ov[j] * mp.sel_ipdo[nv][j];
                    }
                    ipk[NIP - 1] = t;
                }
                const float ek = ((usmask >> kk) & 1u) ? BIGF : stage1<NIP>(ctx, psk, state, numk, denk);
                bool pass = ek < m;
                Eval ev;
                ev.costs = BIGF; ev.m_bits = ev.w_bits = ev.m_err = 0; ev.symp = SYMP_NONE;
#pragma unroll
                for (int k = 0; k < MAXED; k++) ev.f[k] = 0;
                const float i0 = ipk[0], i1 = NIP > 1 ? ipk[1 % NIP] : 0.0f;
                const float i2 = NIP > 2 ? ipk[2 % NIP] : 0.0f, i3 = NIP > 3 ? ipk[3 % NIP] : 0.0f;
                if (pass) full_eval<NIP>(F, sh, mp, sh.lglv, n, psk, state, numk, denk, i0, i1, i2, i3, ev);
                unsigned npass = (unsigned) __popcll(__ballot(pass));
                int last = -1, win = -1;
                for (;;) {
                    unsigned long long ok = __ballot(pass && lane > last && ek < m && ev.costs < m);
                    if (!ok) break;
                    int j = __ffsll((long long) ok) - 1;
                    last = j; win = j;
                    m = __shfl(ev.costs, j);
                }
                if (lane == win) {
                    rb.state = state; rb.idx = psk;
                    rb.cost = ev.costs; rb.mbits = ev.m_bits; rb.wbits = ev.w_bits;
                    rb.err = ev.m_err; rb.symp = ev.symp;
#pragma unroll
                    for (int k = 0; k < MAXED; k++) rb.f[k] = ev.f[k];
                    rb.num = numk; rb.den = denk;
#pragma unroll
                    for (int j = 0; j < MAXED - 1; j++) rb.ip[j] = j < NIP ? ipk[j % NIP] : 0.0f;
                }
                if (lane == 0) { rb.m2[round & 1] = m; rb.evals += npass; rb.blockevals++; }
            }
            __syncthreads();
            m = rb.m2[round & 1];
            round++;
        }
        if (tid == 0) {
            const int bstate = rb.state;
            int index = bstate >= 0 ? rb.idx : -1;
            if (index >= 0) {
                if (rb.cost < mp.costs) {
                    mp.costs = rb.cost; mp.err = rb.err;
                    mp.matrix_bits = rb.mbits; mp.weights_bits = rb.wbits;
#pragma unroll
                    for (int k = 0; k < MAXED; k++) if (k <= n) mp.weight[k] = rb.f[k];
                    mp.symp = rb.symp;
                    mp.best_n = n + 1;
                }
                mp.indices[n] = (short) index;
                mp.into[n] = (short) bstate;
                mp.norm_ov[n] = rb.den;
                mp.ipio[n] = rb.num;
#pragma unroll
                for (int k = 0; k < MAXED - 1; k++) if (k < n) mp.sel_ipdo[n][k] = rb.ip[k];
                mp.row_state = bstate;
                mp.n = n + 1;
                if (mp.n < sh.par.max_elements) mp_step_prepare(F, sh, mp, sh.lglv, sh.lglv_m1);
            }
            mp.index = index;
        }
        __syncthreads();
        if (tid == 0) { unsigned long long t = wall_clock64(); tB += t - tmark; tmark = t; }
        if (!(mp.n < sh.par.max_elements && mp.index >= 0)) break;
    }
    if (tid == 0) {
        sh.cnt.n_fulleval += rb.evals; sh.cnt.n_blockevals += rb.blockevals;
        sh.cnt.t_mpA += tA; sh.cnt.t_mpB += tB;
    }
}
#undef PS

template <int NIP>
__device__ __forceinline__ void mp_steps_list(DevFrame &F, Sh &sh, int q, float size, int D)
{
    const int tid = threadIdx.x, P = sh.par.P;
    MPState &mp = sh.mp;
    RoundBox &rb = sh.rb;
    const bool ok = tid < D;
    const int st = ok ? (int) sh.dl[tid] : 0;
    float den = ok ? sh.par.diag[(size_t) q * P + st] : 1.0f;
    float num = ok ? MP_NUMROW(F, mp)[st] : 0.0f;
    float ip[NIP];
#pragma unroll
    for (int j = 0; j < NIP; j++) ip[j] = 0.0f;
    bool used = !ok;
    unsigned evals = 0, steps = 0;

    for (;;) {
        const int n = mp.n;
        StepCtx ctx;
        load_step_ctx(mp, ctx);
        if (n == 0) {
            if (ok) {
                bool uu = den / size < MIN_NORM;
                if (!uu) uu = fabsf(num) < MIN_NORM;
                used = uu || MP_EXCLUDED(mp, tid);
            }
        } else {
            const int nv = n - 1;
            if (tid == (int) mp.indices[nv]) used = true;
            if (!used) {
                float t = gram_load(PGRAM(sh, q), P, mp.row_state, st, sh.flim);
#pragma unroll
                for (int j = 0; j < NIP; j++)
                    if (j < nv) t -= ip[j] / mp.norm_ov[j] * mp.sel_ipdo[nv][j];
#pragma unroll
                for (int j = 0; j < NIP; j++)
                    if (j == nv) ip[j] = t;
                den -= t * t / mp.norm_ov[nv];
                num -= mp.ipio[nv] / mp.norm_ov[nv] * t;
                if (den / size < MIN_NORM) used = true;
            }
        }
        if (tid < 64) {
            const int lane = tid;
            float e = used ? BIGF : stage1<NIP>(ctx, tid, st, num, den);
            float m = mp.min_costs;
            bool pass = e < m;
            Eval ev;
            ev.costs = BIGF; ev.m_bits = ev.w_bits = ev.m_err = 0; ev.symp = SYMP_NONE;
#pragma unroll
            for (int k = 0; k < MAXED; k++) ev.f[k] = 0;
            if (pass)
                full_eval<NIP>(F, sh, mp, sh.lglv, n, tid, st, num, den, ip[0], NIP > 1 ? ip[1 % NIP] : 0.0f,
                          NIP > 2 ? ip[2 % NIP] : 0.0f, NIP > 3 ? ip[3 % NIP] : 0.0f, ev);
            evals += (unsigned) __popcll(__ballot(pass));
            int last = -1, win = -1;
            for (;;) {
                unsigned long long okm = __ballot(pass && lane > last && e < m && ev.costs < m);
                if (!okm) break;
                int j = __ffsll((long long) okm) - 1;
                last = j; win = j;
                m = __shfl(ev.costs, j);
            }
            if (lane == 0) rb.state = -1;
            if (lane == win) {
                rb.state = st; rb.idx = tid;
                rb.cost = ev.costs; rb.mbits = ev.m_bits; rb.wbits = ev.w_bits; rb.err = ev.m_err; rb.symp = ev.symp;
#pragma unroll
                for (int k = 0; k < MAXED; k++) rb.f[k] = ev.f[k];
                rb.num = num; rb.den = den;
#pragma unroll
                for (int j = 0; j < MAXED - 1; j++) rb.ip[j] = j < NIP ? ip[j % NIP] : 0.0f;
            }
        }
        __syncthreads();
        if (tid == 0) {
            const int bstate = rb.state;
            const int index = bstate >= 0 ? rb.idx : -1;
            if (index >= 0) {
                if (rb.cost < mp.costs) {
                    mp.costs = rb.cost; mp.err = rb.err;
                    mp.matrix_bits = rb.mbits; mp.weights_bits = rb.wbits;
#pragma unroll
                    for (int k = 0; k < MAXED; k++) if (k <= n) mp.weight[k] = rb.f[k];
                    mp.symp = rb.symp;
                    mp.best_n = n + 1;
                }
                mp.indices[n] = (short) index;
                mp.into[n] = (short) bstate;
                mp.norm_ov[n] = rb.den;
                mp.ipio[n] = rb.num;
#pragma unroll
                for (int k = 0; k < MAXED - 1; k++) if (k < n) mp.sel_ipdo[n][k] = rb.ip[k];
                mp.row_state = bstate;
                mp.n = n + 1;
                if (mp.n < sh.par.max_elements) mp_step_prepare(F, sh, mp, sh.lglv, sh.lglv_m1);
            }
            mp.index = index;
        }
        steps++;
        __syncthreads();
        if (!(mp.n < sh.par.max_elements && mp.index >= 0)) break;
    }
    if (tid == 0) { sh.cnt.n_fulleval += evals; sh.cnt.n_blockevals += steps; }
}
```

### include/libfiasco_amd_hip.h

```cpp
#ifndef LIBFIASCO_AMD_HIP_H
#define LIBFIASCO_AMD_HIP_H 1
#include <stddef.h>
#include <stdint.h>
#include "libfiasco_amd.h"
#ifdef __cplusplus
extern "C" {
#endif

typedef struct fiasco_amd_stats {
    double             kernel_ms;
    unsigned long long launches;
    unsigned long long frames;
    unsigned long long bytes_mp, bytes_img, bytes_gram;
    unsigned long long n_mp, n_steps, n_blocks, n_appends, n_fulleval;
    unsigned long long t_init, t_approx, t_ipis, t_append, t_serial, t_total;
    unsigned long long t_mpA, t_mpB, n_blockevals;
    unsigned long long dbg[8];
    unsigned long long states_sum, states_max, reencodes;
    unsigned long long frames_by_build[5];
    unsigned long long spec_frames, spec_tasks, spec_confirmed, spec_wrong, spec_timeout, spec_inline, spec_wait;
    unsigned long long spec_tab_used, spec_tab_missed;
    unsigned long long spec_adopted;
    unsigned long long decoder_frames, decoder_bytes, decoder_us;
    unsigned long long coop_frames, coop_workgroups;
    unsigned long long spec_app_rows, spec_app_wait;
} fiasco_amd_stats;

void fiasco_amd_get_stats(fiasco_amd_stats *out);
void fiasco_amd_reset_stats(void);

int fiasco_amd_spec_workgroups(unsigned frames, int cus, int big_frames, int narrow_only, int occupancy);

const char *fiasco_amd_core_name(void);

int fiasco_amd_rccl_gather(void *comm, void *stream, int rank, int world, int root,
                           unsigned n_local, const unsigned char *const *data, const size_t *len,
                           unsigned char ***all, size_t **all_len, unsigned *n_all);

unsigned fiasco_amd_coop_workgroups(unsigned frames, int cus);
int fiasco_amd_spec_append_helpers(unsigned frames, int cus, int G, int wide_build);
unsigned fiasco_amd_share_of(unsigned share_key, unsigned index, unsigned shares);
int fiasco_amd_set_device(int device);
int fiasco_amd_set_devices(const int *ids, int n);
int fiasco_amd_device_count(void);

enum { FIASCO_AMD_GRAY8 = 0, FIASCO_AMD_RGB8_INTERLEAVED = 1, FIASCO_AMD_RGB8_PLANAR = 2 };
typedef struct fiasco_amd_device_frame {
    const void *data;
    size_t pitch;
    size_t plane_stride;
    unsigned width, height;
    int layout;
} fiasco_amd_device_frame;

fiasco_amd_batch_t *fiasco_amd_batch_stage_device(unsigned n, const fiasco_amd_device_frame *frames,
                                                  void *stream, float quality, const fiasco_c_options_t *options);
int fiasco_amd_batch_upload_device(fiasco_amd_batch_t *b, const fiasco_amd_device_frame *frames, void *stream);
int fiasco_amd_batch_input_planes(const fiasco_amd_batch_t *b, unsigned i, int16_t *out);

void fiasco_amd_release_memory(void);

int fiasco_amd_selftest_log2(unsigned exp_lo, unsigned exp_hi, unsigned long long *n_checked,
                             unsigned long long *n_double, unsigned long long *n_float,
                             float *first_bad);

unsigned long long fiasco_amd_selftest_log2_max_ulp(void);
int fiasco_amd_selftest_log2_patched(unsigned exp_lo, unsigned exp_hi, unsigned long long *n_checked,
                                     unsigned long long *n_double, unsigned long long *n_entries);

#ifdef __cplusplus
}
#endif
#endif
```

Measured before the change: 603.6.

## Cache per-level probability log tables across MP calls using model version counters

Adds a model version counter that is bumped whenever the adaptive coding models change (counts updated, pool appended, state restored, speculation reset). In the non-big variant, mp_tables now builds log2 probability tables for all levels at once and skips rebuilding when the version is unchanged and the requested level is already covered. Consumers index per-level slices of the cached tables. This removes repeated per-call table construction, which includes double-precision log2, at the cost of more LDS and a larger first build, plus the risk of stale tables if any model mutation misses a version bump.

New measurement: 601.9. Within noise of the previous version (-0.3%).

```diff
diff --git a/fiasco_amd/__init__.py b/fiasco_amd/__init__.py
--- a/fiasco_amd/__init__.py
+++ b/fiasco_amd/__init__.py
@@ -65,7 +65,8 @@
                 ("decoder_frames", ctypes.c_ulonglong), ("decoder_bytes", ctypes.c_ulonglong),
                 ("decoder_us", ctypes.c_ulonglong), ("coop_frames", ctypes.c_ulonglong),
                 ("coop_workgroups", ctypes.c_ulonglong),
-                ("spec_app_rows", ctypes.c_ulonglong), ("spec_app_wait", ctypes.c_ulonglong)]
+                ("spec_app_rows", ctypes.c_ulonglong), ("spec_app_wait", ctypes.c_ulonglong),
+                ("tables_built", ctypes.c_ulonglong), ("tables_reused", ctypes.c_ulonglong)]
 
 
 def build(verbose=False):
diff --git a/fiasco_amd/csrc/hip/core_hip.cpp b/fiasco_amd/csrc/hip/core_hip.cpp
--- a/fiasco_amd/csrc/hip/core_hip.cpp
+++ b/fiasco_amd/csrc/hip/core_hip.cpp
@@ -847,6 +847,10 @@
     F.color = job->image->color ? 1 : 0;
     F.chroma_cl_cap = (int) knob_int("FIASCO_AMD_CLMAX", 0);
     F.chroma_sparse = !fa_knob("FIASCO_AMD_CHROMA_FULL") && (cp->pool_kind == FA_POOL_RLE || cp->pool_kind == FA_POOL_ADAPTIVE || cp->pool_kind == FA_POOL_BASIS);
+    {
+        const char *e = fa_knob("FIASCO_AMD_TABLE_REUSE");
+        F.table_reuse = !(e && strcmp(e, "0") == 0);
+    }
     F.chroma_max = (int) cp->chroma_max_states;
     F.chroma_decrease = cp->chroma_decrease;
     F.plane = (unsigned long long) job->image->width * job->image->height;
@@ -1444,6 +1448,7 @@
     g_stats.t_init += F.t_init; g_stats.t_approx += F.t_approx; g_stats.t_ipis += F.t_ipis;
     g_stats.t_append += F.t_append; g_stats.t_serial += F.t_serial; g_stats.t_total += F.t_total;
     g_stats.t_mpA += F.t_mpA; g_stats.t_mpB += F.t_mpB; g_stats.n_blockevals += F.n_blockevals;
+    g_stats.tables_built += F.n_tab_built; g_stats.tables_reused += F.n_tab_reused;
     for (int k = 0; k < 8; k++) g_stats.dbg[k] += F.dbg[k];
     g_stats.states_sum += ns;
     if (ns > g_stats.states_max) g_stats.states_max = ns;
diff --git a/fiasco_amd/csrc/hip/fc_lds.inc b/fiasco_amd/csrc/hip/fc_lds.inc
--- a/fiasco_amd/csrc/hip/fc_lds.inc
+++ b/fiasco_amd/csrc/hip/fc_lds.inc
@@ -24,6 +24,9 @@
     Pool  pool0, pool_lc;
     float max_costs, lincomb, subdiv, ret, price;
     int   label, states, phase, leaf, coop;
+#if !FC_VARIANT_BIG
+    unsigned ver0, ver_lc;
+#endif
     int   y_state, ny[2];
 #if FC_GM
     int   rn0;
@@ -81,6 +84,11 @@
 #define NBLOCKMIN   64
 #endif
 #define TM_WORDS    (4 * 26 + 8)
+#if !FC_VARIANT_BIG
+#define FC_TAB_NL    5
+#define FC_TAB_LANES 192
+#define FC_TAB_LV    (FC_TAB_LANES - 64 - (MAXED + 1) - 5 * FC_TAB_NL + 1)
+#endif
 
 struct RoundBox {
     float m2[2];
@@ -125,10 +133,21 @@
     __attribute__((aligned(16))) unsigned tm[TM_WORDS];
     __attribute__((aligned(16))) unsigned snap_tm[SNAP_TM_WORDS];
     float    m0tab[12];
+#if FC_VARIANT_BIG
     double   lgdc[FC_MAXSYM], lglv[FC_MAXSYM], lglv_m1;
     float    Ltab[MAXED + 1];
     float    Q0, Q1;
-    float    tb[2];
+#else
+    double   lgdc[FC_MAXSYM], lglv[FC_TAB_LV], lglv_m1[FC_TAB_NL];
+    float    Ltab[MAXED + 1];
+    float    Q0, Q1;
+    float    tb[FC_TAB_NL][2];
+    float    wbp[FC_TAB_NL][2];
+    int      tab_all;
+    int      tab_top;
+    int      lv, lv_off;
+    unsigned model_ver, ver_next, tab_ver;
+#endif
     MPState  mp;
 #if FC_VARIANT_BIG
     MPState  mp_keep;
@@ -140,7 +159,7 @@
     unsigned long long tk[16];
     struct {
         unsigned long long bytes_mp, bytes_img, bytes_gram, n_mp, n_steps, n_blocks, n_appends,
-                           n_fulleval, n_blockevals, t_mpA, t_mpB;
+                           n_fulleval, n_blockevals, t_mpA, t_mpB, tables_built, tables_reused;
     } cnt;
 #ifdef FC_SERIAL_PROFILE
     unsigned long long tk_ph[8], ph_t0, tk_init[2], tk_apx[4];
@@ -164,6 +183,7 @@
         const unsigned *l2_keys; const double *l2_vals; unsigned l2_mask;
         int max_elements, rpf_mant, dc_mant, sy, dcs, gl0, images_level, lc_min_opt, trace_on;
         int snap_b1;
+        int tab_reuse;
         int16_t *at_tree, *at_into, *at_pool; float *at_weight, *at_final; uint8_t *at_los, *at_dtype, *at_ycol;
         uint16_t *at_x, *at_y; int color;
         float rpf_range, dc_range;
diff --git a/fiasco_amd/csrc/hip/fc_models.inc b/fiasco_amd/csrc/hip/fc_models.inc
--- a/fiasco_amd/csrc/hip/fc_models.inc
+++ b/fiasco_amd/csrc/hip/fc_models.inc
@@ -95,7 +95,12 @@
     if (tid < sh.n16) SNAP_AT(sh, depth, 0)[tid] = ((const uint4 *) &sh.cb)[tid];
     else if (tid >= 96 && tid < 96 + TM_N16(ML))
         TM_AT(sh, depth, 0, ML)[tid - 96] = ((const uint4 *) sh.tm)[tid - 96];
-    else if (tid == 128) fr.pool0 = sh.pool;
+    else if (tid == 128) {
+        fr.pool0 = sh.pool;
+#if !FC_VARIANT_BIG
+        fr.ver0 = sh.model_ver;
+#endif
+    }
 #if FC_VARIANT_BIG
     else if (sh.nslot == 5 && !fr.delta) {
         if (tid == 129) fr.dpool0 = sh.dpool;
@@ -133,6 +138,9 @@
 #endif
         fr.pool_lc = sh.pool;
         sh.pool = fr.pool0;
+#if !FC_VARIANT_BIG
+        fr.ver_lc = sh.model_ver; sh.model_ver = fr.ver0;
+#endif
 #if FC_GM
         if (fr.delta) sh.dpool.n = (unsigned short) fr.rn0;
 #endif
diff --git a/fiasco_amd/csrc/hip/fc_serial.inc b/fiasco_amd/csrc/hip/fc_serial.inc
--- a/fiasco_amd/csrc/hip/fc_serial.inc
+++ b/fiasco_amd/csrc/hip/fc_serial.inc
@@ -12,6 +12,9 @@
     unsigned *counts = sh.tm + which * 2 * ML;
     if (child) counts[level]++;
     counts[ML + level]++;
+#if !FC_VARIANT_BIG
+    sh.model_ver = ++sh.ver_next;
+#endif
 }
 
 __device__ __forceinline__ void copy16(uint4 *dst, const uint4 *src, int n)
@@ -281,6 +284,9 @@
     }
     sh.after_chroma = 0;
     sh.op = OP_NOP;
+#if !FC_VARIANT_BIG
+    sh.model_ver = ++sh.ver_next;
+#endif
     push_root(F, sh, sh.tree_band[0]);
     return 1;
 }
@@ -430,6 +436,9 @@
                 fr.pool0 = sh.pool;
                 snap_save(F, sh, sp, 0);
                 tm_save(sh, sp, ML);
+#if !FC_VARIANT_BIG
+                fr.ver0 = sh.model_ver;
+#endif
 #if FC_GM
                 fr.rn0 = sh.dpool.n;
                 gq_save(sh, 0, sp, 0);
@@ -488,6 +497,7 @@
 #endif
 #else
                 fr.pool_lc = sh.pool;
+                fr.ver_lc = sh.model_ver;
 #endif
             }
 #if FC_SPEC
@@ -511,7 +521,7 @@
 #if FC_VARIANT_BIG
                 fr.rrange.tree_bits = tree_bits_dev(sh, ML, 1, rg.level, 0);
 #else
-                fr.rrange.tree_bits = rg.level <= sh.par.lc_max ? sh.tb[1] : tree_bits_dev(sh, ML, 1, rg.level, 0);
+                fr.rrange.tree_bits = rg.level <= sh.par.lc_max ? sh.tb[sh.lv][1] : tree_bits_dev(sh, ML, 1, rg.level, 0);
 #endif
                 fr.rrange.matrix_bits = 0;
                 fr.rrange.weights_bits = 0;
@@ -637,6 +647,9 @@
                 sh.pool = fr.pool0;
                 snap_load(F, sh, sp, 0);
                 tm_load(sh, sp, ML);
+#if !FC_VARIANT_BIG
+                sh.model_ver = fr.ver0;
+#endif
 #if FC_GM
                 gq_load(sh, 0, sp, 0);
                 if (fr.delta) sh.dpool.n = (unsigned short) fr.rn0;
@@ -660,6 +673,9 @@
                 sh.pool = fr.pool_lc;
                 snap_load(F, sh, sp, 1);
                 tm_load(sh, sp, ML);
+#if !FC_VARIANT_BIG
+                sh.model_ver = fr.ver_lc;
+#endif
 #if FC_GM
                 gq_load(sh, 0, sp, 1);
                 if (fr.delta) sh.dpool.n = (unsigned short) fr.rn0;
diff --git a/fiasco_amd/csrc/hip/frame_coder.h b/fiasco_amd/csrc/hip/frame_coder.h
--- a/fiasco_amd/csrc/hip/frame_coder.h
+++ b/fiasco_amd/csrc/hip/frame_coder.h
@@ -72,6 +72,7 @@
     int      color;
     int      chroma_sparse;
     int      chroma_cl_cap;
+    int      table_reuse;
     int      chroma_max;
     float    chroma_decrease;
     unsigned long long plane;
@@ -138,6 +139,7 @@
     unsigned long long n_mp, n_steps, n_blocks, n_appends, n_fulleval;
     unsigned long long t_init, t_approx, t_ipis, t_append, t_serial, t_total;
     unsigned long long t_mpA, t_mpB, n_blockevals;
+    unsigned long long n_tab_built, n_tab_reused;
     unsigned long long dbg[8];
     struct FcTrace *trace;
     int      trace_cap, trace_n;
diff --git a/fiasco_amd/csrc/hip/frame_coder.hip b/fiasco_amd/csrc/hip/frame_coder.hip
--- a/fiasco_amd/csrc/hip/frame_coder.hip
+++ b/fiasco_amd/csrc/hip/frame_coder.hip
@@ -208,6 +208,7 @@
         sh.cnt.bytes_mp = sh.cnt.bytes_img = sh.cnt.bytes_gram = 0;
         sh.cnt.n_mp = sh.cnt.n_steps = sh.cnt.n_blocks = sh.cnt.n_appends = sh.cnt.n_fulleval = 0;
         sh.cnt.t_mpA = sh.cnt.t_mpB = sh.cnt.n_blockevals = 0;
+        sh.cnt.tables_built = sh.cnt.tables_reused = 0;
         F.trace_n = 0;
         for (int k = 0; k < 8; k++) F.dbg[k] = 0;
 #ifdef FC_LATENCY_PROBE
@@ -372,6 +373,16 @@
         sh.par.rpf_range = F.rpf_range; sh.par.dc_range = F.dc_range;
         sh.par.half_nd = rtob_dev(0.5f, F.rpf_mant, F.rpf_range); sh.par.half_dc = rtob_dev(0.5f, F.dc_mant, F.dc_range);
         sh.band = 0; sh.lc_min = F.lc_min; sh.after_chroma = 0; sh.ystates = 0;
+#if !FC_VARIANT_BIG
+        {
+            const int nl = F.lc_max - F.lc_min + 1;
+            sh.tab_all = nl >= 1 && nl <= FC_TAB_NL && nl * F.sy <= FC_TAB_LV
+                         && 64 + nl * F.sy + MAXED + 1 + 5 * nl <= FC_TAB_LANES;
+            sh.par.tab_reuse = F.table_reuse;
+            sh.lv = 0; sh.lv_off = 0; sh.tab_top = 0;
+            sh.ver_next = 1; sh.model_ver = 1; sh.tab_ver = 0;
+        }
+#endif
         push_root(F, sh, RANGE_);
         sh.op = OP_NOP;
     }
@@ -427,6 +438,7 @@
                          && __hip_atomic_load(&c->epoch, __ATOMIC_ACQUIRE, __HIP_MEMORY_SCOPE_AGENT) == task_epoch;
             sh.sl = sl_keep;
             sh.sl.epoch = task_epoch;
+            sh.model_ver = ++sh.ver_next; sh.tab_ver = 0;
             const int S0 = sh.states, TB = F.spec_tb;
             if (valid && (S0 > TB || sh.sp < 0 || sh.sp >= FC_DEPTH)) valid = false;
             sh.sl.floor = sh.sp; sh.sl.verdict = 2; sh.sl.abort = valid ? 0 : 1; sh.sl.ops = 0; sh.sl.busy = 0;
@@ -532,6 +544,7 @@
                 if (tid == 0) {
                     sh.sl = sl_keep;
                     sh.sl.nospec = 0;
+                    sh.model_ver = ++sh.ver_next; sh.tab_ver = 0;
                     sh.sl.commit = sh.sl.head;
                     sh.sl.rb_s[sh.sl.epoch % 32u] = (unsigned) S0;
                     __hip_atomic_store(&c->s_pub, (unsigned) S0, __ATOMIC_RELEASE, __HIP_MEMORY_SCOPE_AGENT);
@@ -606,6 +619,7 @@
                 if (tid == 0) {
                     sh.sl = sl_keep;
                     sh.sl.nospec = 1;
+                    sh.model_ver = ++sh.ver_next; sh.tab_ver = 0;
                     sh.sl.commit = sh.sl.head;
                     sh.sl.rb_s[sh.sl.epoch % 32u] = (unsigned) sh.states;
                     __hip_atomic_store(&c->s_pub, (unsigned) sh.states, __ATOMIC_RELEASE, __HIP_MEMORY_SCOPE_AGENT);
@@ -728,6 +742,7 @@
         F.n_mp = sh.cnt.n_mp; F.n_steps = sh.cnt.n_steps; F.n_blocks = sh.cnt.n_blocks;
         F.n_appends = sh.cnt.n_appends; F.n_fulleval = sh.cnt.n_fulleval;
         F.n_blockevals = sh.cnt.n_blockevals; F.t_mpA = sh.cnt.t_mpA; F.t_mpB = sh.cnt.t_mpB;
+        F.n_tab_built = sh.cnt.tables_built; F.n_tab_reused = sh.cnt.tables_reused;
 #if FC_VARIANT_BIG && !defined(FC_SERIAL_PROFILE)
         F.dbg[2] = tk[OP_CHROMA]; F.dbg[3] = tk[OP_PRED_SETUP]; F.dbg[4] = tk[OP_PRED_FINISH];
         F.dbg[5] = tk[OP_NORMS]; F.dbg[6] = tk[OP_MC_SEARCH];
diff --git a/fiasco_amd/csrc/hip/mp_device.inc b/fiasco_amd/csrc/hip/mp_device.inc
--- a/fiasco_amd/csrc/hip/mp_device.inc
+++ b/fiasco_amd/csrc/hip/mp_device.inc
@@ -300,7 +300,7 @@
 #endif
     }
 }
-#else
+#elif FC_VARIANT_BIG
 __device__ __noinline__ void mp_tables(const DevFrame &F, Sh &sh, int level, int y)
 {
     const int tid = threadIdx.x;
@@ -316,7 +316,49 @@
         if (y == 0) { q1 -= sh.m0tab[qac_shift(m.d0_yindex)]; q1 += (float) qac_shift(m.d0_yindex); }
         else        { q1 -= sh.m0tab[qac_shift(m.d0_index)];  q1 += (float) qac_shift(m.d0_index); }
         sh.Q0 = q0; sh.Q1 = q1;
-#if !FC_VARIANT_BIG
+    }
+    if (tid < om + 12) {
+        int ci = 0, ti = 0, role = 0;
+        const int r = tid - om;
+        if (tid < dcs) { role = 1; ci = tid; ti = 0; }
+        else if (tid >= 64 && tid < 64 + sy) { role = 1; ci = dcs + ctx * sy + tid - 64; ti = ctx + 1; }
+        else if (r == 6) {
+            role = 1; ci = dcs + ctx * sy - 1; ti = ctx + 1;
+        }
+        else if (r >= 0 && r < MAXED + 1) { role = 2; ci = r; }
+        float num = 1.0f, den = 1.0f;
+        if (role == 1)      { num = (float) sh.cb.cnt[ci]; den = (float) sh.cb.tot[ti]; }
+        else if (role == 2) { num = (float) sh.pool.count[ci]; den = (float) sh.pool.total; }
+        float p = num / den;
+        const double lg = log2((double) p);
+        if (role == 1) {
+            if (tid < dcs) sh.lgdc[tid] = lg;
+            else if (r == 6) sh.lglv_m1 = lg;
+            else sh.lglv[tid - 64] = lg;
+        } else if (role == 2) sh.Ltab[ci] = (float) -lg;
+    }
+}
+
+#else
+__device__ __noinline__ bool mp_tables(const DevFrame &F, Sh &sh, int level, int y)
+{
+    const int tid = threadIdx.x;
+    const int dcs = sh.par.dcs, sy = sh.par.sy;
+    const int ctx = level - sh.par.lc_min_opt;
+    const int all = sh.tab_all, nl = all ? ctx + 1 : 1, ctx0 = all ? 0 : ctx;
+    const bool build = !all || !sh.par.tab_reuse || sh.tab_ver != sh.model_ver || ctx > sh.tab_top;
+    const int om = 64 + nl * sy, nrole = om + MAXED + 1 + 5 * nl;
+    const int slw = (nrole + 63) & ~63, sl = slw < B ? slw : nrole;
+    if (tid == sl) {
+        const Pool &m = sh.pool;
+        float q0 = 0, q1;
+        if (m.d0_n && y != 0) q0 += sh.m0tab[qac_shift(m.d0_index)];
+        if (y >= 0) q0 += sh.m0tab[qac_shift(m.d0_yindex)];
+        q1 = q0;
+        if (y == 0) { q1 -= sh.m0tab[qac_shift(m.d0_yindex)]; q1 += (float) qac_shift(m.d0_yindex); }
+        else        { q1 -= sh.m0tab[qac_shift(m.d0_index)];  q1 += (float) qac_shift(m.d0_index); }
+        sh.Q0 = q0; sh.Q1 = q1;
+        sh.lv = ctx - ctx0; sh.lv_off = (ctx - ctx0) * sy;
         if (!sh.band) {
             MPState &mp = sh.mp;
             const unsigned N = (unsigned) sh.pool.n;
@@ -332,54 +374,54 @@
             mp.s1_has = 0u;
             mp.np = 0;
         }
-#endif
-    }
-    if (tid < om + 12) {
+    }
+    if (build && tid < nrole) {
         int ci = 0, ti = 0, role = 0;
-        const int r = tid - om;
+        const int t1 = tid - 64;
+        const int r = tid - om - (MAXED + 1);
+        const int c = r >= 0 ? r / 5 : 0, k = r - 5 * c;
         if (tid < dcs) { role = 1; ci = tid; ti = 0; }
-        else if (tid >= 64 && tid < 64 + sy) { role = 1; ci = dcs + ctx * sy + tid - 64; ti = ctx + 1; }
-        else if (r == 6) {
-            role = 1; ci = dcs + ctx * sy - 1; ti = ctx + 1;
-        }
-        else if (r >= 0 && r < MAXED + 1) { role = 2; ci = r; }
-#if !FC_VARIANT_BIG
-        else if (r == 7 || r == 8) role = 3;
-        else if (r == 9 && !sh.band) {
-            role = 1; ci = dcs + ctx * sy + sh.par.half_nd; ti = ctx + 1;
-        } else if (r == 10 && !sh.band) {
-            role = 1; ci = sh.par.half_dc; ti = 0;
-        }
-#endif
+        else if (t1 >= 0 && tid < om) {
+            role = 1; ci = dcs + ctx0 * sy + t1;
+            ti = ctx0 + 1 + (t1 >= sy) + (t1 >= 2 * sy) + (t1 >= 3 * sy) + (t1 >= 4 * sy);
+        }
+        else if (tid >= om && r < 0) { role = 2; ci = tid - om; }
+        else if (r >= 0 && k == 0) {
+            role = 1; ci = dcs + (ctx0 + c) * sy - 1; ti = ctx0 + c + 1;
+        }
+        else if (r >= 0 && k <= 2) role = 3;
+        else if (r >= 0 && k == 3) { role = 1; ci = dcs + (ctx0 + c) * sy + sh.par.half_nd; ti = ctx0 + c + 1; }
+        else if (r >= 0) { role = 1; ci = sh.par.half_dc; ti = 0; }
         float num = 1.0f, den = 1.0f;
         if (role == 1)      { num = (float) sh.cb.cnt[ci]; den = (float) sh.cb.tot[ti]; }
         else if (role == 2) { num = (float) sh.pool.count[ci]; den = (float) sh.pool.total; }
-#if !FC_VARIANT_BIG
         else if (role == 3) {
             const unsigned *counts = sh.tm;
-            num = (float) counts[level]; den = (float) counts[sh.par.ML + level];
-        }
-#endif
+            const int lvl = sh.par.lc_min_opt + ctx0 + c;
+            num = (float) counts[lvl]; den = (float) counts[sh.par.ML + lvl];
+        }
         float p = num / den;
-#if !FC_VARIANT_BIG
-        if (r == 7) p = 1 - p;
-#endif
+        if (role == 3 && k == 1) p = 1 - p;
         const double lg = log2((double) p);
         if (role == 1) {
             if (tid < dcs) sh.lgdc[tid] = lg;
-            else if (r == 6) sh.lglv_m1 = lg;
-#if !FC_VARIANT_BIG
-            else if (r == 9) sh.mp.wb_nd = sub_log2(sh, 0.0f, lg, ci, ti);
-            else if (r == 10) sh.mp.wb_dc = sub_log2(sh, 0.0f, lg, ci, ti);
-#endif
-            else sh.lglv[tid - 64] = lg;
+            else if (r < 0) sh.lglv[t1] = lg;
+            else if (k == 0) sh.lglv_m1[c] = lg;
+            else sh.wbp[c][k - 3] = sub_log2(sh, 0.0f, lg, ci, ti);
         } else if (role == 2) sh.Ltab[ci] = (float) -lg;
-#if !FC_VARIANT_BIG
-        else if (role == 3) sh.tb[r - 7] = (float) -lg;
-#endif
-    }
-}
-
+        else if (role == 3) sh.tb[c][k - 1] = (float) -lg;
+    }
+    return build;
+}
+
+#endif
+
+#if FC_VARIANT_BIG
+__device__ __forceinline__ const double *call_lglv(const Sh &sh) { return sh.lglv; }
+__device__ __forceinline__ double call_lglv_m1(const Sh &sh) { return sh.lglv_m1; }
+#else
+__device__ __forceinline__ const double *call_lglv(const Sh &sh) { return sh.lglv + uni(sh.lv_off); }
+__device__ __forceinline__ double call_lglv_m1(const Sh &sh) { return sh.lglv_m1[sh.lv]; }
 #endif
 
 __device__ void mp_step_prepare(const DevFrame &F, Sh &sh, MPState &mp, const double *lglv, double lglv_m1)
@@ -558,6 +600,9 @@
             sh.cb.tot[0]++;
         }
     }
+#if !FC_VARIANT_BIG
+    sh.model_ver = ++sh.ver_next;
+#endif
 }
 
 __device__ __forceinline__ float wave_min_l63(float v)
@@ -635,6 +680,7 @@
 {
     const int tid = threadIdx.x, lane = tid & 63, wave = tid >> 6, P = F.P;
     MPState &mp = sh.mp;
+    const double *const lglv = call_lglv(sh);
     const int S = sh.states;
     const int nblk = (S + 63) >> 6;
     constexpr int U = 4;
@@ -746,7 +792,7 @@
                     if (pass) {
                         float i0 = n > 0 ? F.ipdo[d] : 0.0f, i1 = n > 1 ? F.ipdo[(size_t) P + d] : 0.0f;
                         float i2 = n > 2 ? F.ipdo[(size_t) 2 * P + d] : 0.0f, i3 = n > 3 ? F.ipdo[(size_t) 3 * P + d] : 0.0f;
-                        full_eval<MAXED - 1>(F, sh, mp, sh.lglv, n, F.pos[d], d, F.num[d], F.den[d], i0, i1, i2, i3, ev);
+                        full_eval<MAXED - 1>(F, sh, mp, lglv, n, F.pos[d], d, F.num[d], F.den[d], i0, i1, i2, i3, ev);
                     }
                     evals += (unsigned) __popcll(__ballot(pass));
                     blockevals++;
@@ -789,7 +835,7 @@
                         if (k < n) mp.sel_ipdo[n][k] = F.ipdo[(size_t) k * P + b_state];
                     mp.row_state = b_state;
                     mp.n = n + 1;
-                    if (mp.n < F.max_elements) mp_step_prepare(F, sh, mp, sh.lglv, sh.lglv_m1);
+                    if (mp.n < F.max_elements) mp_step_prepare(F, sh, mp, lglv, call_lglv_m1(sh));
                 }
                 mp.index = index;
             }
@@ -806,6 +852,7 @@
 {
     const int tid = threadIdx.x, lane = tid & 63, wave = tid >> 6, P = F.P;
     MPState &mp = sh.mp;
+    const double *const lglv = call_lglv(sh);
     const int16_t *const list = F.pool_states;
     const int nblk = (D + 63) >> 6;
     unsigned blockevals = 0;
@@ -893,7 +940,7 @@
 #if FC_GM
                         ev.qc = GM_QAC(sh.gm.pk[0]) && c < (int) sh.pool.n ? (int) GQ_CUR(sh, 0)[c] : 0;
 #endif
-                        full_eval<MAXED - 1>(F, sh, mp, sh.lglv, n, c, list[c], F.num[c], F.den[c], i0, i1, i2, i3, ev);
+                        full_eval<MAXED - 1>(F, sh, mp, lglv, n, c, list[c], F.num[c], F.den[c], i0, i1, i2, i3, ev);
                     }
                     evals += (unsigned) __popcll(__ballot(pass));
                     blockevals++;
@@ -940,7 +987,7 @@
                         if (k < n) mp.sel_ipdo[n][k] = F.ipdo[(size_t) k * P + index];
                     mp.row_state = b_state;
                     mp.n = n + 1;
-                    if (mp.n < F.max_elements) mp_step_prepare(F, sh, mp, sh.lglv, sh.lglv_m1);
+                    if (mp.n < F.max_elements) mp_step_prepare(F, sh, mp, lglv, call_lglv_m1(sh));
                 }
                 mp.index = index;
             }
@@ -979,7 +1026,13 @@
 #define APX_MARK(i) do { } while (0)
 #endif
     if (fr.coop) snap_coop_before(sh, fr, sh.sp, sh.par.ML);
+#if FC_VARIANT_BIG
     mp_tables(F, sh, level, y);
+#else
+    const unsigned ver = (unsigned) uni((int) sh.model_ver);
+    const bool built = uni((int) mp_tables(F, sh, level, y)) != 0;
+    const int lv = uni(sh.tab_all ? level - sh.par.lc_min_opt : 0);
+#endif
     __syncthreads();
     APX_MARK(0);
     const int S = sh.states;
@@ -1043,8 +1096,8 @@
         mp.ab = fr.lrange.tree_bits + fr.lrange.mv_tree_bits + fr.lrange.mv_coord_bits + fr.lrange.nd_tree_bits
                 + fr.lrange.nd_weights_bits;
 #else
-        fr.lrange.tree_bits = sh.tb[0];
-        mp.ab = sh.tb[0];
+        fr.lrange.tree_bits = sh.tb[lv][0];
+        mp.ab = sh.tb[lv][0];
 #endif
         mp.price = fr.price;
         mp.err = mp.norm;
@@ -1058,7 +1111,7 @@
 #if FC_VARIANT_BIG
         mp_step_prepare(F, sh, mp, sh.lglv, sh.lglv_m1);
 #else
-        if (sh.band) mp_step_prepare(F, sh, mp, sh.lglv, sh.lglv_m1);
+        if (sh.band) mp_step_prepare(F, sh, mp, sh.lglv + lv * sh.par.sy, sh.lglv_m1[lv]);
         else {
             const float L0 = sh.Ltab[0], L1 = sh.Ltab[1], q0 = sh.Q0, q1 = sh.Q1;
             float b = L1; b += q0; mp.s1_pre[0] = b;
@@ -1068,6 +1121,11 @@
         }
 #endif
     }
+#if !FC_VARIANT_BIG
+    else if (tid == 64 && !sh.band) {
+        mp.wb_nd = sh.wbp[lv][0]; mp.wb_dc = sh.wbp[lv][1];
+    }
+#endif
     lds_barrier();
 
     APX_MARK(1);
@@ -1200,6 +1258,8 @@
     else if (tid == 64) {
         sh.cnt.bytes_mp += 4ull * D * (2 + mp.n) + 4ull * (1u << level);
         sh.cnt.n_mp++; sh.cnt.n_steps += mp.n;
+        if (built) { sh.tab_ver = ver; sh.tab_top = lv; sh.cnt.tables_built++; }
+        else sh.cnt.tables_reused++;
     }
 #endif
     if (fr.coop) {
diff --git a/fiasco_amd/csrc/hip/mp_reg.inc b/fiasco_amd/csrc/hip/mp_reg.inc
--- a/fiasco_amd/csrc/hip/mp_reg.inc
+++ b/fiasco_amd/csrc/hip/mp_reg.inc
@@ -39,6 +39,7 @@
     const int tid = (int) utid, lane = tid & 63, wave = tid >> 6, P = sh.par.P;
     MPState &mp = sh.mp;
     RoundBox &rb = sh.rb;
+    const double *const lglv = call_lglv(sh);
     const int S = sh.states, K = (S + B - 1) / B, nblk = (S + 63) >> 6;
     const float rsize = 1.0f / size;
     SPEC_DEADMASK(sh)
@@ -235,7 +236,7 @@
                 for (int k = 0; k < MAXED; k++) ev.f[k] = 0;
                 const float i0 = ipk[0], i1 = NIP > 1 ? ipk[1 % NIP] : 0.0f;
                 const float i2 = NIP > 2 ? ipk[2 % NIP] : 0.0f, i3 = NIP > 3 ? ipk[3 % NIP] : 0.0f;
-                if (pass) full_eval<NIP>(F, sh, mp, sh.lglv, n, psk, state, numk, denk, i0, i1, i2, i3, ev);
+                if (pass) full_eval<NIP>(F, sh, mp, lglv, n, psk, state, numk, denk, i0, i1, i2, i3, ev);
                 unsigned npass = (unsigned) __popcll(__ballot(pass));
                 int last = -1, win = -1;
                 for (;;) {
@@ -281,7 +282,7 @@
                 for (int k = 0; k < MAXED - 1; k++) if (k < n) mp.sel_ipdo[n][k] = rb.ip[k];
                 mp.row_state = bstate;
                 mp.n = n + 1;
-                if (mp.n < sh.par.max_elements) mp_step_prepare(F, sh, mp, sh.lglv, sh.lglv_m1);
+                if (mp.n < sh.par.max_elements) mp_step_prepare(F, sh, mp, lglv, call_lglv_m1(sh));
             }
             mp.index = index;
         }
@@ -302,6 +303,7 @@
     const int tid = threadIdx.x, P = sh.par.P;
     MPState &mp = sh.mp;
     RoundBox &rb = sh.rb;
+    const double *const lglv = call_lglv(sh);
     const bool ok = tid < D;
     const int st = ok ? (int) sh.dl[tid] : 0;
     float den = ok ? sh.par.diag[(size_t) q * P + st] : 1.0f;
@@ -348,7 +350,7 @@
 #pragma unroll
             for (int k = 0; k < MAXED; k++) ev.f[k] = 0;
             if (pass)
-                full_eval<NIP>(F, sh, mp, sh.lglv, n, tid, st, num, den, ip[0], NIP > 1 ? ip[1 % NIP] : 0.0f,
+                full_eval<NIP>(F, sh, mp, lglv, n, tid, st, num, den, ip[0], NIP > 1 ? ip[1 % NIP] : 0.0f,
                           NIP > 2 ? ip[2 % NIP] : 0.0f, NIP > 3 ? ip[3 % NIP] : 0.0f, ev);
             evals += (unsigned) __popcll(__ballot(pass));
             int last = -1, win = -1;
@@ -391,7 +393,7 @@
                 for (int k = 0; k < MAXED - 1; k++) if (k < n) mp.sel_ipdo[n][k] = rb.ip[k];
                 mp.row_state = bstate;
                 mp.n = n + 1;
-                if (mp.n < sh.par.max_elements) mp_step_prepare(F, sh, mp, sh.lglv, sh.lglv_m1);
+                if (mp.n < sh.par.max_elements) mp_step_prepare(F, sh, mp, lglv, call_lglv_m1(sh));
             }
             mp.index = index;
         }
diff --git a/include/libfiasco_amd_hip.h b/include/libfiasco_amd_hip.h
--- a/include/libfiasco_amd_hip.h
+++ b/include/libfiasco_amd_hip.h
@@ -24,6 +24,7 @@
     unsigned long long decoder_frames, decoder_bytes, decoder_us;
     unsigned long long coop_frames, coop_workgroups;
     unsigned long long spec_app_rows, spec_app_wait;
+    unsigned long long tables_built, tables_reused;
 } fiasco_amd_stats;
 
 void fiasco_amd_get_stats(fiasco_amd_stats *out);
```
